# hku-systems/apus

Measured on NVIDIA B200. Metric: committed ops/s, higher is better.
Workload: dtype u8

## Files before the change

### apus_b200/csrc/apus_engine.cu

```cuda
#include <cuda.h>
#include <cuda_runtime.h>
#include <emmintrin.h>
#include <pthread.h>
#include <sched.h>
#include <stdarg.h>
#include <stdint.h>
#include <stdio.h>
#include <stdlib.h>
#include <string.h>
#include <time.h>
#include <unistd.h>

#include "apus_gpu.h"
#include "apus_layout.h"

extern "C" cudaError_t apus_launch_roles(const apus_role_t *d_roles, int n_roles, cudaStream_t stream);
extern "C" size_t apus_kernel_smem_bytes(void);

#define MAX_ROLES 160
static __thread char g_err[512];

static int fail(const char *fmt, ...)
{
    va_list ap;
    va_start(ap, fmt);
    vsnprintf(g_err, sizeof g_err, fmt, ap);
    va_end(ap);
    return APUS_ERROR;
}

#define CK(call)                                                                             \
    do {                                                                                     \
        cudaError_t _e = (call);                                                             \
        if (_e != cudaSuccess)                                                               \
            return fail("%s failed: %s (%s:%d)", #call, cudaGetErrorString(_e), __FILE__, __LINE__); \
    } while (0)

struct drv_t {
    CUresult (*MemCreate)(CUmemGenericAllocationHandle *, size_t, const CUmemAllocationProp *, unsigned long long);
    CUresult (*MemAddressReserve)(CUdeviceptr *, size_t, size_t, CUdeviceptr, unsigned long long);
    CUresult (*MemMap)(CUdeviceptr, size_t, size_t, CUmemGenericAllocationHandle, unsigned long long);
    CUresult (*MemSetAccess)(CUdeviceptr, size_t, const CUmemAccessDesc *, size_t);
    CUresult (*MemGetAllocationGranularity)(size_t *, const CUmemAllocationProp *, CUmemAllocationGranularity_flags);
    CUresult (*MemUnmap)(CUdeviceptr, size_t);
    CUresult (*MemRelease)(CUmemGenericAllocationHandle);
    CUresult (*MemAddressFree)(CUdeviceptr, size_t);
    CUresult (*MulticastCreate)(CUmemGenericAllocationHandle *, const CUmulticastObjectProp *);
    CUresult (*MulticastAddDevice)(CUmemGenericAllocationHandle, CUdevice);
    CUresult (*MulticastBindMem)(CUmemGenericAllocationHandle, size_t, CUmemGenericAllocationHandle, size_t, size_t, unsigned long long);
    CUresult (*MulticastGetGranularity)(size_t *, const CUmulticastObjectProp *, CUmulticastGranularity_flags);
    CUresult (*DeviceGetAttribute)(int *, CUdevice_attribute, CUdevice);
    int ok;
};
static drv_t g_drv;
static int drv_load(void)
{
    if (g_drv.ok) return APUS_OK;
#define DRV(field, name) do { void *fn = NULL; cudaDriverEntryPointQueryResult qr;                                   \
        if (cudaGetDriverEntryPoint(name, &fn, cudaEnableDefault, &qr) != cudaSuccess || !fn) {                    \
            cudaGetLastError(); return fail("driver entry point %s is not available", name); }                      \
        *(void **)(&g_drv.field) = fn; } while (0)
    DRV(MemCreate, "cuMemCreate"); DRV(MemAddressReserve, "cuMemAddressReserve"); DRV(MemMap, "cuMemMap");
    DRV(MemSetAccess, "cuMemSetAccess"); DRV(MemGetAllocationGranularity, "cuMemGetAllocationGranularity");
    DRV(MemUnmap, "cuMemUnmap"); DRV(MemRelease, "cuMemRelease"); DRV(MemAddressFree, "cuMemAddressFree");
    DRV(MulticastCreate, "cuMulticastCreate"); DRV(MulticastAddDevice, "cuMulticastAddDevice");
    DRV(MulticastBindMem, "cuMulticastBindMem"); DRV(MulticastGetGranularity, "cuMulticastGetGranularity");
    DRV(DeviceGetAttribute, "cuDeviceGetAttribute");
#undef DRV
    g_drv.ok = 1;
    return APUS_OK;
}
#define CU(call) do { CUresult _e = (call); if (_e != CUDA_SUCCESS) return fail("%s failed: driver error %d (%s:%d)", #call, (int)_e, __FILE__, __LINE__); } while (0)

struct StageLock {
    pthread_mutex_t *m;
    explicit StageLock(pthread_mutex_t *mu) : m(mu) { pthread_mutex_lock(m); }
    ~StageLock() { pthread_mutex_unlock(m); }
};

struct DeviceGuard {
    int prev;
    bool ok;
    explicit DeviceGuard(int dev) : prev(-1), ok(false)
    {
        if (cudaGetDevice(&prev) != cudaSuccess) prev = -1;
        ok = (cudaSetDevice(dev) == cudaSuccess);
    }
    ~DeviceGuard()
    {
        if (prev >= 0) cudaSetDevice(prev);
    }
};

#define PEER_MAGIC 0x4150555342323030ull

struct peer_blob {
    uint64_t magic;
    int64_t  pid;
    int32_t  device;
    uint32_t pad;
    uint64_t ptr;
    uint64_t bytes;
    cudaIpcMemHandle_t ipc;
};
static_assert(sizeof(peer_blob) <= sizeof(apus_peer_handle_t), "peer handle too small");

struct apus_replica {
    apus_config_t cfg;
    uint64_t log_len;
    uint64_t entries_off;
    uint32_t idx_cap;
    uint8_t *region;
    size_t   region_bytes;
    apus_devctx_t  h_ctx;
    apus_devctx_t *d_ctx;
    apus_role_t   *d_roles;
    apus_hostwords_t *hw;
    apus_hostwords_t *hw_dev;
    apus_slot_t *ring_desc_host;
    uint8_t     *ring_pay_host;
    apus_slot_t *ring_desc_dev;
    uint8_t     *ring_pay_dev;
    uint64_t    *sub_tail_dev;
    uint64_t    *sub_tail_stage;
    uint32_t ring_slots, ring_bytes;
    uint64_t submitted, flushed;
    uint64_t belled;
    CUmemGenericAllocationHandle vmm_handle;
    size_t   vmm_bytes;
    CUmemGenericAllocationHandle mc_handle;
    uint8_t *mc_region;
    uint8_t *stage;
    pthread_mutex_t stage_mu;
    size_t   stage_bytes;
    uint64_t pay_head;
    uint64_t pay_flushed;
    uint64_t *pay_end;
    int      defer;
    cudaStream_t stream, copy_stream;
    cudaEvent_t  ev_start, ev_stop;
    apus_replica *launch_owner;
    int      in_flight;
    uint64_t launches;
    void    *peer_ptr[APUS_MAX_SERVERS];
    int      peer_is_ipc[APUS_MAX_SERVERS];
    uint32_t *d_lat;
};

extern "C" int apus_abi_version(void) { return APUS_ABI_VERSION; }
extern "C" const char *apus_last_error(void) { return g_err; }
extern "C" int apus_device_count(void)
{
    int n = 0;
    if (cudaGetDeviceCount(&n) != cudaSuccess) return 0;
    return n;
}

extern "C" int apus_device_numa_node(int device)
{
    char bus[64] = {0}, path[160];
    if (cudaDeviceGetPCIBusId(bus, sizeof bus, device) != cudaSuccess) { cudaGetLastError(); return -1; }
    for (char *c = bus; *c; c++) if (*c >= 'A' && *c <= 'F') *c = (char)(*c - 'A' + 'a');
    snprintf(path, sizeof path, "/sys/bus/pci/devices/%s/numa_node", bus);
    FILE *f = fopen(path, "r");
    if (!f) return -1;
    int node = -1;
    if (fscanf(f, "%d", &node) != 1) node = -1;
    fclose(f);
    return node;
}

static inline int is_leader(const apus_replica *r) { return r->cfg.server_idx == r->cfg.leader_idx; }

static int ensure_host_ring(apus_replica *r)
{
    if (r->ring_desc_host) return APUS_OK;
    CK(cudaHostAlloc(&r->ring_desc_host, sizeof(apus_slot_t) * r->ring_slots, cudaHostAllocMapped | cudaHostAllocPortable));
    CK(cudaHostAlloc(&r->ring_pay_host, r->ring_bytes, cudaHostAllocMapped | cudaHostAllocPortable));
    return APUS_OK;
}

static int fabric_alloc_region(apus_replica *r);
static int leader_ring_init(apus_replica *r)
{
    if (r->pay_end) return APUS_OK;
    if (!r->ring_slots) { r->ring_slots = r->cfg.ring_slots ? r->cfg.ring_slots : (1u << 16);
                          r->ring_bytes = r->cfg.ring_bytes ? r->cfg.ring_bytes : (16u << 20); }
    r->pay_end = (uint64_t *)calloc(r->ring_slots, sizeof(uint64_t));
    if (!r->pay_end) return fail("out of memory");
    if (r->cfg.ring_mode == APUS_RING_HOST_MAPPED) {
        if (ensure_host_ring(r) != APUS_OK) return APUS_ERROR;
        memset(r->ring_desc_host, 0, sizeof(apus_slot_t) * r->ring_slots);
        CK(cudaHostGetDevicePointer(&r->ring_desc_dev, r->ring_desc_host, 0));
        CK(cudaHostGetDevicePointer(&r->ring_pay_dev, r->ring_pay_host, 0));
    } else {
        CK(cudaMalloc(&r->ring_desc_dev, sizeof(apus_slot_t) * r->ring_slots));
        CK(cudaMalloc(&r->ring_pay_dev, r->ring_bytes));
        CK(cudaMalloc(&r->sub_tail_dev, 128));
        CK(cudaMemset(r->sub_tail_dev, 0, 128));
        CK(cudaHostAlloc(&r->sub_tail_stage, 64, cudaHostAllocPortable));
    }
    return APUS_OK;
}

static int replica_init(apus_replica *r, const apus_config_t *cfg, uint64_t log_len)
{
    r->log_len = log_len;
    uint32_t cap = 1024;
    while ((uint64_t)cap * 64ull < log_len) cap <<= 1;
    r->idx_cap = cap;
    r->entries_off = (APUS_INDEX_OFF + (uint64_t)cap * 4ull + 4095ull) & ~4095ull;
    r->region_bytes = r->entries_off + log_len;
    if (r->cfg.flags & APUS_F_FABRIC) { if (fabric_alloc_region(r) != APUS_OK) return APUS_ERROR; }
    else CK(cudaMalloc(&r->region, r->region_bytes));
    CK(cudaMemset(r->region, 0, r->region_bytes));
    apus_loghdr_t h;
    memset(&h, 0, sizeof h);
    h.len = log_len; h.end = log_len; h.tail = log_len; h.old_end = log_len;
    CK(cudaMemcpy(r->region + APUS_HDR_OFF, &h, sizeof h, cudaMemcpyHostToDevice));
    apus_ctrl_t c;
    memset(&c, 0, sizeof c);
    c.next_idx = 1;
    c.pend_head_end = log_len;
    CK(cudaMemcpy(r->region, &c, sizeof c, cudaMemcpyHostToDevice));

    CK(cudaHostAlloc(&r->hw, sizeof(apus_hostwords_t), cudaHostAllocMapped | cudaHostAllocPortable));
    memset((void *)r->hw, 0, sizeof(apus_hostwords_t));
    CK(cudaHostGetDevicePointer(&r->hw_dev, r->hw, 0));
    pthread_mutex_init(&r->stage_mu, NULL);
    r->stage_bytes = 1u << 20;
    CK(cudaHostAlloc(&r->stage, r->stage_bytes, cudaHostAllocPortable));
    CK(cudaMalloc(&r->d_ctx, sizeof(apus_devctx_t)));
    CK(cudaMalloc(&r->d_roles, sizeof(apus_role_t) * MAX_ROLES));
    CK(cudaMalloc(&r->d_lat, sizeof(uint32_t) * APUS_LAT_RING));
    CK(cudaMemset(r->d_lat, 0, sizeof(uint32_t) * APUS_LAT_RING));
    CK(cudaStreamCreateWithFlags(&r->stream, cudaStreamNonBlocking));
    CK(cudaStreamCreateWithFlags(&r->copy_stream, cudaStreamNonBlocking));
    CK(cudaEventCreate(&r->ev_start));
    CK(cudaEventCreate(&r->ev_stop));

    if (is_leader(r) && leader_ring_init(r) != APUS_OK) return APUS_ERROR;
    {
        apus_ctlwords_t w;
        memset(&w, 0, sizeof w);
        w.sid = (r->cfg.term << 9) | (1ull << 8) | r->cfg.leader_idx;
        for (int i = 0; i < 16; i++) w.vote_ack[i] = log_len;
        CK(cudaMemcpy(r->region + APUS_CTL_OFF, &w, sizeof w, cudaMemcpyHostToDevice));
    }
    r->peer_ptr[cfg->server_idx] = r->region;
    return APUS_OK;
}

extern "C" int apus_replica_create(const apus_config_t *cfg, apus_replica_t **out)
{
    if (!cfg || !out) return fail("null argument");
    if (cfg->struct_size != sizeof(apus_config_t) && cfg->struct_size != APUS_CONFIG_SIZE_V1)
        return fail("apus_config_t size mismatch (ABI)");
    if (cfg->group_size < 1 || cfg->group_size > APUS_MAX_SERVER_COUNT) return fail("group_size out of range");
    if (cfg->server_idx >= cfg->group_size || cfg->leader_idx >= cfg->group_size) return fail("bad server/leader idx");
    int ndev = apus_device_count();
    if (ndev <= 0) return fail("no CUDA device: the engine has no CPU fallback");
    if (cfg->device < 0 || cfg->device >= ndev) return fail("device %d out of range (%d present)", cfg->device, ndev);
    uint64_t log_len = cfg->log_size ? cfg->log_size : APUS_LOG_SIZE;
    if (log_len % 4096 || log_len < 8192) return fail("log_size must be a multiple of 4096 (>= 8192)");
    if (log_len > (1ull << 31)) return fail("log_size above 2 GiB is not supported (32-bit offset index)");
    uint32_t slots = cfg->ring_slots ? cfg->ring_slots : (1u << 16);
    uint32_t bytes = cfg->ring_bytes ? cfg->ring_bytes : (16u << 20);
    if (slots & (slots - 1)) return fail("ring_slots must be a power of two");
    if (bytes % 4096 || bytes < (1u << 17)) return fail("ring_bytes must be a multiple of 4096, >= 128 KiB");
    if (bytes / 16 > 0x00ffffffu) return fail("ring_bytes too large for the 24-bit descriptor offset");

    DeviceGuard g(cfg->device);
    if (!g.ok) return fail("cudaSetDevice(%d) failed", cfg->device);
    apus_replica *r = (apus_replica *)calloc(1, sizeof(*r));
    if (!r) return fail("out of memory");
    memset(&r->cfg, 0, sizeof r->cfg);
    memcpy(&r->cfg, cfg, cfg->struct_size);
    r->cfg.struct_size = sizeof(apus_config_t);
    if (!(r->cfg.flags & APUS_F_EXPLICIT)) r->cfg.flags |= APUS_F_DEVICE_STATS;
    if (cfg->server_idx == cfg->leader_idx) { r->ring_slots = slots; r->ring_bytes = bytes; }
    if (replica_init(r, cfg, log_len) != APUS_OK) {
        char keep[sizeof g_err];
        memcpy(keep, g_err, sizeof keep);
        apus_replica_destroy(r);
        memcpy(g_err, keep, sizeof keep);
        return APUS_ERROR;
    }
    *out = r;
    return APUS_OK;
}

extern "C" void apus_replica_destroy(apus_replica_t *r)
{
    if (!r) return;
    DeviceGuard g(r->cfg.device);
    if (r->in_flight && r->hw) {
        r->hw->stop = 1;
        cudaEventSynchronize(r->launch_owner ? r->launch_owner->ev_stop : r->ev_stop);
    }
    for (int i = 0; i < APUS_MAX_SERVER_COUNT; i++)
        if (r->peer_is_ipc[i] && r->peer_ptr[i]) cudaIpcCloseMemHandle(r->peer_ptr[i]);
    if (r->cfg.ring_mode != APUS_RING_HOST_MAPPED) {
        if (r->ring_desc_dev) cudaFree(r->ring_desc_dev);
        if (r->ring_pay_dev) cudaFree(r->ring_pay_dev);
        if (r->sub_tail_dev) cudaFree(r->sub_tail_dev);
        if (r->sub_tail_stage) cudaFreeHost(r->sub_tail_stage);
    }
    if (r->ring_desc_host) cudaFreeHost(r->ring_desc_host);
    if (r->ring_pay_host) cudaFreeHost(r->ring_pay_host);
    if (r->stage) cudaFreeHost(r->stage);
    if (r->d_lat) cudaFree(r->d_lat);
    if (r->d_roles) cudaFree(r->d_roles);
    if (r->d_ctx) cudaFree(r->d_ctx);
    if (r->ev_start) cudaEventDestroy(r->ev_start);
    if (r->ev_stop) cudaEventDestroy(r->ev_stop);
    if (r->stream) cudaStreamDestroy(r->stream);
    if (r->copy_stream) cudaStreamDestroy(r->copy_stream);
    if (r->hw) cudaFreeHost((void *)r->hw);
    if (r->vmm_handle && g_drv.ok) {
// ... 433 lines not shown
static void pool_run(const fill_job *j)
{
    pthread_mutex_lock(&g_pool_run);
    pthread_mutex_lock(&g_pool.mu);
    if (!g_pool.started) {
        int want = 8;
        const char *e = getenv("apus_submit_threads");
        if (e) want = atoi(e);
        long cores = sysconf(_SC_NPROCESSORS_ONLN);
        if (want > cores - 1) want = (int)cores - 1;
        if (want > POOL_MAX) want = POOL_MAX;
        if (want < 1) want = 1;
        g_pool.nthreads = want - 1;
        for (int i = 0; i < g_pool.nthreads; i++)
            if (pthread_create(&g_pool.th[i], NULL, pool_main, NULL)) { g_pool.nthreads = i; break; }
        g_pool.started = 1;
    }
    g_pool.job = j;
    g_pool.chunk = 4096;
    g_pool.parts = (j->n + g_pool.chunk - 1) / g_pool.chunk;
    g_pool.next = 0; g_pool.done_parts = 0;
    g_pool.progressive = (j->r->cfg.ring_mode == APUS_RING_HOST_MAPPED && !j->r->defer && j->r->flushed == j->r->submitted);
    g_pool.adv = 0; g_pool.adv_lock = 0;
    static uint8_t *done_buf; static uint32_t done_cap;
    if (done_cap < g_pool.parts) { free(done_buf); done_cap = g_pool.parts * 2; done_buf = (uint8_t *)malloc(done_cap); }
    memset(done_buf, 0, g_pool.parts);
    g_pool.done = done_buf;
    __atomic_fetch_add(&g_pool.gen, 1, __ATOMIC_RELEASE);
    pthread_cond_broadcast(&g_pool.cv);
    pthread_mutex_unlock(&g_pool.mu);
    pool_work(j);
    while (__atomic_load_n(&g_pool.done_parts, __ATOMIC_ACQUIRE) < g_pool.parts) _mm_pause();
    pthread_mutex_unlock(&g_pool_run);
}

extern "C" int apus_submit_uniform(apus_replica_t *r, uint32_t n, uint8_t type, uint16_t connection_id,
                                   uint64_t first_req_id, uint16_t len, const void *payloads, size_t stride,
                                   uint64_t *first_ticket)
{
    if (!r) return fail("null argument");
    if (!is_leader(r)) return fail("submit on a follower");
    if (len && !payloads) return fail("null payload");
    if (n == 0) return APUS_OK;
    const uint64_t consumed = r->hw->consumed;
    if (r->submitted + n - consumed > r->ring_slots) { snprintf(g_err, sizeof g_err, "submission ring full"); return APUS_RETRY; }
    if (!r->ring_desc_host && ensure_host_ring(r) != APUS_OK) return APUS_ERROR;
    const uint32_t mask = r->ring_slots - 1;
    const uint32_t nb = image_bytes(type, len);
    fill_job j;
    memset(&j, 0, sizeof j);
    j.r = r; j.n = n; j.type = type; j.conn = connection_id; j.first_req = first_req_id; j.len = len;
    j.payloads = (const uint8_t *)payloads; j.stride = stride; j.first_slot = r->submitted;
    uint32_t *tos = NULL; uint64_t *poss = NULL;
    uint64_t head = r->pay_head;
    if (nb > APUS_SLOT_INLINE) {
        tos = (uint32_t *)malloc(sizeof(uint32_t) * n); poss = (uint64_t *)malloc(sizeof(uint64_t) * n);
        if (!tos || !poss) { free(tos); free(poss); return fail("out of memory"); }
        for (uint32_t k = 0; k < n; k++) {
            int rc = place_image(r, type, nb, consumed, &head, &tos[k], &poss[k]);
            if (rc != APUS_OK) { free(tos); free(poss); snprintf(g_err, sizeof g_err, "payload ring full"); return rc; }
            r->pay_end[(r->submitted + k) & mask] = head;
        }
        j.type_off = tos; j.pos = poss;
    } else {
        j.type_off_inline = ((uint32_t)type & APUS_SLOT_TYPE_MASK) << APUS_SLOT_TYPE_SHIFT;
        for (uint32_t k = 0; k < n; k++) r->pay_end[(r->submitted + k) & mask] = head;
    }
    if (n >= 16384) pool_run(&j); else fill_range(&j, 0, n);
    free(tos); free(poss);
    r->pay_head = head;
    if (first_ticket) *first_ticket = r->submitted + 1;
    r->submitted += n;
    if (!r->defer) return ring_flush(r);
    return APUS_OK;
}

__global__ void apus_synth_kernel(apus_slot_t *ring, uint32_t mask, uint8_t *pay, uint64_t first_slot, uint32_t n,
                                  uint32_t type, uint32_t conn, uint64_t first_req, uint32_t len, uint32_t seed,
                                  uint64_t pay_pos0, uint32_t need)
{
    for (uint32_t k = blockIdx.x * blockDim.x + threadIdx.x; k < n; k += gridDim.x * blockDim.x) {
        const uint64_t s = first_slot + k, req = first_req + k;
        apus_slot_t *d = &ring[s & mask];
        const uint32_t nb = 2u + len;
        uint32_t type_off = (type & APUS_SLOT_TYPE_MASK) << APUS_SLOT_TYPE_SHIFT;
        uint8_t *dst0 = d->inl0, *dst1 = d->inl1;
        if (need) {
            const uint64_t pos = pay_pos0 + (uint64_t)k * need;
            type_off |= APUS_SLOT_EXT | (uint32_t)(pos / 16);
            uint8_t *p = pay + pos;
            p[0] = (uint8_t)len; p[1] = (uint8_t)(len >> 8);
            for (uint32_t q = 0; q < len; q++) p[2 + q] = synth_byte(seed, req, q);
        } else {
            for (uint32_t q = 0; q < nb; q++) {
                const uint8_t v = q == 0 ? (uint8_t)len : q == 1 ? (uint8_t)(len >> 8) : synth_byte(seed, req, q - 2);
                if (q < 32) dst0[q] = v; else dst1[q - 32] = v;
            }
        }
        d->req_id = req; d->type_off = type_off; d->len = (uint16_t)len; d->clt_id = (uint16_t)conn;
        d->stamp0 = s + 1; d->stamp1 = s + 1; d->rsv0 = 0; d->rsv1 = 0;
    }
}

extern "C" int apus_submit_synth(apus_replica_t *r, uint32_t n, uint8_t type, uint16_t connection_id,
                                 uint64_t first_req_id, uint16_t len, uint32_t seed, uint64_t *first_ticket)
{
    if (!r) return fail("null argument");
    if (!is_leader(r)) return fail("submit on a follower");
    if (r->cfg.ring_mode != APUS_RING_DEVICE) return fail("apus_submit_synth needs the device submission ring");
    if (type == APUS_NOOP || type == APUS_CONFIG || type == APUS_HEAD) return fail("apus_submit_synth: request types only");
    if (n == 0) return APUS_OK;
    const uint64_t consumed = r->hw->consumed;
    if (r->submitted + n - consumed > r->ring_slots) { snprintf(g_err, sizeof g_err, "submission ring full"); return APUS_RETRY; }
    if (r->flushed != r->submitted) { int rc = ring_push(r); if (rc != APUS_OK) return rc; }
    const uint32_t mask = r->ring_slots - 1;
    const uint32_t nb = 2u + len;
    uint32_t need = 0;
    uint64_t pos0 = 0, head = r->pay_head;
    if (nb > APUS_SLOT_INLINE) {
        need = (nb + 15u) & ~15u;
        const uint64_t R = r->ring_bytes;
        pos0 = head % R;
        const uint64_t tail = consumed ? r->pay_end[(consumed - 1) & mask] : 0;
        if (pos0 + (uint64_t)n * need > R || (head - tail) + (uint64_t)n * need > R)
            return fail("apus_submit_synth: %u images of %u B do not fit the payload ring without wrapping", n, need);
    }
    DeviceGuard g(r->cfg.device);
    const int threads = 256;
    int blocks = (int)((n + threads - 1) / threads);
    if (blocks > 148 * 8) blocks = 148 * 8;
    apus_synth_kernel<<<blocks, threads, 0, r->copy_stream>>>(r->ring_desc_dev, mask, r->ring_pay_dev, r->submitted, n, type,
                                                              connection_id, first_req_id, len, seed, pos0, need);
    CK(cudaGetLastError());
    CK(cudaStreamSynchronize(r->copy_stream));
    for (uint32_t k = 0; k < n; k++) { head += need; r->pay_end[(r->submitted + k) & mask] = head; }
    r->pay_head = head; r->pay_flushed = head;
    if (first_ticket) *first_ticket = r->submitted + 1;
    r->submitted += n;
    r->flushed = r->submitted;
    if (!r->defer) return ring_bell(r, r->submitted);
    return APUS_OK;
}

extern "C" int apus_submit_defer(apus_replica_t *r, int defer)
{
    if (!r) return fail("null argument");
    r->defer = defer;
    return APUS_OK;
}
extern "C" int apus_submit_flush(apus_replica_t *r)
{
    if (!r) return fail("null argument");
    return ring_flush(r);
}
extern "C" int apus_submit_release(apus_replica_t *r, uint64_t ticket)
{
    if (!r) return fail("null argument");
    if (ticket > r->submitted) return fail("release beyond what was submitted");
    int rc = ring_push(r);
    if (rc != APUS_OK) return rc;
    DeviceGuard g(r->cfg.device);
    return ring_bell(r, ticket);
}

extern "C" uint64_t apus_committed_tickets(apus_replica_t *r) { return r ? r->hw->committed_tickets : 0; }

extern "C" int apus_progress(apus_replica_t *r, uint64_t *offset, uint64_t *count)
{
    if (!r) return fail("null argument");
    const __m128i v = _mm_load_si128((const __m128i *)(const void *)&r->hw->commit_off);
    uint64_t w[2];
    _mm_storeu_si128((__m128i *)w, v);
    if (offset) *offset = w[0];
    if (count) *count = w[1];
    return r->hw->error ? fail("kernel reported protocol error %llu", (unsigned long long)r->hw->error) : APUS_OK;
}

extern "C" int apus_wait_committed(apus_replica_t *r, uint64_t ticket, int64_t timeout_us)
{
    if (!r) return fail("null argument");
    if (r->hw->committed_tickets >= ticket) return APUS_OK;
    struct timespec t0, t;
    clock_gettime(CLOCK_MONOTONIC, &t0);
    uint32_t spins = 0;
    while (r->hw->committed_tickets < ticket) {
        if ((++spins & 0x3ff) == 0) {
            if (r->hw->error) return fail("kernel reported protocol error %llu", (unsigned long long)r->hw->error);
            if (timeout_us >= 0) {
                clock_gettime(CLOCK_MONOTONIC, &t);
                int64_t us = (t.tv_sec - t0.tv_sec) * 1000000 + (t.tv_nsec - t0.tv_nsec) / 1000;
                if (us > timeout_us) { snprintf(g_err, sizeof g_err, "timeout"); return APUS_RETRY; }
            }
        }
    }
    return APUS_OK;
}

extern "C" int apus_closed_loop(apus_replica_t *r, uint32_t n, uint16_t payload_len, uint16_t connection_id,
                                uint64_t first_req_id, uint32_t *lat_ns)
{
    if (!r || !lat_ns) return fail("null argument");
    if (!is_leader(r)) return fail("submit on a follower");
    uint8_t *buf = (uint8_t *)malloc(payload_len ? payload_len : 1);
    if (!buf) return fail("out of memory");
    for (uint32_t k = 0; k < payload_len; k++) buf[k] = (uint8_t)(k * 131u + 7u);
    struct timespec t0, t1;
    for (uint32_t i = 0; i < n; i++) {
        clock_gettime(CLOCK_MONOTONIC, &t0);
        int rc = ring_put(r, APUS_SEND, connection_id, first_req_id + i, buf, payload_len);
        if (rc == APUS_OK) rc = ring_flush(r);
        if (rc != APUS_OK) { free(buf); return rc == APUS_RETRY ? rc : fail("closed loop: submit failed"); }
        const uint64_t ticket = r->submitted;
        uint32_t spins = 0;
        while (r->hw->committed_tickets < ticket) {
            if ((++spins & 0xffffff) == 0) {
                clock_gettime(CLOCK_MONOTONIC, &t1);
                if (t1.tv_sec - t0.tv_sec > 10 || r->hw->error) { free(buf); return fail("closed loop: commit timeout"); }
            }
        }
        clock_gettime(CLOCK_MONOTONIC, &t1);
        int64_t ns = (t1.tv_sec - t0.tv_sec) * 1000000000ll + (t1.tv_nsec - t0.tv_nsec);
        lat_ns[i] = ns > 0xffffffffll ? 0xffffffffu : (uint32_t)ns;
    }
    free(buf);
    return APUS_OK;
}

extern "C" int apus_log_offsets(apus_replica_t *r, apus_log_offsets_t *out)
{
    if (!r || !out) return fail("null argument");
    DeviceGuard g(r->cfg.device);
    apus_loghdr_t h;
    CK(cudaMemcpyAsync(&h, r->region + APUS_HDR_OFF, sizeof h, cudaMemcpyDeviceToHost, r->copy_stream));
    CK(cudaStreamSynchronize(r->copy_stream));
    out->head = h.head; out->apply = h.apply; out->commit = h.commit; out->end = h.end;
    out->tail = h.tail; out->old_end = h.old_end; out->old_commit = h.old_commit; out->len = h.len;
    return APUS_OK;
}

extern "C" int apus_log_read(apus_replica_t *r, uint64_t off, uint64_t len, void *dst)
{
    if (!r || !dst) return fail("null argument");
    if (off + len > r->log_len) return fail("range beyond the log");
    DeviceGuard g(r->cfg.device);
    StageLock sl(&r->stage_mu);
    uint8_t *out = (uint8_t *)dst;
    while (len) {
        const uint64_t run = len < r->stage_bytes ? len : r->stage_bytes;
        CK(cudaMemcpyAsync(r->stage, r->region + r->entries_off + off, run, cudaMemcpyDeviceToHost, r->copy_stream));
        CK(cudaStreamSynchronize(r->copy_stream));
        memcpy(out, r->stage, run);
        out += run; off += run; len -= run;
    }
    return APUS_OK;
}

extern "C" int apus_log_read_range(apus_replica_t *r, uint64_t from, uint64_t to, void *dst, uint64_t cap, uint64_t *got)
{
    if (!r || !dst || !got) return fail("null argument");
    if (from >= r->log_len || to >= r->log_len) return fail("range beyond the log");
    const uint64_t L = r->log_len;
    uint64_t n1 = to >= from ? to - from : L - from, n2 = to >= from ? 0 : to;
    if (n1 > cap) { n1 = cap; n2 = 0; }
    if (n1 + n2 > cap) n2 = cap - n1;
    int rc = n1 ? apus_log_read(r, from, n1, dst) : APUS_OK;
    if (rc == APUS_OK && n2) rc = apus_log_read(r, 0, n2, (uint8_t *)dst + n1);
    *got = n1 + n2;
    return rc;
}

extern "C" int apus_set_applied(apus_replica_t *r, uint64_t offset)
{
    if (!r) return fail("null argument");
    if (offset >= r->log_len) return fail("offset beyond the log");
    r->hw->host_apply = offset;
    return APUS_OK;
}

extern "C" uint64_t apus_leader_suspect(apus_replica_t *r) { return r ? r->hw->leader_suspect : 0; }
extern "C" uint64_t apus_last_commit_ns(apus_replica_t *r) { return r ? r->hw->last_commit_ns : 0; }

extern "C" int apus_get_stats(apus_replica_t *r, apus_stats_t *out)
{
    if (!r || !out) return fail("null argument");
    DeviceGuard g(r->cfg.device);
    apus_ctrl_t c;
    CK(cudaMemcpyAsync(&c, r->region, sizeof c, cudaMemcpyDeviceToHost, r->copy_stream));
    CK(cudaStreamSynchronize(r->copy_stream));
    memset(out, 0, sizeof *out);
    out->tickets_submitted = r->submitted;
    out->tickets_consumed = c.consumed;
    out->tickets_committed = c.committed_tickets;
    out->entries_acked = c.acked;
    out->bytes_replicated = c.bytes_replicated;
    out->batches = c.batches;
    out->kernel_launches = r->launches;
    out->lat_samples = c.lat_count;
    out->auto_heads = c.auto_heads;
    out->entries_published = c.published;
    for (int i = 0; i < 8; i++) { out->phase_ns[i] = c.phase_ns[i]; out->turn_ns[i] = c.turn_ns[i]; }
    return APUS_OK;
}

extern "C" int apus_latency_samples(apus_replica_t *r, uint32_t *dst, uint32_t max, uint32_t *n)
{
    if (!r || !dst || !n) return fail("null argument");
    DeviceGuard g(r->cfg.device);
    apus_ctrl_t c;
    CK(cudaMemcpyAsync(&c, r->region, sizeof c, cudaMemcpyDeviceToHost, r->copy_stream));
    CK(cudaStreamSynchronize(r->copy_stream));
    uint64_t have = c.lat_count < APUS_LAT_RING ? c.lat_count : APUS_LAT_RING;
    uint32_t take = (uint32_t)(have < max ? have : max);
    uint32_t *tmp = (uint32_t *)malloc(sizeof(uint32_t) * APUS_LAT_RING);
    if (!tmp) return fail("out of memory");
    cudaError_t e = cudaMemcpyAsync(tmp, r->d_lat, sizeof(uint32_t) * APUS_LAT_RING, cudaMemcpyDeviceToHost, r->copy_stream);
    if (e == cudaSuccess) e = cudaStreamSynchronize(r->copy_stream);
    if (e != cudaSuccess) { free(tmp); return fail("latency copy failed: %s", cudaGetErrorString(e)); }
    for (uint32_t k = 0; k < take; k++)
        dst[k] = tmp[(c.lat_count - take + k) & (APUS_LAT_RING - 1)];
    free(tmp);
    *n = take;
    return APUS_OK;
}



static int fabric_alloc_region(apus_replica *r)
{
    if (drv_load() != APUS_OK) return APUS_ERROR;
    int ndev = apus_device_count();
    CUmemAllocationProp ap;
    memset(&ap, 0, sizeof ap);
    ap.type = CU_MEM_ALLOCATION_TYPE_PINNED;
    ap.location.type = CU_MEM_LOCATION_TYPE_DEVICE;
    ap.location.id = r->cfg.device;
    ap.requestedHandleTypes = CU_MEM_HANDLE_TYPE_POSIX_FILE_DESCRIPTOR;
    size_t gran = 0;
    CU(g_drv.MemGetAllocationGranularity(&gran, &ap, CU_MEM_ALLOC_GRANULARITY_RECOMMENDED));
    if (gran < (2u << 20)) gran = 2u << 20;
    r->vmm_bytes = (r->region_bytes + gran - 1) / gran * gran;
    CU(g_drv.MemCreate(&r->vmm_handle, r->vmm_bytes, &ap, 0));
    CUdeviceptr va = 0;
    CU(g_drv.MemAddressReserve(&va, r->vmm_bytes, gran, 0, 0));
    CU(g_drv.MemMap(va, r->vmm_bytes, 0, r->vmm_handle, 0));
    CUmemAccessDesc acc[64];
    for (int d = 0; d < ndev && d < 64; d++) { acc[d].location.type = CU_MEM_LOCATION_TYPE_DEVICE; acc[d].location.id = d; acc[d].flags = CU_MEM_ACCESS_FLAGS_PROT_READWRITE; }
    CU(g_drv.MemSetAccess(va, r->vmm_bytes, acc, (size_t)(ndev < 64 ? ndev : 64)));
    r->region = (uint8_t *)va;
    return APUS_OK;
}

extern "C" int apus_group_multicast(apus_replica_t **rs, int n)
{
    if (!rs || n < 2 || n > APUS_MAX_SERVER_COUNT) return fail("bad replica list");
    if (drv_load() != APUS_OK) return APUS_ERROR;
    apus_replica *lead = NULL;
    for (int i = 0; i < n; i++) {
        if (!rs[i] || !rs[i]->vmm_handle) return fail("replica %d was not created with APUS_F_FABRIC", i);
        if (rs[i]->in_flight) return fail("stop the kernels first");
        if (rs[i]->vmm_bytes != rs[0]->vmm_bytes) return fail("regions differ in size");
        for (int j = 0; j < i; j++) if (rs[j]->cfg.device == rs[i]->cfg.device) return fail("multicast needs one GPU per replica");
        int mc = 0;
        CU(g_drv.DeviceGetAttribute(&mc, CU_DEVICE_ATTRIBUTE_MULTICAST_SUPPORTED, rs[i]->cfg.device));
        if (!mc) return fail("device %d does not support multicast", rs[i]->cfg.device);
        if (is_leader(rs[i])) lead = rs[i];
    }
    if (!lead) return fail("no leader in the list");
    if (lead->mc_region) return APUS_OK;
    CUmulticastObjectProp mp;
    memset(&mp, 0, sizeof mp);
    mp.numDevices = (unsigned)n; mp.size = lead->vmm_bytes; mp.handleTypes = CU_MEM_HANDLE_TYPE_POSIX_FILE_DESCRIPTOR;
    size_t mgran = 0;
    CU(g_drv.MulticastGetGranularity(&mgran, &mp, CU_MULTICAST_GRANULARITY_MINIMUM));
    if (lead->vmm_bytes % mgran) return fail("region size %zu is not a multiple of the multicast granularity %zu", lead->vmm_bytes, mgran);
    CU(g_drv.MulticastCreate(&lead->mc_handle, &mp));
    for (int i = 0; i < n; i++) CU(g_drv.MulticastAddDevice(lead->mc_handle, rs[i]->cfg.device));
    for (int i = 0; i < n; i++) {
        DeviceGuard g(rs[i]->cfg.device);
        CU(g_drv.MulticastBindMem(lead->mc_handle, 0, rs[i]->vmm_handle, 0, rs[i]->vmm_bytes, 0));
    }
    DeviceGuard g(lead->cfg.device);
    CUdeviceptr va = 0;
    CU(g_drv.MemAddressReserve(&va, lead->vmm_bytes, mgran, 0, 0));
    CU(g_drv.MemMap(va, lead->vmm_bytes, 0, lead->mc_handle, 0));
    CUmemAccessDesc acc;
    acc.location.type = CU_MEM_LOCATION_TYPE_DEVICE; acc.location.id = lead->cfg.device; acc.flags = CU_MEM_ACCESS_FLAGS_PROT_READWRITE;
    CU(g_drv.MemSetAccess(va, lead->vmm_bytes, &acc, 1));
    lead->mc_region = (uint8_t *)va;
    return APUS_OK;
}

#define SID_TERM(s) ((s) >> 9)

static int own_read(apus_replica *r, size_t off, void *dst, size_t len)
{
    StageLock sl(&r->stage_mu);
    CK(cudaMemcpyAsync(r->stage, r->region + off, len, cudaMemcpyDeviceToHost, r->copy_stream));
    CK(cudaStreamSynchronize(r->copy_stream));
    memcpy(dst, r->stage, len);
    return APUS_OK;
}
static int own_write(apus_replica *r, size_t off, const void *src, size_t len)
{
    StageLock sl(&r->stage_mu);
    memcpy(r->stage, src, len);
    CK(cudaMemcpyAsync(r->region + off, r->stage, len, cudaMemcpyHostToDevice, r->copy_stream));
    CK(cudaStreamSynchronize(r->copy_stream));
    return APUS_OK;
}
static int peer_read(apus_replica *r, uint8_t peer, size_t off, void *dst, size_t len)
{
    StageLock sl(&r->stage_mu);
    if (!r->peer_ptr[peer]) return fail("peer %u is not connected", (unsigned)peer);
    CK(cudaMemcpyAsync(r->stage, (uint8_t *)r->peer_ptr[peer] + off, len, cudaMemcpyDefault, r->copy_stream));
    CK(cudaStreamSynchronize(r->copy_stream));
    memcpy(dst, r->stage, len);
    return APUS_OK;
}
static int peer_write(apus_replica *r, uint8_t peer, size_t off, const void *src, size_t len)
{
    StageLock sl(&r->stage_mu);
    if (!r->peer_ptr[peer]) return fail("peer %u is not connected", (unsigned)peer);
    memcpy(r->stage, src, len);
    CK(cudaMemcpyAsync((uint8_t *)r->peer_ptr[peer] + off, r->stage, len, cudaMemcpyDefault, r->copy_stream));
    CK(cudaStreamSynchronize(r->copy_stream));
    return APUS_OK;
}

extern "C" int apus_ctl_read(apus_replica_t *r, apus_ctl_view_t *out)
{
    if (!r || !out) return fail("null argument");
    DeviceGuard g(r->cfg.device);
    apus_ctlwords_t w;
    if (own_read(r, APUS_CTL_OFF, &w, sizeof w) != APUS_OK) return APUS_ERROR;
    memset(out, 0, sizeof *out);
    out->sid = w.sid; out->leader_sid = w.leader_sid; out->adj_end = w.adj_end; out->adj_count = w.adj_count;
    for (int i = 0; i < APUS_MAX_SERVER_COUNT; i++) {
        out->vote_ack[i] = w.vote_ack[i];
        out->vote_req[i].sid = w.vote_req[i].sid; out->vote_req[i].index = w.vote_req[i].index;
        out->vote_req[i].term = w.vote_req[i].term;
        out->vote_req[i].cid[0] = w.vote_req[i].cid[0]; out->vote_req[i].cid[1] = w.vote_req[i].cid[1];
    }
    return APUS_OK;
}

extern "C" int apus_ctl_set_sid(apus_replica_t *r, uint64_t sid)
{
    if (!r) return fail("null argument");
    DeviceGuard g(r->cfg.device);
    return own_write(r, APUS_CTL_OFF + offsetof(apus_ctlwords_t, sid), &sid, 8);
}

extern "C" int apus_ctl_reset_votes(apus_replica_t *r)
{
    if (!r) return fail("null argument");
    DeviceGuard g(r->cfg.device);
    uint64_t v[16];
    for (int i = 0; i < 16; i++) v[i] = r->log_len;
    return own_write(r, APUS_CTL_OFF + offsetof(apus_ctlwords_t, vote_ack), v, sizeof v);
}

extern "C" int apus_ctl_clear_vote_request(apus_replica_t *r, uint8_t from_idx)
{
    if (!r || from_idx >= APUS_MAX_SERVER_COUNT) return fail("bad argument");
    DeviceGuard g(r->cfg.device);
    uint64_t z = 0;
    return own_write(r, APUS_CTL_OFF + offsetof(apus_ctlwords_t, vote_req) + sizeof(apus_vote_req_t) * from_idx, &z, 8);
}

extern "C" int apus_ctl_send_vote_request(apus_replica_t *r, uint8_t peer_idx, uint64_t sid, uint64_t index, uint64_t term,
                                          const void *cid16)
{
    if (!r || peer_idx >= r->cfg.group_size) return fail("bad argument");
    DeviceGuard g(r->cfg.device);
    apus_vote_req_t q;
    memset(&q, 0, sizeof q);
    q.index = index; q.term = term;
    if (cid16) memcpy(q.cid, cid16, 16);
    const size_t base = APUS_CTL_OFF + offsetof(apus_ctlwords_t, vote_req) + sizeof(apus_vote_req_t) * r->cfg.server_idx;
    if (peer_write(r, peer_idx, base + 8, (uint8_t *)&q + 8, sizeof q - 8) != APUS_OK) return APUS_ERROR;
    return peer_write(r, peer_idx, base, &sid, 8);
}

extern "C" int apus_ctl_send_vote_ack(apus_replica_t *r, uint8_t candidate_idx, uint64_t commit)
{
    if (!r || candidate_idx >= r->cfg.group_size) return fail("bad argument");
    DeviceGuard g(r->cfg.device);
    return peer_write(r, candidate_idx, APUS_CTL_OFF + offsetof(apus_ctlwords_t, vote_ack) + 8u * r->cfg.server_idx, &commit, 8);
}

static int entry_at(apus_replica *r, int peer, uint64_t cum, uint64_t *off, uint64_t *idx, uint64_t *term, uint32_t *stride)
{
    uint32_t w = 0;
    const size_t ioff = APUS_INDEX_OFF + 4ull * (cum & (r->idx_cap - 1));
    int rc = peer < 0 ? own_read(r, ioff, &w, 4) : peer_read(r, (uint8_t)peer, ioff, &w, 4);
    if (rc != APUS_OK) return rc;
    const uint64_t o = w & ~APUS_IDX_HEAD_FLAG;
    if (o + APUS_HDR_BYTES > r->log_len) return fail("offset index names an offset beyond the log");
    uint8_t h[64];
    rc = peer < 0 ? own_read(r, r->entries_off + o, h, 64) : peer_read(r, (uint8_t)peer, r->entries_off + o, h, 64);
    if (rc != APUS_OK) return rc;
    memcpy(idx, h + E_IDX, 8); memcpy(term, h + E_TERM, 8);
    uint16_t len; memcpy(&len, h + E_DATA, 2);
    const uint8_t ty = h[E_TYPE];
    *stride = (ty == T_NOOP || ty == T_CONFIG || ty == T_HEAD) ? APUS_HDR_BYTES : APUS_HDR_BYTES + len;
    *off = o;
    return APUS_OK;
}

extern "C" int apus_ctl_heartbeat(apus_replica_t *r, uint64_t *word)
{
    if (!r || !word) return fail("null argument");
    DeviceGuard g(r->cfg.device);
    return own_read(r, offsetof(apus_ctrl_t, hb), word, sizeof *word);
}

extern "C" int apus_ctl_last_entry(apus_replica_t *r, uint64_t *idx, uint64_t *term, uint64_t *commit, uint64_t *end)
{
    if (!r || !idx || !term) return fail("null argument");
    if (r->in_flight) return fail("the replica's kernel must be stopped (exclusive log access)");
    DeviceGuard g(r->cfg.device);
    apus_loghdr_t h; apus_ctrl_t c;
    if (own_read(r, APUS_HDR_OFF, &h, sizeof h) != APUS_OK || own_read(r, 0, &c, sizeof c) != APUS_OK) return APUS_ERROR;
    if (commit) *commit = h.commit;
    if (end) *end = h.end;
    const uint64_t count = is_leader(r) ? c.published : c.acked;
    *idx = 0; *term = 0;
    if (h.end == r->log_len || count == 0) return APUS_OK;
    uint64_t off; uint32_t stride;
    if (entry_at(r, -1, count, &off, idx, term, &stride) != APUS_OK) return APUS_ERROR;
    if (*idx != count) return fail("entry counter %llu does not match the idx %llu of the last entry", (unsigned long long)count, (unsigned long long)*idx);
    return APUS_OK;
}

static int copy_to_peer(apus_replica *r, uint8_t peer, size_t off, size_t len)
{
    if (!len) return APUS_OK;
    CK(cudaMemcpyAsync((uint8_t *)r->peer_ptr[peer] + off, r->region + off, len, cudaMemcpyDefault, r->copy_stream));
    return APUS_OK;
}

extern "C" int apus_ctl_adjust_follower(apus_replica_t *r, uint8_t peer, uint64_t sid, uint64_t *resent)
{
    if (!r || peer >= r->cfg.group_size || peer == r->cfg.server_idx) return fail("bad argument");
    if (!is_leader(r)) return fail("log adjustment is the leader's job");
    if (r->in_flight) return fail("the leader's kernel must be stopped");
    if (!r->peer_ptr[peer]) return fail("peer %u is not connected", (unsigned)peer);
    DeviceGuard g(r->cfg.device);
    const uint64_t L = r->log_len;
    apus_loghdr_t mh, fh; apus_ctrl_t mc, fc;
    if (own_read(r, APUS_HDR_OFF, &mh, sizeof mh) != APUS_OK || own_read(r, 0, &mc, sizeof mc) != APUS_OK) return APUS_ERROR;
    if (peer_read(r, peer, APUS_HDR_OFF, &fh, sizeof fh) != APUS_OK || peer_read(r, peer, 0, &fc, sizeof fc) != APUS_OK) return APUS_ERROR;
    const uint64_t mine = mc.published, theirs = fc.acked;
    uint64_t j = mine < theirs ? mine : theirs;
    uint64_t keep_end = (mh.end == L) ? L : 0;
    bool found = false;
    while (j > 0) {
        uint64_t o1, i1, t1, o2, i2, t2; uint32_t s1, s2;
        if (entry_at(r, -1, j, &o1, &i1, &t1, &s1) != APUS_OK || entry_at(r, peer, j, &o2, &i2, &t2, &s2) != APUS_OK) return APUS_ERROR;
        if (o1 == o2 && i1 == i2 && t1 == t2 && i1 == j) { keep_end = o1 + s1; if (keep_end == L) keep_end = 0; found = true; break; }
        j--;
    }
    if (!found) { j = 0; keep_end = 0; }
    uint64_t bytes = 0;
    if (mine > j && mh.end != L) {
        const uint64_t from = (j == 0) ? mh.head : keep_end;
        const uint64_t to = mh.end;
        if (to > from) { if (copy_to_peer(r, peer, r->entries_off + from, to - from) != APUS_OK) return APUS_ERROR; bytes += to - from; }
        else if (to < from || (to == from && mine > j)) {
            if (copy_to_peer(r, peer, r->entries_off + from, L - from) != APUS_OK) return APUS_ERROR;
            if (copy_to_peer(r, peer, r->entries_off, to) != APUS_OK) return APUS_ERROR;
            bytes += L - from + to;
        }
        const uint64_t cap = r->idx_cap, a = (j + 1) & (cap - 1), n = mine - j;
        if (n >= cap) { if (copy_to_peer(r, peer, APUS_INDEX_OFF, 4ull * cap) != APUS_OK) return APUS_ERROR; }
        else if (a + n <= cap) { if (copy_to_peer(r, peer, APUS_INDEX_OFF + 4ull * a, 4ull * n) != APUS_OK) return APUS_ERROR; }
        else {
            if (copy_to_peer(r, peer, APUS_INDEX_OFF + 4ull * a, 4ull * (cap - a)) != APUS_OK) return APUS_ERROR;
            if (copy_to_peer(r, peer, APUS_INDEX_OFF, 4ull * (a + n - cap)) != APUS_OK) return APUS_ERROR;
        }
        CK(cudaStreamSynchronize(r->copy_stream));
    }
    if (j == 0) {
        if (peer_write(r, peer, APUS_HDR_OFF + offsetof(apus_loghdr_t, head), &mh.head, 8) != APUS_OK) return APUS_ERROR;
        if (peer_write(r, peer, APUS_HDR_OFF + offsetof(apus_loghdr_t, commit), &mh.commit, 8) != APUS_OK) return APUS_ERROR;
    }
    const uint64_t endw[2] = { mh.end, mh.end };
    if (peer_write(r, peer, APUS_HDR_OFF + offsetof(apus_loghdr_t, end), &endw[0], 8) != APUS_OK) return APUS_ERROR;
    if (peer_write(r, peer, APUS_HDR_OFF + offsetof(apus_loghdr_t, old_end), &endw[1], 8) != APUS_OK) return APUS_ERROR;
    if (peer_write(r, peer, offsetof(apus_ctrl_t, acked), &mine, 8) != APUS_OK) return APUS_ERROR;
    const uint64_t none = L;
    if (peer_write(r, peer, offsetof(apus_ctrl_t, pend_head_end), &none, 8) != APUS_OK) return APUS_ERROR;
    if (own_write(r, offsetof(apus_ctrl_t, ack) + 8u * peer, &mine, 8) != APUS_OK) return APUS_ERROR;
    const uint64_t adj[3] = { sid, mh.end, mine };
    if (peer_write(r, peer, APUS_CTL_OFF + offsetof(apus_ctlwords_t, adj_end), &adj[1], 16) != APUS_OK) return APUS_ERROR;
    if (peer_write(r, peer, APUS_CTL_OFF + offsetof(apus_ctlwords_t, leader_sid), &adj[0], 8) != APUS_OK) return APUS_ERROR;
    if (resent) *resent = bytes;
    return APUS_OK;
}

extern "C" int apus_follower_beats(apus_replica_t *r, uint64_t out[APUS_MAX_SERVER_COUNT])
{
    if (!r || !out) return fail("null argument");
    DeviceGuard g(r->cfg.device);
    uint64_t b[16];
    if (own_read(r, offsetof(apus_ctrl_t, fbeat), b, sizeof b) != APUS_OK) return APUS_ERROR;
// ... 83 lines not shown
```

### apus_b200/csrc/apus_kernels.cu

```cuda
#include <cuda_runtime.h>
#include <stdint.h>

#include "apus_layout.h"
#include "apus_cert.h"

__device__ __forceinline__ uint64_t ld_relaxed_sys(const volatile void *p)
{
    uint64_t v;
    asm volatile("ld.relaxed.sys.global.u64 %0, [%1];" : "=l"(v) : "l"(p) : "memory");
    return v;
}
__device__ __forceinline__ uint64_t ld_acquire_sys(const volatile void *p)
{
    uint64_t v;
    asm volatile("ld.acquire.sys.global.u64 %0, [%1];" : "=l"(v) : "l"(p) : "memory");
    return v;
}
__device__ __forceinline__ uint32_t ld_relaxed_sys_u32(const volatile void *p)
{
    uint32_t v;
    asm volatile("ld.relaxed.sys.global.u32 %0, [%1];" : "=r"(v) : "l"(p) : "memory");
    return v;
}
__device__ __forceinline__ void ld_acquire_sys_2x64(const volatile void *p, uint64_t &a, uint64_t &b)
{
    asm volatile("ld.acquire.sys.global.v2.u64 {%0,%1}, [%2];" : "=l"(a), "=l"(b) : "l"(p) : "memory");
}
__device__ __forceinline__ void ld_relaxed_sys_2x64(const volatile void *p, uint64_t &a, uint64_t &b)
{
    asm volatile("ld.relaxed.sys.global.v2.u64 {%0,%1}, [%2];" : "=l"(a), "=l"(b) : "l"(p) : "memory");
}
__device__ __forceinline__ void st_relaxed_sys(volatile void *p, uint64_t v)
{
    asm volatile("st.relaxed.sys.global.u64 [%0], %1;" ::"l"(p), "l"(v) : "memory");
}
__device__ __forceinline__ void st_relaxed_sys_2x64(volatile void *p, uint64_t a, uint64_t b)
{
    asm volatile("st.relaxed.sys.global.v2.u64 [%0], {%1,%2};" ::"l"(p), "l"(a), "l"(b) : "memory");
}
__device__ __forceinline__ void st_relaxed_sys_u8(volatile void *p, uint8_t v)
{
    asm volatile("st.relaxed.sys.global.u8 [%0], %1;" ::"l"(p), "r"((uint32_t)v) : "memory");
}
__device__ __forceinline__ uint4 ld_relaxed_sys_v4(const void *p)
{
    uint4 v;
    asm volatile("ld.relaxed.sys.global.v4.u32 {%0,%1,%2,%3}, [%4];"
                 : "=r"(v.x), "=r"(v.y), "=r"(v.z), "=r"(v.w)
                 : "l"(p)
                 : "memory");
    return v;
}
__device__ __forceinline__ void st_v4(void *p, uint4 v)
{
    asm volatile("st.global.v4.u32 [%0], {%1,%2,%3,%4};" ::"l"(p), "r"(v.x), "r"(v.y), "r"(v.z),
                 "r"(v.w)
                 : "memory");
}
__device__ __forceinline__ void mst_v4(void *p, uint4 v)
{
    asm volatile("multimem.st.relaxed.sys.global.v4.f32 [%0], {%1,%2,%3,%4};" ::"l"(p), "f"(__uint_as_float(v.x)),
                 "f"(__uint_as_float(v.y)), "f"(__uint_as_float(v.z)), "f"(__uint_as_float(v.w))
                 : "memory");
}
__device__ __forceinline__ void mst_u32(void *p, uint32_t v)
{
    asm volatile("multimem.st.relaxed.sys.global.b32 [%0], %1;" ::"l"(p), "r"(v) : "memory");
}
__device__ __forceinline__ void st_u8(void *p, uint32_t v)
{
    asm volatile("st.global.u8 [%0], %1;" ::"l"(p), "r"(v) : "memory");
}
__device__ __forceinline__ uint64_t globaltimer_ns()
{
    uint64_t t;
    asm volatile("mov.u64 %0, %%globaltimer;" : "=l"(t));
    return t;
}
__device__ __forceinline__ void bar_sync(int id, int nthreads)
{
    asm volatile("bar.sync %0, %1;" ::"r"(id), "r"(nthreads) : "memory");
}

__device__ __forceinline__ bool has_cmd(uint32_t type)
{
    return !(type == T_NOOP || type == T_CONFIG || type == T_HEAD);
}
__device__ __forceinline__ uint32_t data_bytes(uint32_t type, uint32_t len)
{
    if (type == T_NOOP) return 0;
    if (type == T_CONFIG) return 16;
    if (type == T_HEAD) return 8;
    return 2u + len;
}
__device__ __forceinline__ uint32_t entry_stride(uint32_t type, uint32_t len)
{
    return has_cmd(type) ? APUS_HDR_BYTES + len : APUS_HDR_BYTES;
}
__device__ __forceinline__ uint64_t ring_dist(uint64_t from, uint64_t to, uint64_t L)
{
    return to >= from ? to - from : L - (from - to);
}
__device__ __forceinline__ uint64_t adopt_head(uint64_t head, uint64_t carried, uint64_t new_end, uint64_t L)
{
    if (carried >= L) return head;
    const uint64_t ne = (new_end == L) ? 0 : new_end;
    return (ring_dist(head, carried, L) <= ring_dist(head, ne, L)) ? carried : head;
}
__device__ __forceinline__ uint64_t slot_head_value(const apus_cslot_t *sl)
{
    uint64_t v = 0;
#pragma unroll
    for (int q = 7; q >= 0; q--) v = (v << 8) | sl->inl[q];
    return v;
}

#define WATCHDOG_NS (20ull * 1000ull * 1000ull * 1000ull)

#define APUS_KERR_WATCHDOG_LEADER   1
#define APUS_KERR_WATCHDOG_FOLLOWER 2
#define APUS_KERR_WATCHDOG_COMMIT   3
#define APUS_KERR_BAD_ENTRY         4
#define APUS_KERR_COUNT_MISMATCH    5

#define N_PRODUCER_WARPS 15
#define NT (N_PRODUCER_WARPS * 32)
#define MAXB APUS_MAX_TILE_ENTRIES
#define PUBMASK (APUS_PUBRING_RECORDS - 1)

struct LeaderShared {
    uint32_t es[MAXB];
    uint32_t xb[MAXB];
    uint32_t cum_es[MAXB];
    uint32_t cum_xb[MAXB];
    uint32_t rel[MAXB];
    uint32_t xoff[MAXB];
    uint64_t ap[32];
    uint32_t ap_valid;
    uint32_t static_cut;
    uint32_t first_ext_all;
    uint32_t host_head_k;
    uint64_t idx_base;
    uint8_t  ty[MAXB];
    uint8_t  flg[MAXB];
    uint32_t n_fetch, finish, abort, was_blocked;
    uint32_t avg_es, avg_xb;
    uint64_t slot0, my_seq, t_dequeue, st_head, t_place_acq, pub_h, pub_tail_seen;
    uint64_t st_end, st_tail, st_next_idx, st_hwm, st_placed;
    uint32_t st_prev_head, pad0;
    uint32_t kbase, m, gap, ghost, fresh, auto_head, ext_bytes, last, blocked, hbytes;
    uint32_t base_es, base_xb, fast, pad1;
    uint64_t ext_base, auto_head_val, a, b, idx0, cum_after, new_end, tail_after, hwm_after;
    uint8_t  *peer_entries[APUS_MAX_SERVERS];
    uint32_t *peer_index[APUS_MAX_SERVERS];
};

#define LS_BYTES ((sizeof(LeaderShared) + 127u) & ~127u)
#define L_SLOTS_OFF LS_BYTES
#define L_EXT_OFF   (L_SLOTS_OFF + MAXB * APUS_CSLOT_BYTES)
#define L_IMG_OFF   (L_EXT_OFF + APUS_LEADER_EXT_BYTES)
#define L_TOTAL     (L_IMG_OFF + APUS_LEADER_IMG_BYTES + 16)

struct FollowerShared {
    uint32_t off[APUS_FOLLOWER_WIN_BYTES / 64 + 8];
    uint32_t n;
    uint32_t done;
    uint64_t win_lo, win_hi, next;
    uint64_t head_val, head_end;
    uint64_t end_seen, cum_seen, commit_seen;
    uint32_t head_j;
    uint32_t cert;
    uint64_t cert_start;
};
#define FS_BYTES ((sizeof(FollowerShared) + 127u) & ~127u)
#define F_TOTAL (FS_BYTES + APUS_FOLLOWER_WIN_BYTES + 16)

extern __shared__ __align__(16) uint8_t smem_raw[];

__device__ __forceinline__ uint64_t ld_acquire_gpu(const volatile void *p)
{
    uint64_t v;
    asm volatile("ld.acquire.gpu.global.u64 %0, [%1];" : "=l"(v) : "l"(p) : "memory");
    return v;
}
__device__ __forceinline__ void ld_acquire_gpu_2x64(const volatile void *p, uint64_t &a, uint64_t &b)
{
    asm volatile("ld.acquire.gpu.global.v2.u64 {%0,%1}, [%2];" : "=l"(a), "=l"(b) : "l"(p) : "memory");
}
__device__ __forceinline__ void st_release_gpu(volatile void *p, uint64_t v)
{
    asm volatile("st.release.gpu.global.u64 [%0], %1;" ::"l"(p), "l"(v) : "memory");
}

__device__ __forceinline__ uint64_t cs_chunk(const uint4 v, uint64_t lo, uint64_t a, uint64_t b)
{
    return cs_chunk_words((uint64_t)v.x | ((uint64_t)v.y << 32), (uint64_t)v.z | ((uint64_t)v.w << 32), lo, a, b);
}
__device__ __forceinline__ uint4 chunk_select(const uint4 nw, const uint4 old, int n)
{
    uint32_t a[4] = {nw.x, nw.y, nw.z, nw.w}, o[4] = {old.x, old.y, old.z, old.w}, r[4];
#pragma unroll
    for (int w = 0; w < 4; w++) {
        const int k = n - 4 * w;
        const uint32_t m = k >= 4 ? 0xffffffffu : (k <= 0 ? 0u : ((1u << (8 * k)) - 1u));
        r[w] = (a[w] & m) | (o[w] & ~m);
    }
    return make_uint4(r[0], r[1], r[2], r[3]);
}


__device__ __forceinline__ uint32_t hdr_byte(uint32_t j, uint64_t idx, uint64_t term, uint64_t req_id,
                                             uint32_t clt, uint32_t type, uint32_t sender)
{
    if (j < 8) return (uint32_t)(idx >> (8 * j)) & 0xFF;
    if (j < 16) return (uint32_t)(term >> (8 * (j - 8))) & 0xFF;
    if (j < 24) return (uint32_t)(req_id >> (8 * (j - 16))) & 0xFF;
    if (j == 24) return clt & 0xFF;
    if (j == 25) return (clt >> 8) & 0xFF;
    if (j == 26) return type;
    if (j == 27) return sender;
    return 0;
}

__device__ __noinline__ void group_write_header(uint8_t *e, int sub, int gl, uint64_t idx, uint64_t term, uint64_t req_id,
                                                   uint32_t clt, uint32_t type, uint32_t sender, bool skip_sender)
{
    if ((((uint32_t)(uintptr_t)e) & 15u) == 0 && !skip_sender) {
        if (sub == 0) *reinterpret_cast<uint4 *>(e + 0) = make_uint4((uint32_t)idx, (uint32_t)(idx >> 32), (uint32_t)term, (uint32_t)(term >> 32));
        else if (sub == 1) *reinterpret_cast<uint4 *>(e + 16) = make_uint4((uint32_t)req_id, (uint32_t)(req_id >> 32),
                                                                         (clt & 0xffffu) | (type << 16) | (sender << 24), 0u);
        else if (sub == 2) *reinterpret_cast<uint64_t *>(e + 32) = 0;
        else if (sub == 3) e[40] = 0;
    } else if ((((uint32_t)(uintptr_t)e) & 7u) == 0) {
        if (sub == 0) *reinterpret_cast<uint64_t *>(e + 0) = idx;
        else if (sub == 1) *reinterpret_cast<uint64_t *>(e + 8) = term;
        else if (sub == 2) *reinterpret_cast<uint64_t *>(e + 16) = req_id;
        else if (sub == 3) {
            if (skip_sender) {
                e[24] = (uint8_t)clt; e[25] = (uint8_t)(clt >> 8); e[26] = (uint8_t)type;
                e[28] = 0; e[29] = 0; e[30] = 0; e[31] = 0;
            } else {
                *reinterpret_cast<uint64_t *>(e + 24) =
                    (uint64_t)(clt & 0xffffu) | ((uint64_t)type << 16) | ((uint64_t)sender << 24);
            }
        } else if (sub == 4) *reinterpret_cast<uint64_t *>(e + 32) = 0;
        else if (sub == 5) e[40] = 0;
    } else {
        for (uint32_t j = sub; j < 41; j += gl)
            if (!(skip_sender && j == E_SENDER)) e[j] = (uint8_t)hdr_byte(j, idx, term, req_id, clt, type, sender);
    }
}

__device__ __noinline__ void group_copy_smem(uint8_t *dst, const uint8_t *src, uint32_t nbytes, int sub, int gl)
{
    const uint32_t nchunks = (nbytes + 15u) >> 4;
    const uint32_t dalign = (uint32_t)(uintptr_t)dst & 15u;
    for (uint32_t c = sub; c < nchunks; c += gl) {
        const uint4 v = *reinterpret_cast<const uint4 *>(src + 16u * c);
        uint8_t *d = dst + 16u * c;
        const uint32_t left = nbytes - 16u * c;
        if (dalign == 0 && left >= 16) {
            *reinterpret_cast<uint4 *>(d) = v;
        } else if ((dalign & 3u) == 0 && left >= 16) {
            uint32_t *d4 = reinterpret_cast<uint32_t *>(d);
            d4[0] = v.x; d4[1] = v.y; d4[2] = v.z; d4[3] = v.w;
        } else if ((dalign & 1u) == 0 && left >= 16) {
            uint16_t *d2 = reinterpret_cast<uint16_t *>(d);
            const uint32_t w[4] = {v.x, v.y, v.z, v.w};
#pragma unroll
            for (int k = 0; k < 8; k++) d2[k] = (uint16_t)(w[k >> 1] >> (16 * (k & 1)));
        } else {
            const uint32_t w[4] = {v.x, v.y, v.z, v.w};
            const uint32_t nb = left < 16 ? left : 16;
#pragma unroll
            for (uint32_t k = 0; k < 16; k++)
                if (k < nb) d[k] = (uint8_t)(w[k >> 2] >> (8 * (k & 3)));
        }
    }
}

__device__ __noinline__ void cta_fetch_chunks(uint8_t *dst, const uint8_t *src, uint32_t nchunks, int tid)
{
    uint32_t c = tid;
    for (; c + 3u * NT < nchunks; c += 4u * NT) {
        const uint4 v0 = ld_relaxed_sys_v4(src + 16ull * c);
        const uint4 v1 = ld_relaxed_sys_v4(src + 16ull * (c + NT));
        const uint4 v2 = ld_relaxed_sys_v4(src + 16ull * (c + 2u * NT));
        const uint4 v3 = ld_relaxed_sys_v4(src + 16ull * (c + 3u * NT));
        reinterpret_cast<uint4 *>(dst)[c] = v0;
        reinterpret_cast<uint4 *>(dst)[c + NT] = v1;
        reinterpret_cast<uint4 *>(dst)[c + 2u * NT] = v2;
        reinterpret_cast<uint4 *>(dst)[c + 3u * NT] = v3;
    }
    for (; c < nchunks; c += NT) reinterpret_cast<uint4 *>(dst)[c] = ld_relaxed_sys_v4(src + 16ull * c);
}

__device__ __forceinline__ void note_desc(LeaderShared *S, uint32_t k, const uint4 v)
{
    const uint32_t to = v.z, ty = (to >> APUS_SLOT_TYPE_SHIFT) & APUS_SLOT_TYPE_MASK, len = v.w & 0xffffu;
    S->ty[k] = (uint8_t)ty;
    S->flg[k] = (uint8_t)(((to & APUS_SLOT_EXT) ? 1u : 0u) | ((to & APUS_SLOT_WRAP) ? 2u : 0u));
    S->es[k] = entry_stride(ty, len);
    S->xb[k] = (to & APUS_SLOT_EXT) ? ((data_bytes(ty, len) + 15u) & ~15u) : 0u;
}

__device__ __noinline__ void cta_fetch_slots(LeaderShared *S, uint8_t *slots, const apus_slot_t *ring, uint64_t s, uint32_t k0,
                                                uint32_t cnt, int tid)
{
    const uint8_t *src = reinterpret_cast<const uint8_t *>(ring + s);
    uint8_t *dst = slots + (size_t)k0 * APUS_CSLOT_BYTES;
    const uint32_t nq = cnt * 6u;
    uint32_t q = (tid >= 32) ? tid - 32 : tid + NT - 32;
#define SRC_OF(qq, kk, rr) const uint32_t kk = (qq) / 6u, rr = (qq) - 6u * kk; const uint8_t *p_##qq = src + (size_t)kk * APUS_SLOT_BYTES + 16u * (rr < 3u ? rr : rr + 1u)
    for (; q + 3u * NT < nq; q += 4u * NT) {
        const uint32_t q0 = q, q1 = q + NT, q2 = q + 2u * NT, q3 = q + 3u * NT;
        SRC_OF(q0, ka, ra); SRC_OF(q1, kb, rb); SRC_OF(q2, kc, rc); SRC_OF(q3, kd, rd);
        const uint4 v0 = ld_relaxed_sys_v4(p_q0);
        const uint4 v1 = ld_relaxed_sys_v4(p_q1);
        const uint4 v2 = ld_relaxed_sys_v4(p_q2);
        const uint4 v3 = ld_relaxed_sys_v4(p_q3);
        reinterpret_cast<uint4 *>(dst)[q0] = v0;
        reinterpret_cast<uint4 *>(dst)[q1] = v1;
        reinterpret_cast<uint4 *>(dst)[q2] = v2;
        reinterpret_cast<uint4 *>(dst)[q3] = v3;
        if (ra == 0) note_desc(S, k0 + ka, v0);
        if (rb == 0) note_desc(S, k0 + kb, v1);
        if (rc == 0) note_desc(S, k0 + kc, v2);
        if (rd == 0) note_desc(S, k0 + kd, v3);
    }
    for (; q < nq; q += NT) {
        const uint32_t q0 = q;
        SRC_OF(q0, ka, ra);
        const uint4 v = ld_relaxed_sys_v4(p_q0);
        reinterpret_cast<uint4 *>(dst)[q0] = v;
        if (ra == 0) note_desc(S, k0 + ka, v);
    }
#undef SRC_OF
}

__device__ void leader_commit_warp(const apus_devctx_t *__restrict__ cx)
{
    const int lane = threadIdx.x & 31;
    const int N = cx->group_size, me = cx->idx, quorum = cx->quorum;
    apus_ctrl_t *ctrl = reinterpret_cast<apus_ctrl_t *>(cx->region);
    apus_seq_t *seq = reinterpret_cast<apus_seq_t *>(cx->region + APUS_SEQ_OFF);
    const apus_pubrec_t *ring = reinterpret_cast<const apus_pubrec_t *>(cx->region + APUS_PUBRING_OFF);
    apus_loghdr_t *hdr = reinterpret_cast<apus_loghdr_t *>(cx->region + APUS_HDR_OFF);
    apus_hostwords_t *hw = cx->hw;
    uint64_t committed = ctrl->committed;
    uint64_t committed_tickets = ctrl->committed_tickets;
    uint64_t lat_count = ctrl->lat_count;
    uint64_t bytes_rep = ctrl->bytes_replicated, batches = ctrl->batches;
    uint64_t tail = 0;
    uint64_t seen = 0;
    uint64_t published = ctrl->published;
    uint64_t last_progress = globaltimer_ns();
    uint32_t spins = 0, hb_spins = 0;
    uint64_t last_hb = 0, hb_beat = globaltimer_ns() >> 10;
    bool S_rec_ok = false;
    volatile uint64_t *peer_commit = nullptr;
    if (lane < N && lane != me && cx->peer[lane])
        peer_commit = &reinterpret_cast<apus_loghdr_t *>(cx->peer[lane] + APUS_HDR_OFF)->commit;

    for (;;) {
        uint64_t st = 0, rv = 0, v = 0;
        const uint64_t seen_before = seen;
        {
            const uint64_t rn = seen + (uint64_t)(lane >> 3);
            ld_relaxed_sys_2x64(&ring[rn & PUBMASK].w[2 * (lane & 7)], st, rv);
            const uint32_t okm = __ballot_sync(0xffffffffu, st == rn + 1);
            uint32_t nvalid = 0;
            while (nvalid < 4 && ((okm >> (8 * nvalid)) & 0xffu) == 0xffu) nvalid++;
            if (nvalid) {
                published = __shfl_sync(0xffffffffu, rv, 8 * (nvalid - 1) + PR_CUM);
                seen += nvalid;
            }
            S_rec_ok = nvalid != 0;
        }
        if (lane < N && lane != me) v = ld_relaxed_sys(&ctrl->ack[lane]);
        if (lane == me) v = published;
        int cnt = 0;
        for (int j = 0; j < N; j++) {
            uint64_t vj = __shfl_sync(0xffffffffu, v, j);
            cnt += (vj >= v) ? 1 : 0;
        }
        uint64_t cand = (lane < N && cnt >= quorum) ? v : 0;
        for (int s = 16; s > 0; s >>= 1) {
            uint64_t o = __shfl_xor_sync(0xffffffffu, cand, s);
            cand = o > cand ? o : cand;
        }
        const uint64_t Q = cand;
        if (Q > committed && tail != seen) {
            uint64_t off = 0, tickets = committed_tickets, r_tail = 0, r_hwm = 0, r_next = 0;
            bool any = false;
            bool reuse = (tail == seen_before);
            while (tail != seen) {
                const uint64_t rn = tail + (uint64_t)(lane >> 3);
                uint64_t st2 = 0, val = 0;
                if (reuse) { val = rv; reuse = false; }
                else if (rn < seen) ld_relaxed_sys_2x64(&ring[rn & PUBMASK].w[2 * (lane & 7)], st2, val);
                const uint32_t cm = __ballot_sync(0xffffffffu, (lane & 7) == PR_CUM && rn < seen && val <= Q);
                uint32_t nc = 0;
                while (nc < 4 && ((cm >> (8 * nc)) & 1u)) nc++;
                if (nc == 0) break;
                const int base = 8 * (int)(nc - 1);
                committed = __shfl_sync(0xffffffffu, val, base + PR_CUM);
                off = __shfl_sync(0xffffffffu, val, base + PR_END);
                tickets = __shfl_sync(0xffffffffu, val, base + PR_TICKETS);
                r_tail = __shfl_sync(0xffffffffu, val, base + PR_TAIL);
                r_hwm = __shfl_sync(0xffffffffu, val, base + PR_HWM);
                r_next = __shfl_sync(0xffffffffu, val, base + PR_NEXTIDX);
                for (uint32_t q = 0; q < nc; q++) {
                    bytes_rep += __shfl_sync(0xffffffffu, val, 8 * q + PR_BYTES);
                    const uint64_t t0 = __shfl_sync(0xffffffffu, val, 8 * q + PR_T0);
                    if ((cx->flags & APUS_FLAG_STATS) && cx->lat_ns && lane == 0) {
                        const uint64_t d = globaltimer_ns() - t0;
                        cx->lat_ns[(lat_count + q) & (APUS_LAT_RING - 1)] = d > 0xffffffffull ? 0xffffffffu : (uint32_t)d;
                    }
                }
                lat_count += nc; batches += nc;
                tail += nc;
                any = true;
                if (nc < 4) break;
            }
            if (any) {
                if (peer_commit) st_relaxed_sys(peer_commit, off);
                if (lane == 0) {
                    st_relaxed_sys_2x64(&hw->commit_off, off, tickets);
                    st_relaxed_sys(&hw->consumed, tickets);
                    st_relaxed_sys(&hw->last_commit_ns, globaltimer_ns());
                    st_relaxed_sys(&seq->pub_tail, tail);
                    hdr->commit = off;
                    st_relaxed_sys(&hdr->apply, off);
                    hdr->end = off; hdr->tail = r_tail; hdr->old_end = off;
                    ctrl->committed = committed; ctrl->committed_tickets = tickets; ctrl->lat_count = lat_count;
                    ctrl->published = committed; ctrl->consumed = tickets; ctrl->next_idx = r_next; ctrl->hwm = r_hwm;
                    ctrl->bytes_replicated = bytes_rep; ctrl->batches = batches;
                }
                committed_tickets = tickets;
                last_progress = globaltimer_ns();
                __syncwarp();
            }
        }
        if (cx->hb_period_ns && (++hb_spins & 0x1fu) == 0) {
            const uint64_t now = globaltimer_ns();
            if (now - last_hb >= cx->hb_period_ns) {
                last_hb = now; hb_beat++;
                if (lane < N && lane != me && cx->peer[lane])
                    st_relaxed_sys(&reinterpret_cast<apus_ctrl_t *>(cx->peer[lane])->hb,
                                   ((cx->term & 0xffffull) << APUS_PUB_TERM_SHIFT) | (hb_beat & APUS_PUB_CUM_MASK));
            }
        }
        const bool rec_ok = S_rec_ok;
        int ex = 0;
        if (lane == 0) {
            if (!rec_ok && tail == seen && committed == published && ld_acquire_gpu(&seq->workers_done) == cx->n_workers) {
                ex = 3;
            } else if ((++spins & 0x3ffu) == 0) {
                if (ld_relaxed_sys(&seq->abort_flag)) ex = 2;
                else if (globaltimer_ns() - last_progress > WATCHDOG_NS && (tail != seen || committed != published) &&
                         (cx->target != ~0ull || ld_relaxed_sys_u32(&hw->stop))) {
                    st_relaxed_sys(&hw->error, APUS_KERR_WATCHDOG_COMMIT);
                    st_relaxed_sys(&seq->abort_flag, 1);
                    ex = 2;
                }
            }
        }
        ex = __shfl_sync(0xffffffffu, ex, 0);
        if (ex == 3) {
            uint64_t st3 = 0, v3 = 0;
            if (lane >= 16 && lane < 24) ld_relaxed_sys_2x64(&ring[seen & PUBMASK].w[2 * (lane - 16)], st3, v3);
            const bool more = __ballot_sync(0xffffffffu, lane >= 16 && lane < 24 && st3 == seen + 1) == 0x00ff0000u;
            ex = more ? 0 : 1;
        }
        if (ex) {
            if (ex == 1 && cx->target != ~0ull && lane < N && lane != me && cx->peer[lane]) {
                apus_ctrl_t *pc = reinterpret_cast<apus_ctrl_t *>(cx->peer[lane]);
                st_relaxed_sys(&pc->fin_entries, committed);
                __threadfence_system();
                st_relaxed_sys(&pc->fin_target, cx->target);
            }
            break;
        }
    }
}

__device__ __noinline__ void leader_prescan(const apus_devctx_t *__restrict__ cx, LeaderShared *S, int lane)
{
    const uint32_t nf = S->n_fetch;
    uint32_t carry = 0, xcarry = 0, scut = nf, fext = 0xffffffffu, hhk = 0xffffffffu;
    const uint32_t es0 = S->es[0], xb0 = S->xb[0];
    bool uniform = true;
    for (uint32_t r = 0; r < nf; r += 32) {
        const uint32_t k = r + lane;
        if (__ballot_sync(0xffffffffu, k < nf && (S->es[k] != es0 || S->xb[k] != xb0))) { uniform = false; break; }
    }
    for (uint32_t r = 0; r < nf; r += 32) {
        const uint32_t k = r + lane;
        const bool in = k < nf;
        uint32_t inc = in ? S->es[k] : 0u, xinc = in ? S->xb[k] : 0u;
        if (uniform) {
            if (in) { S->cum_es[k] = (k + 1u) * es0; S->cum_xb[k] = (k + 1u) * xb0; }
        } else {
#pragma unroll
            for (int sft = 1; sft < 32; sft <<= 1) {
                const uint32_t o = __shfl_up_sync(0xffffffffu, inc, sft);
                const uint32_t xo = __shfl_up_sync(0xffffffffu, xinc, sft);
                if (lane >= sft) { inc += o; xinc += xo; }
            }
            if (in) { S->cum_es[k] = carry + inc; S->cum_xb[k] = xcarry + xinc; }
            carry += __shfl_sync(0xffffffffu, inc, 31);
            xcarry += __shfl_sync(0xffffffffu, xinc, 31);
        }
        const uint32_t hm = __ballot_sync(0xffffffffu, in && S->ty[k] == T_HEAD);
        if (hm) hhk = r + (31u - (uint32_t)__clz(hm));
        const uint32_t wm = __ballot_sync(0xffffffffu, in && k > 0 && (S->flg[k] & 2u));
        const uint32_t em = __ballot_sync(0xffffffffu, in && (S->flg[k] & 1u));
        if (wm && scut == nf) scut = r + (uint32_t)(__ffs(wm) - 1);
        if (em && fext == 0xffffffffu) fext = r + (uint32_t)(__ffs(em) - 1);
    }
    if (lane == 0) { S->static_cut = scut; S->first_ext_all = fext; S->host_head_k = hhk; }
}

__device__ __noinline__ void leader_place(const apus_devctx_t *__restrict__ cx, LeaderShared *S, const apus_cslot_t *sl, int lane)
{
    const int N = cx->group_size;
    apus_loghdr_t *hdr = reinterpret_cast<apus_loghdr_t *>(cx->region + APUS_HDR_OFF);
    const uint64_t L = cx->log_len;
    const bool autoprune = (cx->flags & APUS_FLAG_AUTOPRUNE) != 0;
    const uint32_t kbase = S->kbase, nf = S->n_fetch;
    const uint64_t end = S->st_end;

    uint64_t head = S->st_head;
    const uint64_t pos0 = (end == L) ? 0 : end;
    uint64_t used = (end == L) ? 0 : ring_dist(head, end, L);
    uint32_t autoh = 0;
    uint64_t new_head = 0;
    if (autoprune && end != L && used >= (L >> 2) && (!S->st_prev_head || S->was_blocked) && L - pos0 >= APUS_HDR_BYTES) {
        uint64_t d = 0;
        if (lane < N) {
            d = ring_dist(S->ap[lane], end, L);
            if (d > used) d = used;
        }
#pragma unroll
        for (int sft = 16; sft > 0; sft >>= 1) {
            const uint64_t o = __shfl_xor_sync(0xffffffffu, d, sft);
            d = o > d ? o : d;
        }
        if (d == 0) d = ring_dist(S->st_tail, end, L);
        if (d <= used && used - d >= (L >> 3)) {
            autoh = 1;
            new_head = (end >= d) ? end - d : L - (d - end);
            used = d;
            head = new_head;
        }
    }
    const uint32_t hbytes = autoh ? APUS_HDR_BYTES : 0;
    uint64_t lim = L - pos0;
    const uint64_t imgcap = APUS_LEADER_IMG_BYTES - 16u - (pos0 & 15u);
    if (lim > imgcap) lim = imgcap;
    const uint64_t reserve = autoprune ? APUS_HDR_BYTES : 0;
    const uint64_t lim_space = (L - used > 1 + reserve) ? (L - used - 1 - reserve) : 0;
    const uint64_t limit = lim < lim_space ? lim : lim_space;
    const uint32_t base_es = kbase ? S->cum_es[kbase - 1] : 0u, base_xb = kbase ? S->cum_xb[kbase - 1] : 0u;

    uint32_t m = nf - kbase, first_ext = 0xffffffffu;
    for (uint32_t r = kbase; r < nf; r += 32) {
        const uint32_t k = r + lane;
        const bool in = k < nf;
        const bool bad = in && ((uint64_t)hbytes + (S->cum_es[k] - base_es) > limit ||
                                S->cum_xb[k] - base_xb > APUS_LEADER_EXT_BYTES || (k > kbase && (S->flg[k] & 2u)));
        const uint32_t badmask = __ballot_sync(0xffffffffu, bad);
        const uint32_t good = badmask ? (uint32_t)(__ffs(badmask) - 1) : 32u;
        if (first_ext == 0xffffffffu) {
            const uint32_t extmask = __ballot_sync(0xffffffffu, in && (uint32_t)lane < good && (S->flg[k] & 1u));
            if (extmask) first_ext = r + (uint32_t)(__ffs(extmask) - 1);
        }
        if (badmask) { m = r + good - kbase; break; }
    }
    if (lane == 0) {
        const uint32_t carry = hbytes + (m ? S->cum_es[kbase + m - 1] - base_es : 0u);
        const uint32_t xcarry = m ? S->cum_xb[kbase + m - 1] - base_xb : 0u;
        S->gap = 0; S->ghost = 0; S->blocked = 0; S->last = 0;
        uint64_t a = pos0, b = pos0;
        if (m == 0 && !autoh) {
            const uint32_t es0 = S->es[kbase];
            const uint64_t left = L - pos0;
            if (es0 > left && used + left + es0 + reserve < L) {
                S->gap = 1;
                S->ghost = (left >= APUS_HDR_BYTES && has_cmd(S->ty[kbase])) ? 1u : 0u;
                b = L;
            } else {
                S->blocked = 1;
            }
        } else {
            b = pos0 + carry;
        }
        S->a = a; S->b = b; S->m = m;
        S->hbytes = hbytes; S->base_es = base_es; S->base_xb = base_xb;
        S->ext_bytes = (m && first_ext != 0xffffffffu) ? xcarry : 0u;
        S->ext_base = (first_ext != 0xffffffffu) ? (uint64_t)(sl[first_ext].type_off & APUS_SLOT_OFF_MASK) * 16ull : 0ull;
        S->auto_head = autoh; S->auto_head_val = new_head;
        S->idx0 = S->st_next_idx;
        S->fresh = (a >= S->st_hwm) ? 1u : 0u;
        if (S->blocked) S->was_blocked = 1;
        if (!S->blocked) {
            S->was_blocked = 0;
            if (autoh) st_relaxed_sys(&hdr->head, new_head);
            if (autoh) S->st_head = new_head;
            if (S->host_head_k != 0xffffffffu && S->host_head_k >= kbase && S->host_head_k < kbase + m) {
                const uint64_t nh = adopt_head(S->st_head, slot_head_value(&sl[S->host_head_k]), b, L);
                if (nh != S->st_head) { S->st_head = nh; st_relaxed_sys(&hdr->head, nh); }
            }
            if (S->gap) {
                S->st_end = 0; S->st_hwm = L;
            } else {
                uint64_t ne = b; if (ne == L) ne = 0;
                S->new_end = ne;
                S->st_end = ne;
                S->st_tail = m ? a + hbytes + (S->cum_es[kbase + m - 1] - base_es) - S->es[kbase + m - 1] : a;
                S->tail_after = S->st_tail;
                S->st_next_idx += m + autoh;
                S->st_placed += m + autoh;
                S->cum_after = S->st_placed;
                if (autoh) atomicAdd(reinterpret_cast<unsigned long long *>(&reinterpret_cast<apus_ctrl_t *>(cx->region)->auto_heads), 1ull);
                S->st_prev_head = (autoh && m == 0) ? 1u : 0u;
                if (b > S->st_hwm) S->st_hwm = b;
                S->last = (kbase + m == nf) ? 1u : 0u;
            }
            S->hwm_after = S->st_hwm;
        }
    }
}


struct Express {
    uint64_t next_seq;
    uint64_t placed, end, tf, head;
    uint64_t pub_h;
    uint32_t have_place;
    uint32_t hold;
    uint64_t pub_tail_seen;
    uint64_t dt[5];
};

__device__ __forceinline__ void express_release(apus_seq_t *seq, Express &X, int lane)
{
    __syncwarp();
    if (lane == 0) {
        __threadfence_system();
        st_relaxed_sys_2x64(seq->pub_turn, X.next_seq, X.pub_h);
    }
    X.hold = 0;
    __syncwarp();
}

__device__ __noinline__ int leader_express(const apus_devctx_t *__restrict__ cx, const LeaderShared *S, Express &X,
                                              const uint64_t claimed, uint4 sv, const bool have_slot, uint8_t *scratch,
                                              const int lane, const uint4 pf, const uint64_t pf_pos)
{
    const int N = cx->group_size, me = cx->idx;
    const uint64_t L = cx->log_len;
    apus_ctrl_t *ctrl = reinterpret_cast<apus_ctrl_t *>(cx->region);
    apus_seq_t *seq = reinterpret_cast<apus_seq_t *>(cx->region + APUS_SEQ_OFF);
    apus_pubrec_t *pubring = reinterpret_cast<apus_pubrec_t *>(cx->region + APUS_PUBRING_OFF);
    uint8_t *entries = cx->region + cx->entries_off;
    uint32_t *lindex = reinterpret_cast<uint32_t *>(cx->region + APUS_INDEX_OFF);
    const uint64_t t_deq = (cx->flags & (APUS_FLAG_STATS | APUS_FLAG_PROFILE)) ? globaltimer_ns() : 0;

    if (!have_slot && lane < 8)
        sv = ld_relaxed_sys_v4(reinterpret_cast<const uint8_t *>(cx->sub_slots + (claimed & cx->sub_mask)) + 16u * lane);
    const uint32_t to = __shfl_sync(0xffffffffu, sv.z, 0), lw = __shfl_sync(0xffffffffu, sv.w, 0);
    const uint32_t ty = (to >> APUS_SLOT_TYPE_SHIFT) & APUS_SLOT_TYPE_MASK, len = lw & 0xffffu, clt = lw >> 16;
    const uint64_t req_id = (uint64_t)__shfl_sync(0xffffffffu, sv.x, 0) | ((uint64_t)__shfl_sync(0xffffffffu, sv.y, 0) << 32);
    if (!has_cmd(ty) || (to & APUS_SLOT_EXT)) return 1;
    const uint32_t es = APUS_HDR_BYTES + len, nb = 2u + len;

    const bool isf = lane < N && lane != me && cx->peer[lane];
    uint64_t ackv = 0;
    if (isf) ackv = ld_relaxed_sys(&ctrl->ack[lane]);

    uint64_t placed = X.placed, end = X.end, tf = X.tf, headv = X.head;
    if (!(X.have_place && X.next_seq == claimed)) {
        uint32_t ab = 0;
        if (lane == 0) {
            uint64_t s0, s1, s2, s3;
            uint32_t spins = 0;
            for (;;) {
                ld_relaxed_sys_2x64(seq->rec_placed, s0, placed);
                ld_relaxed_sys_2x64(seq->rec_end, s1, end);
                ld_relaxed_sys_2x64(seq->rec_tail, s2, tf);
                ld_relaxed_sys_2x64(seq->rec_head, s3, headv);
                if (s0 == claimed && s1 == claimed && s2 == claimed && s3 == claimed) break;
                if ((++spins & 0x3ffu) == 0 && ld_relaxed_sys(&seq->abort_flag)) { ab = 1; break; }
            }
        }
        ab = __shfl_sync(0xffffffffu, ab, 0);
        if (ab) return 2;
        placed = __shfl_sync(0xffffffffu, placed, 0); end = __shfl_sync(0xffffffffu, end, 0);
        tf = __shfl_sync(0xffffffffu, tf, 0); headv = __shfl_sync(0xffffffffu, headv, 0);
        X.placed = placed; X.end = end; X.tf = tf; X.head = headv; X.have_place = 1; X.next_seq = claimed;
    }
    const bool wrapped = (tf & APUS_REC_WRAPPED) != 0;
    const uint64_t pos0 = (end == L) ? 0 : end;
    const uint64_t used = (end == L) ? 0 : ring_dist(headv, end, L);
    const bool autoprune = (cx->flags & APUS_FLAG_AUTOPRUNE) != 0;
    const uint64_t reserve = autoprune ? APUS_HDR_BYTES : 0;
    if (autoprune && used >= (L >> 1)) return 1;
    if (pos0 + es > L || used + es + reserve >= L) return 1;

    const uint64_t a = pos0, b = pos0 + es;
    const uint64_t ne = (b == L) ? 0 : b;
    const bool nw = wrapped || b == L;
    const uint64_t cum = placed + 1;
    if (lane == 0) {
        st_relaxed_sys_2x64(seq->rec_placed, claimed + 1, cum);
        st_relaxed_sys_2x64(seq->rec_end, claimed + 1, ne);
        st_relaxed_sys_2x64(seq->rec_tail, claimed + 1, a | (nw ? APUS_REC_WRAPPED : 0ull));
        st_relaxed_sys_2x64(seq->rec_head, claimed + 1, headv);
    }
    X.placed = cum; X.end = ne; X.tf = a | (nw ? APUS_REC_WRAPPED : 0ull); X.head = headv; X.have_place = 1;
    const uint64_t idx = S->idx_base + placed + 1;
    const bool xprof = (cx->flags & APUS_FLAG_PROFILE) != 0;
    const uint64_t t_place = xprof ? globaltimer_ns() : 0;

    const uint64_t a16 = a & ~15ull;
    const uint32_t nch = (uint32_t)(((b + 15ull) & ~15ull) - a16) >> 4;
    const uint64_t lo = a16 + 16ull * lane;
    uint4 v = make_uint4(0, 0, 0, 0);
    if ((a & 15ull) == 0) {
        uint4 oldv = make_uint4(0, 0, 0, 0);
        if (wrapped) {
            if (pf_pos == a) oldv = pf;
            else if (lane < (int)nch) oldv = ld_relaxed_sys_v4(entries + lo);
        }
        const int j = lane - 3;
        const int srcl = (j < 0) ? 0 : ((j < 2) ? j + 1 : ((j + 2) & 31));
        uint4 dv;
        dv.x = __shfl_sync(0xffffffffu, sv.x, srcl); dv.y = __shfl_sync(0xffffffffu, sv.y, srcl);
        dv.z = __shfl_sync(0xffffffffu, sv.z, srcl); dv.w = __shfl_sync(0xffffffffu, sv.w, srcl);
        if (lane == 0) v = make_uint4((uint32_t)idx, (uint32_t)(idx >> 32), (uint32_t)cx->term, (uint32_t)(cx->term >> 32));
        else if (lane == 1) v = make_uint4((uint32_t)req_id, (uint32_t)(req_id >> 32), (clt & 0xffffu) | (ty << 16) | ((uint32_t)me << 24), 0u);
        else if (lane == 2) v = make_uint4(0u, 0u, oldv.z & 0xffffff00u, oldv.w);
        else v = chunk_select(dv, oldv, (int)nb - 16 * j);
    } else {
        uint8_t *img = scratch, *xsl = scratch + 256;
        if (lane < (int)nch)
            reinterpret_cast<uint4 *>(img)[lane] = wrapped ? ld_relaxed_sys_v4(entries + lo) : make_uint4(0, 0, 0, 0);
        if (lane == 1 || lane == 2) reinterpret_cast<uint4 *>(xsl)[lane - 1] = sv;
        if (lane >= 4 && lane <= 6) reinterpret_cast<uint4 *>(xsl)[lane - 2] = sv;
        __syncwarp();
        uint8_t *e = img + (a - a16);
        group_write_header(e, lane, 32, idx, cx->term, req_id, clt, ty, me, false);
        group_copy_smem(e + E_DATA, xsl, nb, lane, 32);
        __syncwarp();
        if (lane < (int)nch) v = reinterpret_cast<const uint4 *>(img)[lane];
    }
    const uint64_t t_compose = xprof ? globaltimer_ns() : 0;

    uint64_t cs = 0;
    if (lane < (int)nch) {
        cs = cs_chunk(v, lo, a, b);
        if (lo >= a && lo + 16 <= b) {
            if (cx->mc_region) {
                mst_v4(cx->mc_region + cx->entries_off + lo, v);
            } else {
                st_v4(entries + lo, v);
#pragma unroll 1
                for (int f = 0; f < N; f++)
                    if (S->peer_entries[f]) st_v4(S->peer_entries[f] + lo, v);
            }
        } else {
#pragma unroll 1
            for (uint32_t jb = 0; jb < 16; jb++) {
                const uint64_t o = lo + jb;
                if (o < a || o >= b) continue;
                const uint32_t w = (jb < 4) ? v.x : (jb < 8) ? v.y : (jb < 12) ? v.z : v.w;
                const uint32_t byte = (w >> (8 * (jb & 3))) & 0xff;
                st_u8(entries + o, byte);
#pragma unroll 1
                for (int f = 0; f < N; f++)
                    if (S->peer_entries[f]) st_u8(S->peer_entries[f] + o, byte);
            }
        }
    }
    {
        const uint32_t at = (uint32_t)cum & cx->idx_mask;
        uint32_t *ip = (lane == me) ? lindex : (lane < N ? S->peer_index[lane] : nullptr);
        if (ip) ip[at] = (uint32_t)a;
    }
#pragma unroll
    for (int sft = 16; sft > 0; sft >>= 1) cs += __shfl_xor_sync(0xffffffffu, cs, sft);
    const bool caught = __ballot_sync(0xffffffffu, isf && ackv != placed) == 0;

    const uint64_t t_push = xprof ? globaltimer_ns() : 0;
    uint64_t h = X.pub_h;
    if (!X.hold) {
        uint32_t ab = 0;
        if (lane == 0) {
            uint64_t sq;
            uint32_t spins = 0;
            for (;;) {
                ld_acquire_gpu_2x64(seq->pub_turn, sq, h);
                if (sq == claimed) break;
                if ((++spins & 0x3ffu) == 0 && ld_relaxed_sys(&seq->abort_flag)) { ab = 1; break; }
            }
        }
        ab = __shfl_sync(0xffffffffu, ab, 0);
        if (ab) return 2;
        h = __shfl_sync(0xffffffffu, h, 0);
    }
    if (lane == 0) {
        uint32_t spins = 0;
        while (h - X.pub_tail_seen >= APUS_PUBRING_RECORDS - 2) {
            X.pub_tail_seen = ld_relaxed_sys(&seq->pub_tail);
            if ((++spins & 0x3ffu) == 0 && ld_relaxed_sys(&seq->abort_flag)) break;
        }
    }
    __syncwarp();
    const uint64_t t_turn = xprof ? globaltimer_ns() : 0;
    const uint64_t cumt = cum | ((cx->term & 0xffffull) << APUS_PUB_TERM_SHIFT);
    const bool cert = caught && !(cx->flags & APUS_FLAG_NO_EXPRESS);
    if (isf) {
        apus_ctrl_t *pc = reinterpret_cast<apus_ctrl_t *>(cx->peer[lane]);
        if (cert) {
            st_relaxed_sys_2x64(&pc->pub_csum, cs + cs_key(cumt), a);
            st_relaxed_sys_2x64(&pc->pub_end, ne | APUS_PUB_CERT, cumt);
        } else {
            __threadfence_system();
            st_relaxed_sys_2x64(&pc->pub_end, ne, cumt);
        }
    }
    if (lane >= 16 && lane < 24) {
        const int q = lane - 16;
        const uint64_t val = q == PR_CUM ? cum : q == PR_END ? ne : q == PR_TICKETS ? claimed + 1
                           : q == PR_T0 ? t_deq : q == PR_TAIL ? a : q == PR_HWM ? (nw ? L : b)
                           : q == PR_NEXTIDX ? idx + 1 : (uint64_t)es * (uint64_t)(N - 1);
        st_relaxed_sys_2x64(&pubring[h & PUBMASK].w[2 * q], h + 1, val);
    }
    X.next_seq = claimed + 1; X.pub_h = h + 1;
    if (xprof) {
        const uint64_t t_end = globaltimer_ns();
        X.dt[0] = t_place - t_deq; X.dt[1] = t_compose - t_place; X.dt[2] = t_push - t_compose; X.dt[3] = t_turn - t_push; X.dt[4] = t_end - t_turn;
    }
    if (cert) {
        X.hold = 1;
    } else {
        X.hold = 0;
        __syncwarp();
        if (lane == 0) st_relaxed_sys_2x64(seq->pub_turn, claimed + 1, h + 1);
    }
    return 0;
}

__device__ void leader_main(const apus_devctx_t *__restrict__ cx, const uint32_t wid)
{
    LeaderShared *S = reinterpret_cast<LeaderShared *>(smem_raw);
    uint8_t *slots = smem_raw + L_SLOTS_OFF;
    uint8_t *ext = smem_raw + L_EXT_OFF;
    uint8_t *img = smem_raw + L_IMG_OFF;
    const int tid = threadIdx.x, lane = tid & 31, warp = tid >> 5;
    const int N = cx->group_size, me = cx->idx;
    apus_ctrl_t *ctrl = reinterpret_cast<apus_ctrl_t *>(cx->region);
    apus_seq_t *seq = reinterpret_cast<apus_seq_t *>(cx->region + APUS_SEQ_OFF);
    apus_pubrec_t *pubring = reinterpret_cast<apus_pubrec_t *>(cx->region + APUS_PUBRING_OFF);
    apus_loghdr_t *hdr = reinterpret_cast<apus_loghdr_t *>(cx->region + APUS_HDR_OFF);
    uint8_t *entries = cx->region + cx->entries_off;
    uint32_t *lindex = reinterpret_cast<uint32_t *>(cx->region + APUS_INDEX_OFF);
    apus_hostwords_t *hw = cx->hw;

    if (tid == 0) {
        if (wid == 0) {
            seq->claimed_slots = ctrl->consumed;
            seq->doorbell = ctrl->consumed;
            seq->place_seq = 0; seq->workers_done = 0; seq->abort_flag = 0; seq->w0_idle = 0;
            for (uint32_t i = 0; i < APUS_PUBRING_RECORDS; i++)
                for (int q = 0; q < 8; q++) pubring[i].w[2 * q] = 0;
            seq->rec_placed[0] = ctrl->consumed; seq->rec_placed[1] = ctrl->published;
            seq->rec_end[0] = ctrl->consumed; seq->rec_end[1] = hdr->end;
            seq->rec_tail[0] = ctrl->consumed; seq->rec_tail[1] = hdr->tail | (ctrl->hwm == cx->log_len ? APUS_REC_WRAPPED : 0ull);
            seq->rec_head[0] = ctrl->consumed; seq->rec_head[1] = hdr->head;
            seq->pub_head = 0; seq->pub_tail = 0;
            seq->pub_turn[0] = ctrl->consumed; seq->pub_turn[1] = 0;
            __threadfence();
            st_release_gpu(&seq->ready_epoch, cx->epoch);
        } else {
            while (ld_acquire_gpu(&seq->ready_epoch) != cx->epoch) { }
        }
        S->finish = 0; S->abort = 0; S->was_blocked = 0; S->avg_es = 128; S->avg_xb = 0; S->pub_tail_seen = 0; S->ap_valid = 0;
        S->idx_base = ctrl->next_idx - 1 - ctrl->published;
        for (int i = 0; i < APUS_MAX_SERVERS; i++) {
            S->peer_entries[i] = (i < N && i != me && cx->peer[i]) ? cx->peer[i] + cx->entries_off : nullptr;
            S->peer_index[i] = (i < N && i != me && cx->peer[i]) ? reinterpret_cast<uint32_t *>(cx->peer[i] + APUS_INDEX_OFF) : nullptr;
        }
    }
    __syncthreads();

    if (warp == N_PRODUCER_WARPS) {
        if (wid == 0) leader_commit_warp(cx);
        else if (wid == 1 && cx->doorbell_relay && lane == 0) {
            uint64_t last = ld_relaxed_sys(&seq->doorbell);
            uint32_t spins = 0;
            for (;;) {
                const uint64_t t = ld_acquire_sys(cx->sub_tail);
                if (t != last) { st_release_gpu(&seq->doorbell, t); last = t; }
                if ((++spins & 0x3fu) == 0 &&
                    (ld_relaxed_sys(&seq->abort_flag) || ld_relaxed_sys(&seq->workers_done) >= cx->n_workers)) break;
            }
        }
        return;
    }

    uint64_t last_progress = globaltimer_ns();
    const bool prof = (cx->flags & APUS_FLAG_STATS) != 0 && tid == 0 && wid == 0;
    uint64_t ph[8], tn[8], tprev = globaltimer_ns();
    for (int i = 0; i < 8; i++) { ph[i] = ctrl->phase_ns[i]; tn[i] = ctrl->turn_ns[i]; }
#define PHASE(i) do { if (prof) { const uint64_t _t = globaltimer_ns(); ph[i] += _t - tprev; tprev = _t; } } while (0)
    Express X;
    X.next_seq = 0; X.placed = 0; X.end = 0; X.tf = 0; X.head = 0; X.pub_h = 0; X.have_place = 0; X.hold = 0; X.pub_tail_seen = 0;
    for (int q = 0; q < 5; q++) X.dt[q] = 0;
    uint64_t xguess = ctrl->consumed;
    uint4 pf = make_uint4(0, 0, 0, 0);
    uint64_t pf_pos = ~0ull;

    for (;;) {
        if (warp == 0) {
            uint32_t n = 0, fin = 0, spins = 0, lone_waits = 0;
            const uint64_t tw0 = prof ? globaltimer_ns() : 0;
            uint64_t claimed = 0;
            const bool poll_slot = cx->slot_poll != 0 && wid == 0;
            const bool express_on = (cx->flags & APUS_FLAG_NO_EXPRESS) == 0;
            if (wid == 0 && lane == 0) st_relaxed_sys(&seq->w0_idle, 1);
            for (;;) {
                uint4 sv = make_uint4(0, 0, 0, 0);
                const uint64_t sv_for = xguess;
                if (poll_slot && lane < 8)
                    sv = ld_relaxed_sys_v4(reinterpret_cast<const uint8_t *>(cx->sub_slots + (xguess & cx->sub_mask)) + 16u * lane);
                if (express_on && X.have_place && X.end != cx->log_len && (X.tf & APUS_REC_WRAPPED) && pf_pos != X.end &&
                    (X.end & 15ull) == 0 && X.end + 16ull * 12 <= cx->log_len) {
                    if (lane < 12) pf = ld_relaxed_sys_v4(entries + X.end + 16ull * lane);
                    pf_pos = X.end;
                }
                uint32_t ctl = 0;
                uint64_t t = 0, w0i = 0;
                if (lane == 0) {
                    if ((spins & 0x3fu) == 0 && ld_relaxed_sys(&seq->abort_flag)) ctl = 1;
                    t = cx->doorbell_relay ? ld_relaxed_sys(&seq->doorbell) : ld_relaxed_sys(cx->sub_tail);
                    claimed = ld_relaxed_sys(&seq->claimed_slots);
                    if (claimed >= cx->target) ctl = 1;
                    if (wid != 0) w0i = ld_relaxed_sys(&seq->w0_idle);
                    if (t > claimed) t = cx->doorbell_relay ? ld_acquire_gpu(&seq->doorbell) : ld_acquire_sys(cx->sub_tail);
                }
                ctl = __shfl_sync(0xffffffffu, ctl, 0);
                claimed = __shfl_sync(0xffffffffu, claimed, 0);
                t = __shfl_sync(0xffffffffu, t, 0);
                w0i = __shfl_sync(0xffffffffu, w0i, 0);
                if (X.hold && (ctl || claimed != X.next_seq)) express_release(seq, X, lane);
                if (ctl) { fin = 1; break; }
                bool slot_ok = false;
                if (poll_slot) {
                    const uint64_t stamp = (uint64_t)sv.x | ((uint64_t)sv.y << 32);
                    slot_ok = (__ballot_sync(0xffffffffu, (lane == 3 || lane == 7) && stamp == sv_for + 1) == 0x88u) && sv_for == claimed;
                    xguess = claimed;
                }
                uint64_t avail = t > claimed ? t - claimed : 0;
                if (slot_ok && avail == 0) avail = 1;
                if (poll_slot && express_on && avail == 1 && !slot_ok && ++lone_waits < 8) avail = 0; else lone_waits = 0;
                if (avail == 1 && wid != 0 && w0i) avail = 0;
                if (avail) {
                    const uint64_t room = cx->target - claimed;
                    if (avail > room) avail = room;
                    uint32_t nn = 0, won = 0;
                    if (lane == 0) {
                        uint64_t want = (avail + cx->n_workers - 1) / cx->n_workers;
                        if (want < 32) want = avail < 32 ? avail : 32;
                        uint64_t aes = ld_relaxed_sys(&seq->avg_es), axb = ld_relaxed_sys(&seq->avg_xb);
                        if (aes < 64) aes = 128;
                        uint64_t fit = (APUS_LEADER_IMG_BYTES - 256u) / aes;
                        if (axb) { const uint64_t xf = APUS_LEADER_EXT_BYTES / axb; if (xf < fit) fit = xf; }
                        if (fit < 1) fit = 1;
                        if (want > fit) want = fit;
                        nn = want > MAXB ? MAXB : (uint32_t)want;
                        won = atomicCAS(reinterpret_cast<unsigned long long *>(&seq->claimed_slots), (unsigned long long)claimed,
                                        (unsigned long long)(claimed + nn)) == (unsigned long long)claimed;
                    }
                    nn = __shfl_sync(0xffffffffu, nn, 0);
                    won = __shfl_sync(0xffffffffu, won, 0);
                    if (!won) continue;
                    if (nn == 1 && express_on) {
                        const int rc = leader_express(cx, S, X, claimed, sv, slot_ok, img, lane, pf, pf_pos);
                        if (rc == 0) {
                            xguess = claimed + 1; last_progress = globaltimer_ns();
                            if (prof) { tn[5]++; ph[7]++; for (int q = 0; q < 5; q++) ph[1 + q] += X.dt[q]; }
                            continue;
                        }
                        if (rc == 2) { fin = 1; break; }
                    }
                    n = nn;
                    break;
                }
                if ((++spins & 0x1ffu) == 0) {
                    uint32_t stopf = 0;
                    if (lane == 0) {
                        if (ld_relaxed_sys_u32(&hw->stop)) stopf = 1;
                        else if (cx->target != ~0ull && globaltimer_ns() - last_progress > WATCHDOG_NS) {
                            st_relaxed_sys(&hw->error, APUS_KERR_WATCHDOG_LEADER);
                            st_relaxed_sys(&seq->abort_flag, 1); stopf = 1;
                        }
                        if (prof) for (int i = 0; i < 8; i++) { ctrl->phase_ns[i] = ph[i]; ctrl->turn_ns[i] = tn[i]; }
                    }
                    stopf = __shfl_sync(0xffffffffu, stopf, 0);
                    if (stopf) { fin = 1; break; }
                }
            }
            if (X.hold) express_release(seq, X, lane);
            X.have_place = 0; pf_pos = ~0ull;
            if (lane == 0) {
                if (wid == 0) st_relaxed_sys(&seq->w0_idle, 0);
                if (prof) { tn[0] += globaltimer_ns() - tw0; tn[6]++; }
                if (n) { S->slot0 = claimed; S->my_seq = claimed; }
                S->n_fetch = n; S->finish = fin;
                S->t_dequeue = globaltimer_ns();
            }
        }
        bar_sync(1, NT);
        if (S->finish) break;
        const uint32_t nf = S->n_fetch;
        PHASE(0);

        {
            const uint64_t s0 = S->slot0 & cx->sub_mask;
            const uint64_t nslots = (uint64_t)cx->sub_mask + 1;
            const uint32_t first = (s0 + nf <= nslots) ? nf : (uint32_t)(nslots - s0);
            cta_fetch_slots(S, slots, cx->sub_slots, s0, 0, first, tid);
            if (first < nf) cta_fetch_slots(S, slots, cx->sub_slots, 0, first, nf - first, tid);
        }
        if (tid == 0) S->kbase = 0;
        bar_sync(1, NT);
        PHASE(1);
        if (warp == 1) {
            uint32_t se = 0, sx = 0;
            for (uint32_t k = lane; k < nf; k += 32) { se += S->es[k]; sx += S->xb[k]; }
            for (int sft = 16; sft > 0; sft >>= 1) { se += __shfl_xor_sync(0xffffffffu, se, sft); sx += __shfl_xor_sync(0xffffffffu, sx, sft); }
            if (lane == 0) { st_relaxed_sys(&seq->avg_es, (se + nf - 1) / nf); st_relaxed_sys(&seq->avg_xb, (sx + nf - 1) / nf); }
        }
        const apus_cslot_t *sl = reinterpret_cast<const apus_cslot_t *>(slots);
        bool have_pub_turn = false, have_place_turn = false, aborted = false;
        uint64_t gap_bytes = 0;

        while (S->kbase < nf) {
            if (warp == 0) {
                bool placed_fast = false;
                if (!have_place_turn) {
                    if (nf == 1) {
                        if (lane == 0) {
                            S->cum_es[0] = S->es[0]; S->cum_xb[0] = S->xb[0];
                            S->static_cut = 1; S->first_ext_all = (S->flg[0] & 1u) ? 0u : 0xffffffffu;
                            S->host_head_k = (S->ty[0] == T_HEAD) ? 0u : 0xffffffffu;
                        }
                        S->ap_valid = 0;
                    } else {
                        leader_prescan(cx, S, lane);
                        if (lane == 0) S->ap_valid = 0;
                    }
                    __syncwarp();
                    if (lane == 0) {
                        uint32_t spins = 0;
                        const uint64_t tw0 = prof ? globaltimer_ns() : 0;
                        uint64_t s0, s1, s2, s3, placed, end, tf, headv;
                        for (;;) {
                            ld_relaxed_sys_2x64(seq->rec_placed, s0, placed);
                            ld_relaxed_sys_2x64(seq->rec_end, s1, end);
                            ld_relaxed_sys_2x64(seq->rec_tail, s2, tf);
                            ld_relaxed_sys_2x64(seq->rec_head, s3, headv);
                            if (s0 == S->my_seq && s1 == S->my_seq && s2 == S->my_seq && s3 == S->my_seq) break;
                            if ((++spins & 0x3ffu) == 0 && ld_relaxed_sys(&seq->abort_flag)) { S->abort = 1; break; }
                        }
                        if (prof) { tn[1] += globaltimer_ns() - tw0; S->t_place_acq = globaltimer_ns(); }
                        if (S->abort) { S->fast = 1; S->blocked = 0; goto place_done; }
                        {
                        const uint64_t L = cx->log_len;
                        const bool wrapped = (tf & APUS_REC_WRAPPED) != 0, prevh = (tf & APUS_REC_PREV_HEAD) != 0;
                        const uint64_t tail = tf & ~(APUS_REC_WRAPPED | APUS_REC_PREV_HEAD);
                        S->st_head = headv;
                        const uint64_t pos0 = (end == L) ? 0 : end;
                        const uint64_t used = (end == L) ? 0 : ring_dist(headv, end, L);
                        const uint64_t total = S->cum_es[nf - 1];
                        const bool autoprune = (cx->flags & APUS_FLAG_AUTOPRUNE) != 0;
                        const uint64_t reserve = autoprune ? APUS_HDR_BYTES : 0;
                        bool prune_due = false;
                        if (autoprune && end != L && used >= (L >> 2) && !prevh && L - pos0 >= APUS_HDR_BYTES) {
                            if (!S->ap_valid) {
                                for (int i = 0; i < cx->group_size; i++)
                                    S->ap[i] = (i == me) ? ld_relaxed_sys(&hdr->apply) : ld_relaxed_sys(&ctrl->apply_off[i]);
                                S->ap_valid = 1;
                            }
                            uint64_t d = 0;
                            for (int i = 0; i < cx->group_size; i++) {
                                uint64_t di = ring_dist(S->ap[i], end, L);
                                if (di > used) di = used;
                                d = di > d ? di : d;
                            }
                            if (d == 0) d = ring_dist(tail, end, L);
                            prune_due = (d <= used && used - d >= (L >> 3));
                        }
                        if (!prune_due && pos0 + total <= L &&
                            total <= APUS_LEADER_IMG_BYTES - 16u - (pos0 & 15u) && used + total + reserve < L && S->cum_xb[nf - 1] <= APUS_LEADER_EXT_BYTES && S->static_cut == nf) {
                            const uint64_t b = pos0 + total;
                            const uint64_t ne = (b == L) ? 0 : b;
                            const uint64_t nt = b - S->es[nf - 1];
                            const bool nw = wrapped || b == L;
                            if (S->host_head_k != 0xffffffffu) {
                                const uint64_t nh = adopt_head(headv, slot_head_value(&sl[S->host_head_k]), ne, L);
                                if (nh != headv) { headv = nh; st_relaxed_sys(&hdr->head, nh); }
                            }
                            st_relaxed_sys_2x64(seq->rec_placed, S->my_seq + S->n_fetch, placed + nf);
                            st_relaxed_sys_2x64(seq->rec_end, S->my_seq + S->n_fetch, ne);
                            st_relaxed_sys_2x64(seq->rec_tail, S->my_seq + S->n_fetch, nt | (nw ? APUS_REC_WRAPPED : 0ull));
                            st_relaxed_sys_2x64(seq->rec_head, S->my_seq + S->n_fetch, headv);
                            if (prof) { tn[7] += globaltimer_ns() - S->t_place_acq; tn[3]++; }
                            const uint64_t hwm = wrapped ? L : pos0;
                            S->gap = 0; S->ghost = 0; S->blocked = 0; S->last = 1;
                            S->a = pos0; S->b = b; S->m = nf;
                            S->hbytes = 0; S->base_es = 0; S->base_xb = 0;
                            S->ext_bytes = (S->first_ext_all != 0xffffffffu) ? S->cum_xb[nf - 1] : 0u;
                            S->ext_base = (S->first_ext_all != 0xffffffffu)
                                              ? (uint64_t)(sl[S->first_ext_all].type_off & APUS_SLOT_OFF_MASK) * 16ull : 0ull;
                            S->auto_head = 0; S->auto_head_val = 0;
                            S->idx0 = S->idx_base + placed + 1;
                            S->fresh = (pos0 >= hwm && !wrapped) ? 1u : 0u;
                            S->new_end = ne; S->tail_after = nt; S->cum_after = placed + nf;
                            S->hwm_after = nw ? L : b;
                            S->fast = 1;
                        } else {
                            S->st_end = end; S->st_tail = tail; S->st_placed = placed;
                            S->st_next_idx = S->idx_base + placed + 1;
                            S->st_hwm = wrapped ? L : pos0; S->st_prev_head = prevh ? 1u : 0u;
                            S->fast = 0;
                            if (prof) tn[4]++;
                        }
                        }
                    place_done:;
                    }
                    __syncwarp();
                    placed_fast = S->fast != 0;
                }
                if (!placed_fast) {
                    if (!S->ap_valid) {
                        if (lane < N) S->ap[lane] = (lane == me) ? ld_relaxed_sys(&hdr->apply) : ld_relaxed_sys(&ctrl->apply_off[lane]);
                        __syncwarp();
                        if (lane == 0) S->ap_valid = 1;
                        __syncwarp();
                    }
                    leader_place(cx, S, sl, lane);
                    if (lane == 0 && S->last) {
                        st_relaxed_sys_2x64(seq->rec_placed, S->my_seq + S->n_fetch, S->st_placed);
                        st_relaxed_sys_2x64(seq->rec_end, S->my_seq + S->n_fetch, S->st_end);
                        st_relaxed_sys_2x64(seq->rec_tail, S->my_seq + S->n_fetch, S->st_tail | (S->st_hwm == cx->log_len ? APUS_REC_WRAPPED : 0ull) |
                                                                              (S->st_prev_head ? APUS_REC_PREV_HEAD : 0ull));
                        st_relaxed_sys_2x64(seq->rec_head, S->my_seq + S->n_fetch, S->st_head);
                        if (prof) tn[7] += globaltimer_ns() - S->t_place_acq;
                    }
                }
            }
            have_place_turn = true;
            bar_sync(1, NT);
            PHASE(2);
            if (S->abort) { aborted = true; break; }
            if (S->blocked) {
                if (tid == 0) {
                    if (ld_relaxed_sys_u32(&hw->stop) || ld_relaxed_sys(&seq->abort_flag)) { st_relaxed_sys(&seq->abort_flag, 1); S->finish = 1; }
                    else if (cx->target != ~0ull && globaltimer_ns() - last_progress > WATCHDOG_NS) {
                        st_relaxed_sys(&hw->error, APUS_KERR_WATCHDOG_LEADER);
                        st_relaxed_sys(&seq->abort_flag, 1); S->finish = 1;
                    }
                }
                if (tid < N) S->ap[tid] = (tid == me) ? ld_relaxed_sys(&hdr->apply) : ld_relaxed_sys(&ctrl->apply_off[tid]);
                bar_sync(1, NT);
                if (S->finish) { aborted = true; break; }
                continue;
            }
            const uint32_t kbase = S->kbase, m = S->m, gap = S->gap, autoh = S->auto_head;
            const uint64_t a = S->a, b = S->b;
            const uint64_t a16 = a & ~15ull;
            const uint32_t nchunks = (uint32_t)(((b + 15ull) & ~15ull) - a16) >> 4;

            const bool holes_only = !gap && (b - a) >= (uint64_t)(m + autoh) * 512ull;
            if (holes_only) {
                for (uint32_t j = tid; j < m + autoh; j += NT) {
                    uint32_t rel, es_, nb_;
                    if (autoh && j == 0) { rel = 0; es_ = APUS_HDR_BYTES; nb_ = 8; }
                    else {
                        const uint32_t k = kbase + j - autoh;
                        rel = S->hbytes + (S->cum_es[k] - S->base_es) - S->es[k];
                        es_ = S->es[k]; nb_ = data_bytes(S->ty[k], sl[k].len);
                    }
                    const uint64_t eo = a + rel;
                    const uint64_t h0 = eo + 41, h1 = eo + 47, g0 = eo + 48 + nb_, g1 = eo + es_ - 1;
                    const uint64_t cs[4] = { h0 >> 4, h1 >> 4, g0 >> 4, g1 >> 4 };
#pragma unroll
                    for (int q = 0; q < 4; q++) {
                        if (q == 3 && g1 < g0) continue;
                        if (q == 2 && g1 < g0) continue;
                        if (q > 0 && cs[q] == cs[q - 1]) continue;
                        const uint64_t lo = cs[q] << 4;
                        if (lo < a16 || lo >= a16 + 16ull * nchunks) continue;
                        reinterpret_cast<uint4 *>(img)[(lo - a16) >> 4] =
                            S->fresh ? make_uint4(0, 0, 0, 0) : ld_relaxed_sys_v4(entries + lo);
                    }
                }
            } else if (S->fresh) {
                for (uint32_t c = tid; c < nchunks; c += NT) reinterpret_cast<uint4 *>(img)[c] = make_uint4(0, 0, 0, 0);
            } else {
                cta_fetch_chunks(img, entries + a16, nchunks, tid);
            }
            if (!gap && S->ext_bytes) cta_fetch_chunks(ext, cx->sub_pay + S->ext_base, S->ext_bytes >> 4, tid);
            for (uint32_t j = tid; j < m; j += NT) {
                const uint32_t k = kbase + j;
                S->rel[k] = S->hbytes + (S->cum_es[k] - S->base_es) - S->es[k];
                S->xoff[k] = (S->cum_xb[k] - S->base_xb) - S->xb[k];
            }
            bar_sync(1, NT);
            PHASE(3);

            if (gap) {
                if (S->ghost && warp == 0) {
                    uint8_t *e = img + (a - a16);
                    group_write_header(e, lane, 32, S->idx0, cx->term, sl[kbase].req_id, sl[kbase].clt_id, S->ty[kbase], 0, true);
                    if (lane == 8) { e[E_DATA] = (uint8_t)(sl[kbase].len & 0xff); e[E_DATA + 1] = (uint8_t)(sl[kbase].len >> 8); }
                }
            } else {
                if (autoh && warp == N_PRODUCER_WARPS - 1) {
                    uint8_t *e = img + (a - a16);
                    group_write_header(e, lane, 32, S->idx0, cx->term, 0, 0, T_HEAD, me, false);
                    if (lane >= 8 && lane < 16) e[E_DATA + lane - 8] = (uint8_t)(S->auto_head_val >> (8 * (lane - 8)));
                }
                const bool small = (b - a) <= (uint64_t)(m + autoh) * 256ull;
                const int gl = small ? 8 : 32;
                const int grp = small ? (lane >> 3) : 0, sub = small ? (lane & 7) : lane;
                const uint32_t per_step = small ? 4u * N_PRODUCER_WARPS : N_PRODUCER_WARPS;
                for (uint32_t j = (small ? warp * 4u + grp : warp); j < m; j += per_step) {
                    const uint32_t k = kbase + j;
                    uint8_t *e = img + (a - a16) + S->rel[k];
                    const uint32_t ty = S->ty[k];
                    const uint32_t nb = data_bytes(ty, sl[k].len);
                    const uint32_t es_k = S->es[k];
                    if (((uint32_t)(uintptr_t)e & 15u) == 0 && (es_k & 15u) == 0) {
                        const uint64_t idx = S->idx0 + autoh + j, rq = sl[k].req_id;
                        const uint8_t *src = (S->flg[k] & 1u) ? ext + S->xoff[k] : sl[k].inl;
                        const uint32_t nch_e = es_k >> 4;
                        for (uint32_t c = (uint32_t)sub; c < nch_e; c += (uint32_t)gl) {
                            uint4 *dst = reinterpret_cast<uint4 *>(e) + c;
                            if (c == 0) *dst = make_uint4((uint32_t)idx, (uint32_t)(idx >> 32), (uint32_t)cx->term, (uint32_t)(cx->term >> 32));
                            else if (c == 1) *dst = make_uint4((uint32_t)rq, (uint32_t)(rq >> 32),
                                                               ((uint32_t)sl[k].clt_id) | (ty << 16) | ((uint32_t)me << 24), 0u);
                            else if (c == 2) { const uint4 o = *dst; *dst = make_uint4(0u, 0u, o.z & 0xffffff00u, o.w); }
                            else {
                                const int nbv = (int)nb - 16 * (int)(c - 3);
                                if (nbv >= 16) *dst = *reinterpret_cast<const uint4 *>(src + 16u * (c - 3));
                                else if (nbv > 0) *dst = chunk_select(*reinterpret_cast<const uint4 *>(src + 16u * (c - 3)), *dst, nbv);
                            }
                        }
                    } else {
                        group_write_header(e, sub, gl, S->idx0 + autoh + j, cx->term, sl[k].req_id, sl[k].clt_id, ty, me, false);
                        if (nb) group_copy_smem(e + E_DATA, (S->flg[k] & 1u) ? ext + S->xoff[k] : sl[k].inl, nb, sub, gl);
                    }
                }
            }
            bar_sync(1, NT);
            PHASE(4);

            uint8_t *mc_entries = cx->mc_region ? cx->mc_region + cx->entries_off : nullptr;
            for (uint32_t c = tid; c < nchunks; c += NT) {
                const uint64_t lo = a16 + 16ull * c;
                const uint4 v = reinterpret_cast<const uint4 *>(img)[c];
                if (lo >= a && lo + 16 <= b) {
                    if (mc_entries) {
                        mst_v4(mc_entries + lo, v);
                    } else {
                        st_v4(entries + lo, v);
#pragma unroll 1
                        for (int f = 0; f < N; f++)
                            if (S->peer_entries[f]) st_v4(S->peer_entries[f] + lo, v);
                    }
                } else {
#pragma unroll 1
                    for (uint32_t j = 0; j < 16; j++) {
                        const uint64_t o = lo + j;
                        if (o < a || o >= b) continue;
                        const uint32_t w = (j < 4) ? v.x : (j < 8) ? v.y : (j < 12) ? v.z : v.w;
                        const uint32_t byte = (w >> (8 * (j & 3))) & 0xff;
                        st_u8(entries + o, byte);
#pragma unroll 1
                        for (int f = 0; f < N; f++)
                            if (S->peer_entries[f]) st_u8(S->peer_entries[f] + o, byte);
                    }
                }
            }
            if (!gap) {
                const uint64_t cum0 = S->cum_after - (m + autoh);
                for (uint32_t j = tid; j < m + autoh; j += NT) {
                    uint32_t w;
                    if (autoh && j == 0) w = (uint32_t)a | APUS_IDX_HEAD_FLAG;
                    else {
                        const uint32_t k = kbase + j - autoh;
                        w = (uint32_t)(a + S->rel[k]) | (S->ty[k] == T_HEAD ? APUS_IDX_HEAD_FLAG : 0u);
                    }
                    const uint32_t at = (uint32_t)(cum0 + 1 + j) & cx->idx_mask;
                    if (cx->mc_region) {
                        mst_u32(reinterpret_cast<uint32_t *>(cx->mc_region + APUS_INDEX_OFF) + at, w);
                    } else {
                        lindex[at] = w;
#pragma unroll 1
                        for (int f = 0; f < N; f++)
                            if (S->peer_index[f]) S->peer_index[f][at] = w;
                    }
                }
            }
            bar_sync(1, NT);
            PHASE(5);

            if (gap) {
                gap_bytes += b - a;
                bar_sync(1, NT);
                continue;
            }
            if (warp == 0) {
                const bool pubs = lane < N && lane != me && cx->peer[lane];
                if (pubs) __threadfence_system();
                if (lane == 0) {
                    if (!have_pub_turn) {
                        uint32_t spins = 0;
                        const uint64_t tw0 = prof ? globaltimer_ns() : 0;
                        uint64_t sq, h;
                        for (;;) {
                            ld_acquire_gpu_2x64(seq->pub_turn, sq, h);
                            if (sq == S->my_seq) break;
                            if ((++spins & 0x3ffu) == 0 && ld_relaxed_sys(&seq->abort_flag)) { S->abort = 1; break; }
                        }
                        if (prof) tn[2] += globaltimer_ns() - tw0;
                        S->pub_h = h;
                    }
                    uint32_t spins = 0;
                    while (!S->abort && S->pub_h - S->pub_tail_seen >= APUS_PUBRING_RECORDS - 2) {
                        S->pub_tail_seen = ld_relaxed_sys(&seq->pub_tail);
                        if ((++spins & 0x3ffu) == 0 && ld_relaxed_sys(&seq->abort_flag)) { S->abort = 1; break; }
                    }
                }
                __syncwarp();
                const bool pub_ok = S->abort == 0;
                if (pubs && pub_ok) {
                    apus_ctrl_t *pc = reinterpret_cast<apus_ctrl_t *>(cx->peer[lane]);
                    st_relaxed_sys_2x64(&pc->pub_end, S->new_end, S->cum_after | ((cx->term & 0xffffull) << APUS_PUB_TERM_SHIFT));
                }
                if (pub_ok && lane >= 16 && lane < 24) {
                    const int q = lane - 16;
                    const uint64_t h = S->pub_h;
                    const uint64_t val = q == PR_CUM ? S->cum_after : q == PR_END ? S->new_end : q == PR_TICKETS ? S->slot0 + kbase + m
                                       : q == PR_T0 ? S->t_dequeue : q == PR_TAIL ? S->tail_after : q == PR_HWM ? S->hwm_after
                                       : q == PR_NEXTIDX ? S->idx0 + m + autoh : (b - a + gap_bytes) * (uint64_t)(N - 1);
                    st_relaxed_sys_2x64(&pubring[h & PUBMASK].w[2 * q], h + 1, val);
                }
                __syncwarp();
                if (lane == 0 && pub_ok) {
                    S->pub_h += 1;
                    if (S->last) st_relaxed_sys_2x64(seq->pub_turn, S->my_seq + S->n_fetch, S->pub_h);
                    S->kbase = kbase + m;
                }
            }
            have_pub_turn = true;
            gap_bytes = 0;
            last_progress = globaltimer_ns();
            bar_sync(1, NT);
            if (S->abort) { aborted = true; break; }
            if (prof) {
                PHASE(6); ph[7]++;
                for (int i = 0; i < 8; i++) { ctrl->phase_ns[i] = ph[i]; ctrl->turn_ns[i] = tn[i]; }
            }
        }
        if (aborted) break;
    }
    if (prof) for (int i = 0; i < 8; i++) { ctrl->phase_ns[i] = ph[i]; ctrl->turn_ns[i] = tn[i]; }
    if (tid == 0) { __threadfence(); atomicAdd(reinterpret_cast<unsigned long long *>(&seq->workers_done), 1ull); }
}

__device__ void follower_main(const apus_devctx_t *__restrict__ cx)
{
    FollowerShared *S = reinterpret_cast<FollowerShared *>(smem_raw);
    uint8_t *win = smem_raw + FS_BYTES;
    const int tid = threadIdx.x, nthr = blockDim.x;
    const int me = cx->idx, ldr = cx->leader_idx;
    apus_ctrl_t *ctrl = reinterpret_cast<apus_ctrl_t *>(cx->region);
    apus_loghdr_t *hdr = reinterpret_cast<apus_loghdr_t *>(cx->region + APUS_HDR_OFF);
    uint8_t *entries = cx->region + cx->entries_off;
    apus_hostwords_t *hw = cx->hw;
    uint8_t *lregion = cx->peer[ldr];
    apus_ctrl_t *lctrl = reinterpret_cast<apus_ctrl_t *>(lregion);
    uint8_t *lentries = lregion + cx->entries_off;
    const uint64_t L = cx->log_len;
    const bool fenced = (cx->flags & APUS_FLAG_FENCED_ACK) != 0;
    const bool walk = (cx->flags & APUS_FLAG_WALK) != 0;
    const uint32_t *index = reinterpret_cast<const uint32_t *>(cx->region + APUS_INDEX_OFF);

    uint64_t old_end = hdr->old_end;
    uint64_t acked = ctrl->acked;
    uint64_t applied = hdr->apply;
    uint64_t pend_val = ctrl->pend_head_val, pend_end = ctrl->pend_head_end;
    uint64_t last_progress = globaltimer_ns();
    uint32_t spins = 0;

    const uint64_t myterm16 = cx->term & 0xffffull;
    const bool host_apply = (cx->flags & APUS_FLAG_HOST_APPLY) != 0;
    uint64_t host_applied = hdr->apply;
    uint64_t last_hb = ld_relaxed_sys(&ctrl->hb), last_hb_t = globaltimer_ns();
    bool suspected = false;
    const bool fstat = (cx->flags & APUS_FLAG_PROFILE) != 0;
    uint64_t cert_first_cum = 0, cert_first_t = 0, fbeat = globaltimer_ns() >> 8;

    for (;;) {
        if (tid < 32) {
            const int lane = tid;
            uint64_t e = 0, cumt = 0, c = 0, cert_start = 0;
            uint32_t done = 0, is_cert = 0;
            for (;;) {
                uint64_t x0 = 0, x1 = 0;
                const uint64_t spec_a = (old_end == L) ? 0 : old_end;
                const uint64_t spec_lo = (spec_a & ~15ull) + 16ull * (uint64_t)(lane - 4);
                uint4 spec = make_uint4(0, 0, 0, 0);
                if (lane == 0) ld_acquire_sys_2x64(&ctrl->pub_end, x0, x1);
                else if (lane == 1) ld_relaxed_sys_2x64(&ctrl->pub_csum, x0, x1);
                else if (lane == 2) x0 = ld_relaxed_sys(&hdr->commit);
                else if (lane == 3) x0 = ld_relaxed_sys(&ctrl->hb);
                else if (lane < 16 && spec_lo + 16 <= L) spec = ld_relaxed_sys_v4(entries + spec_lo);
                e = __shfl_sync(0xffffffffu, x0, 0); cumt = __shfl_sync(0xffffffffu, x1, 0);
                const uint64_t csum = __shfl_sync(0xffffffffu, x0, 1);
                cert_start = __shfl_sync(0xffffffffu, x1, 1);
                c = __shfl_sync(0xffffffffu, x0, 2);
                const uint64_t hbw = __shfl_sync(0xffffffffu, x0, 3);
                uint64_t cum = cumt & APUS_PUB_CUM_MASK;
                if ((cumt >> APUS_PUB_TERM_SHIFT) != myterm16) cum = 0;
                is_cert = (e & APUS_PUB_CERT) ? 1u : 0u;
                e &= ~APUS_PUB_CERT;
                bool new_entries = cum > acked;
                if (new_entries && is_cert && fstat && cum != cert_first_cum) { cert_first_cum = cum; cert_first_t = globaltimer_ns(); }
                if (new_entries && is_cert) {
                    const uint64_t a = cert_start, b = (e == 0) ? L : e;
                    bool ok = cum == acked + 1 && a == ((old_end == L) ? 0 : old_end) && b > a && b - a <= 32u * 16u - 16u;
                    if (ok) {
                        const uint64_t a16 = a & ~15ull;
                        const uint32_t nch = (uint32_t)(((b + 15ull) & ~15ull) - a16) >> 4;
                        uint64_t cs = 0;
                        if (nch <= 12) {
                            if (lane >= 4 && lane < 4 + (int)nch) cs = cs_chunk(spec, spec_lo, a, b);
                        } else if (lane < (int)nch) cs = cs_chunk(ld_relaxed_sys_v4(entries + a16 + 16ull * lane), a16 + 16ull * lane, a, b);
#pragma unroll
                        for (int sft = 16; sft > 0; sft >>= 1) cs += __shfl_xor_sync(0xffffffffu, cs, sft);
                        ok = (cs + cs_key(cumt)) == csum;
                    }
                    if (fstat && lane == 0) { if (ok) { ctrl->phase_ns[0]++; ctrl->phase_ns[1] += globaltimer_ns() - cert_first_t; } else ctrl->phase_ns[2]++; }
                    if (!ok) { new_entries = false; cum = acked; }
                }
                const bool new_commit = (c != applied) && (old_end != L) && (applied != old_end);
                if (new_entries || new_commit) { cumt = cum; break; }
                if (cx->target != ~0ull) {
                    uint64_t ft = 0;
                    if (lane == 0) ft = ld_acquire_sys(&ctrl->fin_target);
                    ft = __shfl_sync(0xffffffffu, ft, 0);
                    if (ft == cx->target) {
                        const uint64_t fe = ld_relaxed_sys(&ctrl->fin_entries);
                        if (acked >= fe && (old_end == L || (applied == old_end && c == old_end))) { done = 1; cumt = acked; break; }
                    }
                }
                if (hbw != last_hb) { last_hb = hbw; last_hb_t = globaltimer_ns(); if (lane == 0) st_relaxed_sys(&hw->hb_seen, hbw); }
                if ((++spins & 0xffu) == 0) {
                    uint32_t stopf = 0;
                    uint64_t ha = host_applied;
                    if (lane == 0) {
                        if (ld_relaxed_sys_u32(&hw->stop)) stopf = 1;
                        else if (cx->target != ~0ull && globaltimer_ns() - last_progress > WATCHDOG_NS) {
                            st_relaxed_sys(&hw->error, APUS_KERR_WATCHDOG_FOLLOWER);
                            stopf = 1;
                        }
                        if (cx->hb_timeout_ns && !suspected && globaltimer_ns() - last_hb_t > cx->hb_timeout_ns)
                            st_relaxed_sys(&hw->leader_suspect, 1 + cx->term);
                        if (host_apply) ha = ld_relaxed_sys(&hw->host_apply);
                    }
                    if (cx->hb_timeout_ns && globaltimer_ns() - last_hb_t > cx->hb_timeout_ns) suspected = true;
                    if (lane == 0) st_relaxed_sys(&lctrl->fbeat[me], ++fbeat);
                    stopf = __shfl_sync(0xffffffffu, stopf, 0);
                    ha = __shfl_sync(0xffffffffu, ha, 0);
                    if (host_apply && ha != host_applied) {
                        host_applied = ha;
                        if (lane == 0) { hdr->apply = ha; st_relaxed_sys(&lctrl->apply_off[me], ha); }
                    }
                    if (stopf) { done = 1; cumt = acked; break; }
                }
            }
            if (lane == 0) {
                if (!done && !fenced && cumt > acked) st_relaxed_sys(&lctrl->ack[me], cumt);
                S->end_seen = e; S->cum_seen = cumt; S->commit_seen = c; S->done = done;
                S->cert = (cumt > acked) ? is_cert : 0u; S->cert_start = cert_start;
            }
        }
        __syncthreads();
        if (S->done) break;
        const uint64_t end_seen = S->end_seen, cum_seen = S->cum_seen, commit_seen = S->commit_seen;

        if (cum_seen > acked && !walk) {
            const uint64_t n = cum_seen - acked;
            if (tid == 0) S->head_j = 0;
            __syncthreads();
            for (uint64_t j = tid; j < n; j += nthr) {
                const uint32_t w = S->cert ? (uint32_t)S->cert_start : ld_relaxed_sys_u32(&index[(uint32_t)(acked + 1 + j) & cx->idx_mask]);
                const uint64_t at = (uint64_t)(w & ~APUS_IDX_HEAD_FLAG) + E_REPLY + (uint64_t)me;
                st_relaxed_sys_u8(entries + at, 1);
                st_relaxed_sys_u8(lentries + at, 1);
                if (w & APUS_IDX_HEAD_FLAG) atomicMax(&S->head_j, (uint32_t)(j + 1));
            }
            __syncthreads();
            if (S->head_j) {
                const uint32_t w = ld_relaxed_sys_u32(&index[(uint32_t)(acked + S->head_j) & cx->idx_mask]);
                const uint64_t off = (uint64_t)(w & ~APUS_IDX_HEAD_FLAG);
                pend_val = ld_relaxed_sys(entries + ((off + E_DATA) & ~7ull));
                if ((off + E_DATA) & 7ull) {
                    uint64_t hv = 0;
                    for (int q = 7; q >= 0; q--) hv = (hv << 8) | (uint64_t)(ld_relaxed_sys_u32(entries + ((off + E_DATA + q) & ~3ull)) >> (8 * ((off + E_DATA + q) & 3ull)) & 0xffu);
                    pend_val = hv;
                }
                pend_end = (off + APUS_HDR_BYTES == L) ? 0 : off + APUS_HDR_BYTES;
            }
            acked = cum_seen;
            old_end = end_seen;
            if (tid == 0) {
                if (fenced) {
                    __threadfence_system();
                    st_relaxed_sys(&lctrl->ack[me], acked);
                }
                hdr->end = end_seen; hdr->old_end = old_end;
                ctrl->acked = acked;
                ctrl->pend_head_val = pend_val; ctrl->pend_head_end = pend_end;
            }
            last_progress = globaltimer_ns();
        } else if (cum_seen > acked) {
            uint64_t walked = 0;
            while (old_end != end_seen) {
                if (tid == 0) {
                    uint64_t lo = (old_end == L) ? 0 : old_end;
                    if (L - lo < APUS_HDR_BYTES) lo = 0;
                    uint64_t hi = (end_seen > lo) ? end_seen : L;
                    if (lo == end_seen) hi = lo;
                    if (hi - (lo & ~15ull) > APUS_FOLLOWER_WIN_BYTES) hi = (lo & ~15ull) + APUS_FOLLOWER_WIN_BYTES;
                    S->win_lo = lo; S->win_hi = hi;
                }
                __syncthreads();
                const uint64_t lo = S->win_lo, hi = S->win_hi;
                if (lo == hi) { old_end = lo; break; }
                const uint64_t lo16 = lo & ~15ull;
                const uint32_t nch = (uint32_t)(((hi + 15ull) & ~15ull) - lo16) >> 4;
                {
                    uint32_t c = tid;
                    const uint8_t *src = entries + lo16;
                    for (; c + 3u * nthr < nch; c += 4u * nthr) {
                        const uint4 v0 = ld_relaxed_sys_v4(src + 16ull * c);
                        const uint4 v1 = ld_relaxed_sys_v4(src + 16ull * (c + nthr));
                        const uint4 v2 = ld_relaxed_sys_v4(src + 16ull * (c + 2u * nthr));
                        const uint4 v3 = ld_relaxed_sys_v4(src + 16ull * (c + 3u * nthr));
                        reinterpret_cast<uint4 *>(win)[c] = v0;
                        reinterpret_cast<uint4 *>(win)[c + nthr] = v1;
                        reinterpret_cast<uint4 *>(win)[c + 2u * nthr] = v2;
                        reinterpret_cast<uint4 *>(win)[c + 3u * nthr] = v3;
                    }
                    for (; c < nch; c += nthr) reinterpret_cast<uint4 *>(win)[c] = ld_relaxed_sys_v4(src + 16ull * c);
                }
                __syncthreads();
                if (tid == 0) {
                    uint64_t off = lo;
                    uint32_t n = 0;
                    uint64_t next = off;
                    bool wrapped = false;
                    uint64_t hv = 0, he = L;
                    while (off < hi) {
                        if (L - off < APUS_HDR_BYTES) { next = 0; wrapped = true; break; }
                        if (hi - off < APUS_HDR_BYTES) { next = off; break; }
                        const uint8_t *e = win + (off - lo16);
                        const uint32_t ty = e[E_TYPE];
                        const uint32_t ln = (uint32_t)e[E_DATA] | ((uint32_t)e[E_DATA + 1] << 8);
                        const uint32_t es = entry_stride(ty, ln);
                        if (L - off < es) { next = 0; wrapped = true; break; }
                        if (off + es > hi) { next = off; break; }
                        if (ty == T_HEAD) {
                            hv = 0;
                            for (int q = 7; q >= 0; q--) hv = (hv << 8) | e[E_DATA + q];
                            he = (off + es == L) ? 0 : off + es;
                        }
                        S->off[n++] = (uint32_t)(off - lo);
                        off += es;
                        next = off;
                    }
                    if (!wrapped && next == L) next = 0;
                    S->n = n; S->next = next;
                    S->head_val = hv; S->head_end = he;
                }
                __syncthreads();
                const uint32_t n = S->n;
                for (uint32_t k = tid; k < n; k += nthr) {
                    const uint64_t at = lo + S->off[k] + E_REPLY + (uint64_t)me;
                    st_relaxed_sys_u8(entries + at, 1);
                    st_relaxed_sys_u8(lentries + at, 1);
                }
                __syncthreads();
                const uint64_t next = S->next;
                if (n == 0 && next == old_end) {
                    if (tid == 0) st_relaxed_sys(&hw->error, APUS_KERR_BAD_ENTRY);
                    old_end = end_seen;
                    break;
                }
                if (S->head_end != L) { pend_val = S->head_val; pend_end = S->head_end; }
                walked += n;
                old_end = next;
            }
            if (acked + walked != cum_seen && tid == 0) st_relaxed_sys(&hw->error, APUS_KERR_COUNT_MISMATCH);
            acked = cum_seen;
            if (tid == 0) {
                if (fenced) {
                    __threadfence_system();
                    st_relaxed_sys(&lctrl->ack[me], acked);
                }
                hdr->end = end_seen; hdr->old_end = old_end;
                ctrl->acked = acked;
                ctrl->pend_head_val = pend_val; ctrl->pend_head_end = pend_end;
            }
            last_progress = globaltimer_ns();
        }

        if (old_end != L && applied != old_end && commit_seen != applied) {
            const uint64_t from = applied;
            const uint64_t held = ring_dist(from, old_end, L);
            uint64_t want = ring_dist(from, commit_seen, L);
            uint64_t to = commit_seen;
            if (want > held) { want = held; to = old_end; }
            if (want) {
                if (pend_end != L) {
                    const uint64_t dh = ring_dist(from, pend_end, L);
                    if (dh > 0 && dh <= want) {
                        if (tid == 0) { hdr->head = pend_val; ctrl->pend_head_end = L; }
                        pend_end = L;
                    }
                }
                applied = to;
                if (tid == 0) {
                    if (!host_apply) {
                        hdr->apply = applied;
                        st_relaxed_sys(&lctrl->apply_off[me], applied);
                    }
                    st_relaxed_sys_2x64(&hw->commit_off, applied, acked);
                }
                last_progress = globaltimer_ns();
            }
        }
        __syncthreads();
    }
}

extern "C" __global__ void __launch_bounds__(APUS_KERNEL_THREADS, 1)
apus_replica_kernel(const apus_role_t *__restrict__ roles)
{
    const apus_role_t r = roles[blockIdx.x];
    if (r.kind == APUS_ROLE_LEADER) leader_main(r.ctx, r.worker);
    else if (r.kind == APUS_ROLE_FOLLOWER) follower_main(r.ctx);
}

extern "C" size_t apus_kernel_smem_bytes(void)
{
    size_t a = L_TOTAL, b = F_TOTAL;
    return a > b ? a : b;
}

extern "C" cudaError_t apus_launch_roles(const apus_role_t *d_roles, int n_roles, cudaStream_t stream)
{
    static bool attr_set[64] = {false};
    int dev = 0;
    cudaGetDevice(&dev);
    const size_t smem = apus_kernel_smem_bytes();
    if (dev < 64 && !attr_set[dev]) {
        cudaError_t e = cudaFuncSetAttribute(apus_replica_kernel, cudaFuncAttributeMaxDynamicSharedMemorySize, (int)smem);
// ... 7 lines not shown
```

### apus_b200/csrc/apus_layout.h

```cpp
#ifndef APUS_LAYOUT_H
#define APUS_LAYOUT_H

#include <stdint.h>

#define APUS_MAX_SERVERS      13
#define APUS_HDR_BYTES        64u
#define APUS_CTRL_BYTES       4096u
#define APUS_LOGHDR_REF_BYTES 319656u
#define APUS_LOGHDR_BYTES     (320u * 1024u)
#define APUS_SEQ_OFF          4096u
#define APUS_PUBRING_OFF      8192u
#define APUS_PUBRING_RECORDS  256u
#define APUS_HDR_OFF          65536u
#define APUS_INDEX_OFF        (APUS_HDR_OFF + APUS_LOGHDR_BYTES)
#define APUS_IDX_HEAD_FLAG    0x80000000u

#define E_IDX     0
#define E_TERM    8
#define E_REQID  16
#define E_CLTID  24
#define E_TYPE   26
#define E_SENDER 27
#define E_REPLY  28
#define E_DATA   48
#define E_CMD    50

#define T_NOOP   0
#define T_CONFIG 2
#define T_HEAD   3

typedef struct apus_loghdr {
    uint64_t head, apply, commit, end, tail, old_end, old_commit, len;
} apus_loghdr_t;

#define APUS_PUB_RING 1024u
#define APUS_LAT_RING 65536u

typedef struct apus_ctrl {
    uint64_t ack[16];
    uint64_t apply_off[16];
    uint64_t fbeat[16];
    uint64_t next_idx;
    uint64_t consumed;
    uint64_t published;
    uint64_t committed;
    uint64_t committed_tickets;
    uint64_t hwm;
    uint64_t bytes_replicated;
    uint64_t batches;
    uint64_t acked;
    uint64_t lat_count;
    uint64_t auto_heads;
    uint64_t pend_head_val;
    uint64_t pend_head_end;
    uint64_t pad0[3];
    uint64_t fin_entries;
    uint64_t fin_target;
    uint64_t pad1[14];
    uint64_t pub_end;
    uint64_t pub_cum;
    uint64_t pub_csum;
    uint64_t pub_start;
    uint64_t pad2[4];
    uint64_t hb;
    uint64_t pad3[7];
    uint64_t phase_ns[8];
    uint64_t turn_ns[8];
} apus_ctrl_t;

#define APUS_CTL_OFF 1024u
typedef struct apus_vote_req {
    uint64_t sid, index, term;
    uint64_t cid[2];
    uint64_t pad[3];
} apus_vote_req_t;
typedef struct apus_ctlwords {
    uint64_t sid;
    uint64_t leader_sid;
    uint64_t adj_end;
    uint64_t adj_count;
    uint64_t pad[4];
    uint64_t vote_ack[16];
    apus_vote_req_t vote_req[APUS_MAX_SERVERS];
} apus_ctlwords_t;

typedef struct apus_seq {
    uint64_t claimed_slots;
    uint64_t pad_c[15];
    uint64_t place_seq;      uint64_t pad_d[15];
    uint64_t pub_turn[2];    uint64_t pad_e[14];
    uint64_t pub_head;       uint64_t pad_f[15];
    uint64_t pub_tail;       uint64_t pad_g[15];
    uint64_t workers_done;
    uint64_t abort_flag;
    uint64_t ready_epoch;
    uint64_t pad_h[13];
    uint64_t rec_placed[2];
    uint64_t rec_end[2];
    uint64_t rec_tail[2];
    uint64_t rec_head[2];
    uint64_t avg_es, avg_xb;
    uint64_t doorbell;
    uint64_t w0_idle;
    uint64_t pad_i[4];
} apus_seq_t;
#define APUS_REC_PREV_HEAD (1ull << 62)
#define APUS_REC_WRAPPED   (1ull << 63)

#define PR_CUM     0
#define PR_END     1
#define PR_TICKETS 2
#define PR_T0      3
#define PR_TAIL    4
#define PR_HWM     5
#define PR_NEXTIDX 6
#define PR_BYTES   7
typedef struct apus_pubrec {
    uint64_t w[16];
} apus_pubrec_t;

#define APUS_SLOT_BYTES   128u
#define APUS_SLOT_INLINE  80u
#define APUS_CSLOT_BYTES  96u
#define APUS_SLOT_OFF_MASK 0x00ffffffu
#define APUS_SLOT_TYPE_SHIFT 24
#define APUS_SLOT_TYPE_MASK 0x1fu
#define APUS_SLOT_EXT   (1u << 29)
#define APUS_SLOT_WRAP  (1u << 30)
typedef struct apus_slot {
    uint64_t req_id;
    uint32_t type_off;
    uint16_t len;
    uint16_t clt_id;
    uint8_t  inl0[32];
    uint64_t stamp0, rsv0;
    uint8_t  inl1[48];
    uint64_t stamp1, rsv1;
} apus_slot_t;
typedef struct apus_cslot {
    uint64_t req_id;
    uint32_t type_off;
    uint16_t len;
    uint16_t clt_id;
    uint8_t  inl[APUS_SLOT_INLINE];
} apus_cslot_t;

typedef struct apus_hostwords {
    volatile uint64_t sub_tail;
    uint64_t pad0[15];
    volatile uint64_t commit_off;
    volatile uint64_t committed_tickets;
    volatile uint64_t consumed;
    volatile uint64_t last_commit_ns;
    uint64_t pad1[12];
    volatile uint32_t stop;
    uint32_t pad2[31];
    volatile uint64_t host_apply;
    uint64_t pad3[15];
    volatile uint64_t heartbeat;
    volatile uint64_t error;
    volatile uint64_t leader_suspect;
    volatile uint64_t hb_seen;
} apus_hostwords_t;

#define APUS_FLAG_FENCED_ACK 0x1u
#define APUS_FLAG_STATS      0x2u
#define APUS_FLAG_AUTOPRUNE  0x4u
#define APUS_FLAG_WALK       0x8u
#define APUS_FLAG_HOST_APPLY 0x10u
#define APUS_FLAG_NO_EXPRESS 0x20u
#define APUS_FLAG_PROFILE    0x40u

#define APUS_PUB_CERT      (1ull << 63)
#define APUS_PUB_TERM_SHIFT 48
#define APUS_PUB_CUM_MASK  ((1ull << 48) - 1)

#define APUS_ROLE_NONE     0
#define APUS_ROLE_LEADER   1
#define APUS_ROLE_FOLLOWER 2

typedef struct apus_devctx {
    uint8_t  idx, group_size, leader_idx, quorum;
    uint32_t flags;
    uint64_t term;
    uint64_t log_len;
    uint64_t entries_off;
    uint32_t idx_mask;
    uint32_t pad_i;
    uint64_t target;
    uint32_t n_workers;
    uint32_t doorbell_relay;
    uint32_t slot_poll;
    uint32_t epoch;
    uint64_t hb_period_ns;
    uint64_t hb_timeout_ns;
    uint8_t *region;
    uint8_t *mc_region;
    uint8_t *peer[APUS_MAX_SERVERS];
    const apus_slot_t *sub_slots;
    const uint8_t     *sub_pay;
    uint32_t           sub_mask;
    uint32_t           pad;
    const volatile uint64_t *sub_tail;
    apus_hostwords_t  *hw;
    uint32_t          *lat_ns;
} apus_devctx_t;

typedef struct apus_role {
    uint32_t       kind;
    uint32_t       worker;
    apus_devctx_t *ctx;
} apus_role_t;

#define APUS_KERNEL_THREADS    512
#define APUS_MAX_TILE_ENTRIES  256u
#define APUS_LEADER_IMG_BYTES  (80u * 1024u)
#define APUS_LEADER_EXT_BYTES  (66u * 1024u)
#define APUS_FOLLOWER_WIN_BYTES (96u * 1024u)

#endif
```

### apus_b200/engine.py

```python
import ctypes as C
import os

import numpy as np

HERE = os.path.dirname(os.path.abspath(__file__))
LIB_PATH = os.path.join(HERE, "libapus_gpu.so")

APUS_OK, APUS_ERROR, APUS_RETRY = 0, 1, -1
NOOP, CSM, CONFIG, HEAD, CONNECT, SEND, CLOSE = 0, 1, 2, 3, 4, 5, 6
RING_HOST_MAPPED, RING_DEVICE = 0, 1
LOG_SIZE = 16384 * 4096
MAX_SERVERS = 13
F_FENCED_ACK, F_DEVICE_STATS, F_AUTOPRUNE, F_FOLLOWER_WALK, F_EXPLICIT = 0x1, 0x2, 0x4, 0x8, 0x80000000
F_HOST_APPLY, F_NO_EXPRESS, F_PROFILE, F_FABRIC = 0x10, 0x20, 0x40, 0x100
UINT64_MAX = (1 << 64) - 1

u64, u32, u16, u8, i64, i32 = C.c_uint64, C.c_uint32, C.c_uint16, C.c_uint8, C.c_int64, C.c_int32


class ApusError(RuntimeError):
    pass


class Config(C.Structure):
    _fields_ = [("struct_size", u32), ("device", i32), ("server_idx", u8), ("group_size", u8),
                ("leader_idx", u8), ("ring_mode", u8), ("flags", u32), ("term", u64),
                ("log_size", u64), ("ring_slots", u32), ("ring_bytes", u32), ("leader_ctas", u32), ("reserved", u32),
                ("hb_period_us", u32), ("hb_timeout_us", u32)]


class PeerHandle(C.Structure):
    _fields_ = [("bytes", u8 * 128)]


class LogOffsets(C.Structure):
    _fields_ = [(k, u64) for k in ("head", "apply", "commit", "end", "tail", "old_end", "old_commit", "len")]


class Stats(C.Structure):
    _fields_ = [(k, u64) for k in ("tickets_submitted", "tickets_consumed", "tickets_committed",
                                   "entries_acked", "bytes_replicated", "batches", "kernel_launches",
                                   "lat_samples", "auto_heads", "entries_published")] + [("phase_ns", u64 * 8), ("turn_ns", u64 * 8)]


_lib = None

EXPORTS = [
    "apus_abi_version", "apus_last_error", "apus_device_count", "apus_replica_create",
    "apus_replica_destroy", "apus_replica_export", "apus_replica_connect", "apus_replicas_launch",
    "apus_replica_wait", "apus_replica_last_launch_ms", "apus_replicas_stop", "apus_submit",
    "apus_submit_batch", "apus_submit_defer", "apus_submit_flush", "apus_committed_tickets",
    "apus_progress", "apus_wait_committed", "apus_closed_loop", "apus_log_offsets", "apus_log_read", "apus_get_stats",
    "apus_latency_samples", "apus_set_head", "apus_remote_apply_offsets",
    "apus_submit_uniform", "apus_submit_synth", "apus_synth_byte", "apus_submit_release", "apus_set_applied",
    "apus_log_read_range", "apus_leader_suspect", "apus_last_commit_ns",
    "apus_ctl_read", "apus_ctl_set_sid", "apus_ctl_reset_votes", "apus_ctl_clear_vote_request", "apus_ctl_send_vote_request",
    "apus_ctl_send_vote_ack", "apus_ctl_last_entry", "apus_ctl_adjust_follower", "apus_replica_set_role",
    "apus_replica_disconnect", "apus_follower_beats", "apus_device_numa_node", "apus_group_multicast", "apus_ctl_heartbeat",
]


def load_library(path=LIB_PATH):
    global _lib
    if _lib is not None:
        return _lib
    if not os.path.exists(path):
        raise ApusError(f"{path} not built: run `python -c 'import __graft_entry__ as g; g.build()'` "
                        "(make -C apus_b200/csrc). There is no CPU fallback.")
    L = C.CDLL(path)
    vp = C.c_void_p
    L.apus_abi_version.restype = C.c_int
    L.apus_last_error.restype = C.c_char_p
    L.apus_device_count.restype = C.c_int
    L.apus_replica_create.argtypes = [C.POINTER(Config), C.POINTER(vp)]
    L.apus_replica_destroy.argtypes = [vp]
    L.apus_replica_destroy.restype = None
    L.apus_replica_export.argtypes = [vp, C.POINTER(PeerHandle)]
    L.apus_replica_connect.argtypes = [vp, u8, C.POINTER(PeerHandle)]
    L.apus_replicas_launch.argtypes = [C.POINTER(vp), C.c_int, u64]
    L.apus_replica_wait.argtypes = [vp, i64]
    L.apus_replica_last_launch_ms.argtypes = [vp, C.POINTER(C.c_float)]
    L.apus_replicas_stop.argtypes = [C.POINTER(vp), C.c_int]
    L.apus_submit.argtypes = [vp, u8, u16, u64, vp, u16, C.POINTER(u64)]
    L.apus_submit_batch.argtypes = [vp, u32, vp, vp, vp, vp, vp, C.c_size_t, C.POINTER(u64)]
    L.apus_submit_defer.argtypes = [vp, C.c_int]
    L.apus_submit_flush.argtypes = [vp]
    L.apus_committed_tickets.argtypes = [vp]
    L.apus_committed_tickets.restype = u64
    L.apus_wait_committed.argtypes = [vp, u64, i64]
    L.apus_closed_loop.argtypes = [vp, u32, u16, u16, u64, vp]
    L.apus_progress.argtypes = [vp, C.POINTER(u64), C.POINTER(u64)]
    L.apus_log_offsets.argtypes = [vp, C.POINTER(LogOffsets)]
    L.apus_log_read.argtypes = [vp, u64, u64, vp]
    L.apus_get_stats.argtypes = [vp, C.POINTER(Stats)]
    L.apus_latency_samples.argtypes = [vp, vp, u32, C.POINTER(u32)]
    L.apus_set_head.argtypes = [vp, u64]
    L.apus_remote_apply_offsets.argtypes = [vp, C.POINTER(u64)]
    if hasattr(L, "apus_submit_uniform"):
        L.apus_submit_uniform.argtypes = [vp, u32, u8, u16, u64, u16, vp, C.c_size_t, C.POINTER(u64)]
        L.apus_submit_synth.argtypes = [vp, u32, u8, u16, u64, u16, u32, C.POINTER(u64)]
        L.apus_synth_byte.argtypes = [u32, u64, u32]
        L.apus_synth_byte.restype = u8
        L.apus_submit_release.argtypes = [vp, u64]
        L.apus_set_applied.argtypes = [vp, u64]
        L.apus_log_read_range.argtypes = [vp, u64, u64, vp, u64, C.POINTER(u64)]
        L.apus_leader_suspect.argtypes = [vp]
        L.apus_leader_suspect.restype = u64
        L.apus_last_commit_ns.argtypes = [vp]
        L.apus_last_commit_ns.restype = u64
    _lib = L
    return L


def lib():
    return load_library()


def _ck(rc, what):
    if rc == APUS_OK:
        return
    msg = lib().apus_last_error().decode(errors="replace")
    if rc == APUS_RETRY:
        raise BlockingIOError(f"{what}: {msg}")
    raise ApusError(f"{what}: {msg}")


class Replica:
    def __init__(self, device, server_idx, group_size, leader_idx=0, term=1, log_size=0,
                 ring_mode=RING_HOST_MAPPED, ring_slots=0, ring_bytes=0, flags=None, leader_ctas=0,
                 hb_period_us=0, hb_timeout_us=0):
        cfg = Config()
        cfg.leader_ctas = leader_ctas
        cfg.hb_period_us, cfg.hb_timeout_us = hb_period_us, hb_timeout_us
        cfg.struct_size = C.sizeof(Config) if lib().apus_abi_version() >= 2 else 48
        cfg.device, cfg.server_idx, cfg.group_size, cfg.leader_idx = device, server_idx, group_size, leader_idx
        cfg.ring_mode, cfg.term, cfg.log_size = ring_mode, term, log_size
        cfg.ring_slots, cfg.ring_bytes = ring_slots, ring_bytes
        cfg.flags = 0 if flags is None else (flags | F_EXPLICIT)
        self.h = C.c_void_p()
        _ck(lib().apus_replica_create(C.byref(cfg), C.byref(self.h)), "apus_replica_create")
        self.cfg = cfg
        self.device, self.idx, self.n, self.leader = device, server_idx, group_size, leader_idx
        self.log_len = log_size or LOG_SIZE

    @property
    def is_leader(self):
        return self.idx == self.leader

    def close(self):
        if self.h:
            lib().apus_replica_destroy(self.h)
            self.h = C.c_void_p()

    def export(self) -> bytes:
        ph = PeerHandle()
        _ck(lib().apus_replica_export(self.h, C.byref(ph)), "apus_replica_export")
        return bytes(ph.bytes)

    def connect(self, peer_idx, blob: bytes):
        ph = PeerHandle()
        C.memmove(ph.bytes, blob, 128)
        _ck(lib().apus_replica_connect(self.h, peer_idx, C.byref(ph)), "apus_replica_connect")

    def wait(self, timeout_ms=-1):
        _ck(lib().apus_replica_wait(self.h, timeout_ms), "apus_replica_wait")

    def last_launch_ms(self):
        ms = C.c_float()
        _ck(lib().apus_replica_last_launch_ms(self.h, C.byref(ms)), "apus_replica_last_launch_ms")
        return float(ms.value)

    def submit(self, typ, conn, req_id, payload=b""):
        t = u64()
        buf = (u8 * max(len(payload), 1)).from_buffer_copy(bytes(payload) or b"\0")
        _ck(lib().apus_submit(self.h, typ, conn, req_id, C.cast(buf, C.c_void_p), len(payload), C.byref(t)),
            "apus_submit")
        return int(t.value)

    def submit_batch(self, types, conns, req_ids, lens, payloads, stride):
        n = len(types)
        types = np.ascontiguousarray(types, dtype=np.uint8)
        conns = np.ascontiguousarray(conns, dtype=np.uint16)
        req_ids = np.ascontiguousarray(req_ids, dtype=np.uint64)
        lens = np.ascontiguousarray(lens, dtype=np.uint16)
        pp = None
        if payloads is not None:
            payloads = np.ascontiguousarray(payloads, dtype=np.uint8)
            pp = payloads.ctypes.data
        t = u64()
        _ck(lib().apus_submit_batch(self.h, n, types.ctypes.data, conns.ctypes.data, req_ids.ctypes.data,
                                    lens.ctypes.data, pp, stride, C.byref(t)), "apus_submit_batch")
        return int(t.value)

    def submit_uniform(self, n, typ, conn, first_req_id, length, payloads, stride=None):
        pp = None
        if payloads is not None and length:
            payloads = np.ascontiguousarray(payloads, dtype=np.uint8)
            pp = payloads.ctypes.data
        t = u64()
        _ck(lib().apus_submit_uniform(self.h, n, typ, conn, first_req_id, length, pp, length if stride is None else stride,
                                      C.byref(t)), "apus_submit_uniform")
        return int(t.value)

    def submit_synth(self, n, typ, conn, first_req_id, length, seed):
        t = u64()
        _ck(lib().apus_submit_synth(self.h, n, typ, conn, first_req_id, length, seed, C.byref(t)), "apus_submit_synth")
        return int(t.value)

    def release(self, ticket):
        _ck(lib().apus_submit_release(self.h, ticket), "apus_submit_release")

    def set_applied(self, offset):
        _ck(lib().apus_set_applied(self.h, offset), "apus_set_applied")

    def read_range(self, start, stop, cap=1 << 20):
        out = np.empty(cap, dtype=np.uint8)
        got = u64()
        _ck(lib().apus_log_read_range(self.h, start, stop, out.ctypes.data, cap, C.byref(got)), "apus_log_read_range")
        return out[: got.value].copy()

    def leader_suspect(self):
        return int(lib().apus_leader_suspect(self.h))

    def last_commit_ns(self):
        return int(lib().apus_last_commit_ns(self.h))

    def defer(self, on=True):
        _ck(lib().apus_submit_defer(self.h, 1 if on else 0), "apus_submit_defer")

    def flush(self):
        _ck(lib().apus_submit_flush(self.h), "apus_submit_flush")

    def committed(self):
        return int(lib().apus_committed_tickets(self.h))

    def progress(self):
        off, cnt = u64(), u64()
        _ck(lib().apus_progress(self.h, C.byref(off), C.byref(cnt)), "apus_progress")
        return int(off.value), int(cnt.value)

    def wait_committed(self, ticket, timeout_us=10_000_000):
        _ck(lib().apus_wait_committed(self.h, ticket, timeout_us), "apus_wait_committed")

    def closed_loop(self, n, payload_len, conn, first_req_id):
        out = np.empty(n, dtype=np.uint32)
        _ck(lib().apus_closed_loop(self.h, n, payload_len, conn, first_req_id, out.ctypes.data), "apus_closed_loop")
        return out

    def offsets(self):
        o = LogOffsets()
        _ck(lib().apus_log_offsets(self.h, C.byref(o)), "apus_log_offsets")
        return {k: int(getattr(o, k)) for k, _ in LogOffsets._fields_}

    def image(self, start=0, stop=None):
        stop = self.log_len if stop is None else stop
        out = np.empty(stop - start, dtype=np.uint8)
        if stop > start:
            _ck(lib().apus_log_read(self.h, start, stop - start, out.ctypes.data), "apus_log_read")
        return out

    def stats(self):
        s = Stats()
        _ck(lib().apus_get_stats(self.h, C.byref(s)), "apus_get_stats")
        d = {k: int(getattr(s, k)) for k, _ in Stats._fields_ if k not in ("phase_ns", "turn_ns")}
        d["phase_ns"] = [int(x) for x in s.phase_ns]
        d["turn_ns"] = [int(x) for x in s.turn_ns]
        return d

    def latency_ns(self, max_samples=65536):
        out = np.empty(max_samples, dtype=np.uint32)
        n = u32()
        _ck(lib().apus_latency_samples(self.h, out.ctypes.data, max_samples, C.byref(n)), "apus_latency_samples")
        return out[: n.value].copy()

    def set_head(self, head):
        _ck(lib().apus_set_head(self.h, head), "apus_set_head")

    def remote_apply_offsets(self):
        arr = (u64 * MAX_SERVERS)()
        _ck(lib().apus_remote_apply_offsets(self.h, arr), "apus_remote_apply_offsets")
        return [int(x) for x in arr]


def synth_payload(seed: int, req_id: int, length: int) -> bytes:
    if length == 0:
        return b""
    w = np.arange((length + 3) // 4, dtype=np.uint64)
    x = (np.uint64(seed) ^ np.uint64((req_id * 0x9E3779B1) & 0xFFFFFFFF) ^ np.uint64(((req_id >> 32) * 0x7F4A7C15) & 0xFFFFFFFF)
         ^ ((w * np.uint64(0x85EBCA77)) & np.uint64(0xFFFFFFFF)))
    M = np.uint64(0xFFFFFFFF)
    x ^= x >> np.uint64(16); x = (x * np.uint64(0x7FEB352D)) & M
    x ^= x >> np.uint64(15); x = (x * np.uint64(0x846CA68B)) & M
    x ^= x >> np.uint64(16)
    return x.astype(np.uint32).view(np.uint8)[:length].tobytes()


def pin_to_device_node(device: int):
    try:
        lib().apus_device_numa_node.argtypes = [C.c_int]
        node = int(lib().apus_device_numa_node(device))
        if node < 0:
            return None
        cpus = set()
        for part in open(f"/sys/devices/system/node/node{node}/cpulist").read().strip().split(","):
            a, _, b = part.partition("-")
            cpus.update(range(int(a), int(b or a) + 1))
        cpus &= os.sched_getaffinity(0)
        if cpus:
            os.sched_setaffinity(0, cpus)
            return node
    except Exception:
        pass
    return None


def cid_image(n: int) -> bytes:
    return (0).to_bytes(8, "little") + bytes([n, 0, 0, 0]) + ((1 << n) - 1).to_bytes(4, "little")


class Group:

    def __init__(self, n, devices=None, leader=0, term=1, log_size=0, ring_mode=RING_HOST_MAPPED,
                 ring_slots=0, ring_bytes=0, flags=None, leader_ctas=0, hb_period_us=0, hb_timeout_us=0):
        ndev = lib().apus_device_count()
        if ndev <= 0:
            raise ApusError("no CUDA device visible: the engine has no CPU fallback")
        if devices is None:
            devices = [i % ndev for i in range(n)]
        self.n, self.leader_idx, self.devices = n, leader, list(devices)
        self.replicas = [Replica(devices[i], i, n, leader, term, log_size, ring_mode, ring_slots, ring_bytes, flags,
                                 leader_ctas, hb_period_us, hb_timeout_us) for i in range(n)]
        blobs = [r.export() for r in self.replicas]
        for r in self.replicas:
            for j, b in enumerate(blobs):
                if j != r.idx:
                    r.connect(j, b)
        self.tickets = 0

    @property
    def leader(self) -> Replica:
        return self.replicas[self.leader_idx]

    def close(self):
        for r in self.replicas:
            r.close()

    def __enter__(self):
        return self

    def __exit__(self, *a):
        try:
            self.stop()
        except Exception:
            pass
        self.close()

    def launch(self, target=None):
        target = self.tickets if target is None else target
        by_dev = {}
        for r in self.replicas:
            by_dev.setdefault(r.device, []).append(r)
        for dev, rs in sorted(by_dev.items(), key=lambda kv: any(r.is_leader for r in kv[1])):
            arr = (C.c_void_p * len(rs))(*[r.h for r in rs])
            _ck(lib().apus_replicas_launch(arr, len(rs), target), "apus_replicas_launch")

    def wait(self, timeout_ms=60_000):
        for r in self.replicas:
            r.wait(timeout_ms)

    def stop(self):
        arr = (C.c_void_p * self.n)(*[r.h for r in self.replicas])
        _ck(lib().apus_replicas_stop(arr, self.n), "apus_replicas_stop")

    def multicast(self):
        arr = (C.c_void_p * self.n)(*[r.h for r in self.replicas])
        lib().apus_group_multicast.argtypes = [C.POINTER(C.c_void_p), C.c_int]
        _ck(lib().apus_group_multicast(arr, self.n), "apus_group_multicast")

    def prologue(self):
        if self.n == 1:
            return 0
        self.tickets = self.leader.submit(CONFIG, 0, 0, cid_image(self.n))
        return self.tickets

    def submit(self, typ, conn, req_id, payload=b""):
        self.tickets = self.leader.submit(typ, conn, req_id, payload)
        return self.tickets

    def submit_stream(self, stream):
        self.leader.defer(True)
        try:
            for typ, conn, rid, payload in stream:
                self.tickets = self.leader.submit(typ, conn, rid, payload)
        finally:
            self.leader.flush()
            self.leader.defer(False)
        return self.tickets

    def submit_uniform(self, n_req, length, conn, first_req_id, payloads=None, typ=SEND):
        types = np.full(n_req, typ, dtype=np.uint8)
        conns = np.full(n_req, conn, dtype=np.uint16)
        req_ids = np.arange(first_req_id, first_req_id + n_req, dtype=np.uint64)
        lens = np.full(n_req, length, dtype=np.uint16)
        t0 = self.leader.submit_batch(types, conns, req_ids, lens, payloads, length)
        self.tickets = t0 + n_req - 1
        return self.tickets

    def run(self, timeout_ms=60_000):
        self.launch()
        self.wait(timeout_ms)
```

### include/apus_gpu.h

```cpp
#ifndef APUS_GPU_H
#define APUS_GPU_H

#include <stddef.h>
#include <stdint.h>

#ifdef __cplusplus
extern "C" {
#endif

#define APUS_ABI_VERSION 2

#define APUS_OK       0
#define APUS_ERROR    1
#define APUS_RETRY  (-1)

#define APUS_MAX_SERVER_COUNT 13
#define APUS_LOG_SIZE (16384ull * 4096ull)
#define APUS_ENTRY_HDR 64u

#define APUS_NOOP    0
#define APUS_CSM     1
#define APUS_CONFIG  2
#define APUS_HEAD    3
#define APUS_CONNECT 4
#define APUS_SEND    5
#define APUS_CLOSE   6

#define APUS_RING_HOST_MAPPED 0
#define APUS_RING_DEVICE      1

#define APUS_F_FENCED_ACK   0x1u
#define APUS_F_DEVICE_STATS 0x2u
#define APUS_F_AUTOPRUNE    0x4u
#define APUS_F_FOLLOWER_WALK 0x8u
#define APUS_F_HOST_APPLY   0x10u
#define APUS_F_NO_EXPRESS   0x20u
#define APUS_F_FABRIC      0x100u
#define APUS_F_PROFILE      0x40u
#define APUS_F_EXPLICIT     0x80000000u

typedef struct apus_replica apus_replica_t;

typedef struct apus_config {
    uint32_t struct_size;
    int32_t  device;
    uint8_t  server_idx;
    uint8_t  group_size;
    uint8_t  leader_idx;
    uint8_t  ring_mode;
    uint32_t flags;
    uint64_t term;
    uint64_t log_size;
    uint32_t ring_slots;
    uint32_t ring_bytes;
    uint32_t leader_ctas;
    uint32_t reserved;
    uint32_t hb_period_us;
    uint32_t hb_timeout_us;
} apus_config_t;
#define APUS_CONFIG_SIZE_V1 48u

typedef struct apus_peer_handle {
    uint8_t bytes[128];
} apus_peer_handle_t;

typedef struct apus_log_offsets {
    uint64_t head, apply, commit, end, tail, old_end, old_commit, len;
} apus_log_offsets_t;

typedef struct apus_stats {
    uint64_t tickets_submitted;
    uint64_t tickets_consumed;
    uint64_t tickets_committed;
    uint64_t entries_acked;
    uint64_t bytes_replicated;
    uint64_t batches;
    uint64_t kernel_launches;
    uint64_t lat_samples;
    uint64_t auto_heads;
    uint64_t entries_published;
    uint64_t phase_ns[8];
    uint64_t turn_ns[8];
} apus_stats_t;

int         apus_abi_version(void);
const char *apus_last_error(void);
int         apus_device_count(void);
int         apus_device_numa_node(int device);

int  apus_replica_create(const apus_config_t *cfg, apus_replica_t **out);
void apus_replica_destroy(apus_replica_t *r);

int  apus_replica_export(apus_replica_t *r, apus_peer_handle_t *out);
int  apus_replica_connect(apus_replica_t *r, uint8_t peer_idx, const apus_peer_handle_t *peer);

int  apus_group_multicast(apus_replica_t **rs, int n);

int  apus_replicas_launch(apus_replica_t **rs, int n, uint64_t target_tickets);
int  apus_replica_wait(apus_replica_t *r, int64_t timeout_ms);
int  apus_replica_last_launch_ms(apus_replica_t *r, float *ms);
int  apus_replicas_stop(apus_replica_t **rs, int n);

int  apus_submit(apus_replica_t *leader, uint8_t type, uint16_t connection_id, uint64_t req_id,
                 const void *cmd, uint16_t len, uint64_t *ticket);
int  apus_submit_batch(apus_replica_t *leader, uint32_t n, const uint8_t *types,
                       const uint16_t *connection_ids, const uint64_t *req_ids,
                       const uint16_t *lens, const void *payloads, size_t stride,
                       uint64_t *first_ticket);
int  apus_submit_uniform(apus_replica_t *leader, uint32_t n, uint8_t type, uint16_t connection_id,
                         uint64_t first_req_id, uint16_t len, const void *payloads, size_t stride,
                         uint64_t *first_ticket);
int  apus_submit_synth(apus_replica_t *leader, uint32_t n, uint8_t type, uint16_t connection_id,
                       uint64_t first_req_id, uint16_t len, uint32_t seed, uint64_t *first_ticket);
uint8_t apus_synth_byte(uint32_t seed, uint64_t req_id, uint32_t k);
int  apus_submit_defer(apus_replica_t *leader, int defer);
int  apus_submit_flush(apus_replica_t *leader);
int  apus_submit_release(apus_replica_t *leader, uint64_t ticket);

uint64_t apus_committed_tickets(apus_replica_t *leader);
int  apus_progress(apus_replica_t *r, uint64_t *offset, uint64_t *count);
int  apus_wait_committed(apus_replica_t *leader, uint64_t ticket, int64_t timeout_us);

int  apus_closed_loop(apus_replica_t *leader, uint32_t n, uint16_t payload_len, uint16_t connection_id,
                      uint64_t first_req_id, uint32_t *lat_ns);

int  apus_log_offsets(apus_replica_t *r, apus_log_offsets_t *out);
int  apus_log_read(apus_replica_t *r, uint64_t off, uint64_t len, void *dst);
int  apus_get_stats(apus_replica_t *r, apus_stats_t *out);
int  apus_latency_samples(apus_replica_t *r, uint32_t *dst_ns, uint32_t max, uint32_t *n);

int  apus_set_applied(apus_replica_t *r, uint64_t offset);
int  apus_log_read_range(apus_replica_t *r, uint64_t from, uint64_t to, void *dst, uint64_t cap, uint64_t *got);
uint64_t apus_leader_suspect(apus_replica_t *follower);
uint64_t apus_last_commit_ns(apus_replica_t *leader);

typedef struct apus_ctl_view {
    uint64_t sid, leader_sid, adj_end, adj_count;
    uint64_t vote_ack[APUS_MAX_SERVER_COUNT];
    struct { uint64_t sid, index, term, cid[2]; } vote_req[APUS_MAX_SERVER_COUNT];
} apus_ctl_view_t;
int  apus_ctl_read(apus_replica_t *r, apus_ctl_view_t *out);
int  apus_ctl_set_sid(apus_replica_t *r, uint64_t sid);
int  apus_ctl_reset_votes(apus_replica_t *r);
int  apus_ctl_clear_vote_request(apus_replica_t *r, uint8_t from_idx);
int  apus_ctl_send_vote_request(apus_replica_t *r, uint8_t peer_idx, uint64_t sid, uint64_t index, uint64_t term,
                                const void *cid16);
int  apus_ctl_send_vote_ack(apus_replica_t *r, uint8_t candidate_idx, uint64_t commit);
int  apus_ctl_heartbeat(apus_replica_t *r, uint64_t *word);
int  apus_ctl_last_entry(apus_replica_t *r, uint64_t *idx, uint64_t *term, uint64_t *commit, uint64_t *end);
int  apus_ctl_adjust_follower(apus_replica_t *leader, uint8_t peer_idx, uint64_t sid, uint64_t *resent);
int  apus_replica_set_role(apus_replica_t *r, uint8_t leader_idx, uint64_t term);
int  apus_follower_beats(apus_replica_t *leader, uint64_t out[APUS_MAX_SERVER_COUNT]);
int  apus_replica_disconnect(apus_replica_t *r, uint8_t peer_idx);

int  apus_set_head(apus_replica_t *r, uint64_t head);
int  apus_remote_apply_offsets(apus_replica_t *leader, uint64_t out[APUS_MAX_SERVER_COUNT]);

#ifdef __cplusplus
}
#endif
#endif
```

Baseline: 133.0 million.

## Replace serialized publish turn with placement-carried ring slot and commit-warp pushes

Workers no longer spin on a global pub_turn token before writing their publish-ring record. The ring slot index is now carried along with the placement sequence (rec_pubh). Publishing pub_end to peers for non-certified batches moves from each worker to the commit warp, which gates on a pub_fenced watermark advanced via atomicMax after a gpu-scope fence. The commit warp also reads up to eight ring records per iteration and adds per-worker profiling rows. This is meant to remove serialization between workers at the publish stage, at the cost of more complex ordering reasoning and extra work in the commit loop.

```diff
diff --git a/apus_b200/csrc/apus_engine.cu b/apus_b200/csrc/apus_engine.cu
--- a/apus_b200/csrc/apus_engine.cu
+++ b/apus_b200/csrc/apus_engine.cu
@@ -15,6 +15,11 @@
 #include "apus_layout.h"
 
 extern "C" cudaError_t apus_launch_roles(const apus_role_t *d_roles, int n_roles, cudaStream_t stream);
+
+static_assert(sizeof(apus_ctrl_t) <= APUS_CTL_OFF, "ctrl words overlap the control-plane words");
+static_assert(APUS_CTL_OFF + sizeof(apus_ctlwords_t) <= APUS_WSTAT_OFF, "control-plane words overlap the profiling rows");
+static_assert(APUS_WSTAT_OFF + (APUS_WSTAT_ROWS + 1) * APUS_WSTAT_WORDS * sizeof(uint64_t) <= APUS_CTRL_BYTES,
+              "profiling rows do not fit the ctrl block");
 extern "C" size_t apus_kernel_smem_bytes(void);
 
 #define MAX_ROLES 160
@@ -1054,6 +1059,18 @@
     return APUS_OK;
 }
 
+extern "C" int apus_worker_stats(apus_replica_t *r, uint64_t *dst, uint32_t rows)
+{
+    if (!r || !dst) return fail("null argument");
+    const uint32_t all = APUS_WSTAT_ROWS + 1;
+    if (rows > all) rows = all;
+    DeviceGuard g(r->cfg.device);
+    CK(cudaMemcpyAsync(dst, r->region + APUS_WSTAT_OFF, (size_t)rows * APUS_WSTAT_WORDS * sizeof(uint64_t),
+                       cudaMemcpyDeviceToHost, r->copy_stream));
+    CK(cudaStreamSynchronize(r->copy_stream));
+    return APUS_OK;
+}
+
 extern "C" int apus_latency_samples(apus_replica_t *r, uint32_t *dst, uint32_t max, uint32_t *n)
 {
     if (!r || !dst || !n) return fail("null argument");
diff --git a/apus_b200/csrc/apus_kernels.cu b/apus_b200/csrc/apus_kernels.cu
--- a/apus_b200/csrc/apus_kernels.cu
+++ b/apus_b200/csrc/apus_kernels.cu
@@ -153,6 +153,7 @@
     uint64_t ext_base, auto_head_val, a, b, idx0, cum_after, new_end, tail_after, hwm_after;
     uint8_t  *peer_entries[APUS_MAX_SERVERS];
     uint32_t *peer_index[APUS_MAX_SERVERS];
+    uint64_t prof_ph[8], prof_tn[8];
 };
 
 #define LS_BYTES ((sizeof(LeaderShared) + 127u) & ~127u)
@@ -186,6 +187,10 @@
 __device__ __forceinline__ void ld_acquire_gpu_2x64(const volatile void *p, uint64_t &a, uint64_t &b)
 {
     asm volatile("ld.acquire.gpu.global.v2.u64 {%0,%1}, [%2];" : "=l"(a), "=l"(b) : "l"(p) : "memory");
+}
+__device__ __forceinline__ void fence_acq_rel_gpu()
+{
+    asm volatile("fence.acq_rel.gpu;" ::: "memory");
 }
 __device__ __forceinline__ void st_release_gpu(volatile void *p, uint64_t v)
 {
@@ -359,24 +364,70 @@
     uint64_t last_hb = 0, hb_beat = globaltimer_ns() >> 10;
     bool S_rec_ok = false;
     volatile uint64_t *peer_commit = nullptr;
-    if (lane < N && lane != me && cx->peer[lane])
+    apus_ctrl_t *peer_ctrl = nullptr;
+    if (lane < N && lane != me && cx->peer[lane]) {
         peer_commit = &reinterpret_cast<apus_loghdr_t *>(cx->peer[lane] + APUS_HDR_OFF)->commit;
+        peer_ctrl = reinterpret_cast<apus_ctrl_t *>(cx->peer[lane]);
+    }
+    bool pend = false;
+    uint64_t pend_end = 0, pend_cumt = 0;
+    uint64_t self_hi = 0;
+    uint64_t need_fenced = 0;
+    uint64_t fenced_seen = 0;
+    const uint64_t term16 = (cx->term & 0xffffull) << APUS_PUB_TERM_SHIFT;
+    const bool cstat = (cx->flags & APUS_FLAG_STATS) != 0;
+    uint64_t *crow = reinterpret_cast<uint64_t *>(cx->region + APUS_WSTAT_OFF) + (size_t)APUS_WSTAT_ROWS * APUS_WSTAT_WORDS;
+    uint64_t cs_loops = crow[CS_LOOPS], cs_batches = crow[CS_BATCHES], cs_records = crow[CS_RECORDS],
+             cs_pub_ns = crow[CS_PUB_NS], cs_loop_ns = crow[CS_LOOP_NS];
+    const uint64_t t_start = globaltimer_ns();
+    bool wide = false;
 
     for (;;) {
-        uint64_t st = 0, rv = 0, v = 0;
+        uint64_t st = 0, rv = 0, st_b = 0, rv_b = 0, v = 0;
         const uint64_t seen_before = seen;
         {
             const uint64_t rn = seen + (uint64_t)(lane >> 3);
             ld_relaxed_sys_2x64(&ring[rn & PUBMASK].w[2 * (lane & 7)], st, rv);
-            const uint32_t okm = __ballot_sync(0xffffffffu, st == rn + 1);
+            if (wide) ld_relaxed_sys_2x64(&ring[(rn + 4) & PUBMASK].w[2 * (lane & 7)], st_b, rv_b);
+            const uint64_t okm = (uint64_t)__ballot_sync(0xffffffffu, st == rn + 1) |
+                                 ((uint64_t)__ballot_sync(0xffffffffu, wide && st_b == rn + 5) << 32);
             uint32_t nvalid = 0;
-            while (nvalid < 4 && ((okm >> (8 * nvalid)) & 0xffu) == 0xffu) nvalid++;
-            if (nvalid) {
-                published = __shfl_sync(0xffffffffu, rv, 8 * (nvalid - 1) + PR_CUM);
-                seen += nvalid;
-            }
+            while (nvalid < 8 && ((okm >> (8 * nvalid)) & 0xffull) == 0xffull) nvalid++;
+            for (uint32_t i = 0; i < nvalid; i++) {
+                const uint64_t e = __shfl_sync(0xffffffffu, i < 4 ? rv : rv_b, 8 * (i & 3) + PR_END);
+                const uint64_t c = __shfl_sync(0xffffffffu, i < 4 ? rv : rv_b, 8 * (i & 3) + PR_CUM);
+                if (e & PR_SELF) {
+                    pend = false;
+                    self_hi = seen + i + 1;
+                } else {
+                    pend = true; pend_end = e; pend_cumt = c | term16; need_fenced = self_hi;
+                }
+                published = c;
+            }
+            seen += nvalid;
+            wide = nvalid >= 4;
             S_rec_ok = nvalid != 0;
-        }
+            if (cstat) cs_records += nvalid;
+        }
+        if (pend) {
+            bool ok = need_fenced <= fenced_seen;
+            if (!ok) {
+                uint64_t f = 0;
+                if (lane == 0) f = ld_relaxed_sys(&seq->pub_fenced);
+                fenced_seen = __shfl_sync(0xffffffffu, f, 0);
+                ok = need_fenced <= fenced_seen;
+            }
+            if (ok) {
+                const uint64_t tp0 = cstat ? globaltimer_ns() : 0;
+                fence_acq_rel_gpu();
+                __syncwarp();
+                __threadfence_system();
+                if (peer_ctrl) st_relaxed_sys_2x64(&peer_ctrl->pub_end, pend_end, pend_cumt);
+                pend = false;
+                if (cstat) { cs_batches++; cs_pub_ns += globaltimer_ns() - tp0; }
+            }
+        }
+        if (cstat) cs_loops++;
         if (lane < N && lane != me) v = ld_relaxed_sys(&ctrl->ack[lane]);
         if (lane == me) v = published;
         int cnt = 0;
@@ -405,7 +456,7 @@
                 if (nc == 0) break;
                 const int base = 8 * (int)(nc - 1);
                 committed = __shfl_sync(0xffffffffu, val, base + PR_CUM);
-                off = __shfl_sync(0xffffffffu, val, base + PR_END);
+                off = __shfl_sync(0xffffffffu, val, base + PR_END) & ~PR_SELF;
                 tickets = __shfl_sync(0xffffffffu, val, base + PR_TICKETS);
                 r_tail = __shfl_sync(0xffffffffu, val, base + PR_TAIL);
                 r_hwm = __shfl_sync(0xffffffffu, val, base + PR_HWM);
@@ -454,11 +505,11 @@
         const bool rec_ok = S_rec_ok;
         int ex = 0;
         if (lane == 0) {
-            if (!rec_ok && tail == seen && committed == published && ld_acquire_gpu(&seq->workers_done) == cx->n_workers) {
+            if (!rec_ok && !pend && tail == seen && committed == published && ld_acquire_gpu(&seq->workers_done) == cx->n_workers) {
                 ex = 3;
             } else if ((++spins & 0x3ffu) == 0) {
                 if (ld_relaxed_sys(&seq->abort_flag)) ex = 2;
-                else if (globaltimer_ns() - last_progress > WATCHDOG_NS && (tail != seen || committed != published) &&
+                else if (globaltimer_ns() - last_progress > WATCHDOG_NS && (tail != seen || committed != published || pend) &&
                          (cx->target != ~0ull || ld_relaxed_sys_u32(&hw->stop))) {
                     st_relaxed_sys(&hw->error, APUS_KERR_WATCHDOG_COMMIT);
                     st_relaxed_sys(&seq->abort_flag, 1);
@@ -474,6 +525,10 @@
             ex = more ? 0 : 1;
         }
         if (ex) {
+            if (cstat && lane == 0) {
+                crow[CS_LOOPS] = cs_loops; crow[CS_BATCHES] = cs_batches; crow[CS_RECORDS] = cs_records;
+                crow[CS_PUB_NS] = cs_pub_ns; crow[CS_LOOP_NS] = cs_loop_ns + (globaltimer_ns() - t_start);
+            }
             if (ex == 1 && cx->target != ~0ull && lane < N && lane != me && cx->peer[lane]) {
                 apus_ctrl_t *pc = reinterpret_cast<apus_ctrl_t *>(cx->peer[lane]);
                 st_relaxed_sys(&pc->fin_entries, committed);
@@ -648,8 +703,8 @@
 {
     __syncwarp();
     if (lane == 0) {
-        __threadfence_system();
-        st_relaxed_sys_2x64(seq->pub_turn, X.next_seq, X.pub_h);
+        fence_acq_rel_gpu();
+        atomicMax(reinterpret_cast<unsigned long long *>(&seq->pub_fenced), (unsigned long long)X.pub_h);
     }
     X.hold = 0;
     __syncwarp();
@@ -680,18 +735,19 @@
     uint64_t ackv = 0;
     if (isf) ackv = ld_relaxed_sys(&ctrl->ack[lane]);
 
-    uint64_t placed = X.placed, end = X.end, tf = X.tf, headv = X.head;
+    uint64_t placed = X.placed, end = X.end, tf = X.tf, headv = X.head, h = X.pub_h;
     if (!(X.have_place && X.next_seq == claimed)) {
         uint32_t ab = 0;
         if (lane == 0) {
-            uint64_t s0, s1, s2, s3;
+            uint64_t s0, s1, s2, s3, s4;
             uint32_t spins = 0;
             for (;;) {
                 ld_relaxed_sys_2x64(seq->rec_placed, s0, placed);
                 ld_relaxed_sys_2x64(seq->rec_end, s1, end);
                 ld_relaxed_sys_2x64(seq->rec_tail, s2, tf);
                 ld_relaxed_sys_2x64(seq->rec_head, s3, headv);
-                if (s0 == claimed && s1 == claimed && s2 == claimed && s3 == claimed) break;
+                ld_relaxed_sys_2x64(seq->rec_pubh, s4, h);
+                if (s0 == claimed && s1 == claimed && s2 == claimed && s3 == claimed && s4 == claimed) break;
                 if ((++spins & 0x3ffu) == 0 && ld_relaxed_sys(&seq->abort_flag)) { ab = 1; break; }
             }
         }
@@ -699,7 +755,8 @@
         if (ab) return 2;
         placed = __shfl_sync(0xffffffffu, placed, 0); end = __shfl_sync(0xffffffffu, end, 0);
         tf = __shfl_sync(0xffffffffu, tf, 0); headv = __shfl_sync(0xffffffffu, headv, 0);
-        X.placed = placed; X.end = end; X.tf = tf; X.head = headv; X.have_place = 1; X.next_seq = claimed;
+        h = __shfl_sync(0xffffffffu, h, 0);
+        X.placed = placed; X.end = end; X.tf = tf; X.head = headv; X.pub_h = h; X.have_place = 1; X.next_seq = claimed;
     }
     const bool wrapped = (tf & APUS_REC_WRAPPED) != 0;
     const uint64_t pos0 = (end == L) ? 0 : end;
@@ -718,8 +775,9 @@
         st_relaxed_sys_2x64(seq->rec_end, claimed + 1, ne);
         st_relaxed_sys_2x64(seq->rec_tail, claimed + 1, a | (nw ? APUS_REC_WRAPPED : 0ull));
         st_relaxed_sys_2x64(seq->rec_head, claimed + 1, headv);
-    }
-    X.placed = cum; X.end = ne; X.tf = a | (nw ? APUS_REC_WRAPPED : 0ull); X.head = headv; X.have_place = 1;
+        st_relaxed_sys_2x64(seq->rec_pubh, claimed + 1, h + 1);
+    }
+    X.placed = cum; X.end = ne; X.tf = a | (nw ? APUS_REC_WRAPPED : 0ull); X.head = headv; X.pub_h = h + 1; X.have_place = 1;
     const uint64_t idx = S->idx_base + placed + 1;
     const bool xprof = (cx->flags & APUS_FLAG_PROFILE) != 0;
     const uint64_t t_place = xprof ? globaltimer_ns() : 0;
@@ -794,22 +852,6 @@
     const bool caught = __ballot_sync(0xffffffffu, isf && ackv != placed) == 0;
 
     const uint64_t t_push = xprof ? globaltimer_ns() : 0;
-    uint64_t h = X.pub_h;
-    if (!X.hold) {
-        uint32_t ab = 0;
-        if (lane == 0) {
-            uint64_t sq;
-            uint32_t spins = 0;
-            for (;;) {
-                ld_acquire_gpu_2x64(seq->pub_turn, sq, h);
-                if (sq == claimed) break;
-                if ((++spins & 0x3ffu) == 0 && ld_relaxed_sys(&seq->abort_flag)) { ab = 1; break; }
-            }
-        }
-        ab = __shfl_sync(0xffffffffu, ab, 0);
-        if (ab) return 2;
-        h = __shfl_sync(0xffffffffu, h, 0);
-    }
     if (lane == 0) {
         uint32_t spins = 0;
         while (h - X.pub_tail_seen >= APUS_PUBRING_RECORDS - 2) {
@@ -820,36 +862,28 @@
     __syncwarp();
     const uint64_t t_turn = xprof ? globaltimer_ns() : 0;
     const uint64_t cumt = cum | ((cx->term & 0xffffull) << APUS_PUB_TERM_SHIFT);
-    const bool cert = caught && !(cx->flags & APUS_FLAG_NO_EXPRESS);
-    if (isf) {
+    const bool cert = caught;
+    if (!cert && X.hold) express_release(seq, X, lane);
+    if (cert && isf) {
         apus_ctrl_t *pc = reinterpret_cast<apus_ctrl_t *>(cx->peer[lane]);
-        if (cert) {
-            st_relaxed_sys_2x64(&pc->pub_csum, cs + cs_key(cumt), a);
-            st_relaxed_sys_2x64(&pc->pub_end, ne | APUS_PUB_CERT, cumt);
-        } else {
-            __threadfence_system();
-            st_relaxed_sys_2x64(&pc->pub_end, ne, cumt);
-        }
-    }
+        st_relaxed_sys_2x64(&pc->pub_csum, cs + cs_key(cumt), a);
+        st_relaxed_sys_2x64(&pc->pub_end, ne | APUS_PUB_CERT, cumt);
+    }
+    __syncwarp();
     if (lane >= 16 && lane < 24) {
         const int q = lane - 16;
-        const uint64_t val = q == PR_CUM ? cum : q == PR_END ? ne : q == PR_TICKETS ? claimed + 1
+        const uint64_t val = q == PR_CUM ? cum : q == PR_END ? (ne | (cert ? PR_SELF : 0ull)) : q == PR_TICKETS ? claimed + 1
                            : q == PR_T0 ? t_deq : q == PR_TAIL ? a : q == PR_HWM ? (nw ? L : b)
                            : q == PR_NEXTIDX ? idx + 1 : (uint64_t)es * (uint64_t)(N - 1);
+        if (!cert) fence_acq_rel_gpu();
         st_relaxed_sys_2x64(&pubring[h & PUBMASK].w[2 * q], h + 1, val);
     }
-    X.next_seq = claimed + 1; X.pub_h = h + 1;
+    X.next_seq = claimed + 1;
     if (xprof) {
         const uint64_t t_end = globaltimer_ns();
         X.dt[0] = t_place - t_deq; X.dt[1] = t_compose - t_place; X.dt[2] = t_push - t_compose; X.dt[3] = t_turn - t_push; X.dt[4] = t_end - t_turn;
     }
-    if (cert) {
-        X.hold = 1;
-    } else {
-        X.hold = 0;
-        __syncwarp();
-        if (lane == 0) st_relaxed_sys_2x64(seq->pub_turn, claimed + 1, h + 1);
-    }
+    if (cert) X.hold = 1;
     return 0;
 }
 
@@ -880,8 +914,8 @@
             seq->rec_end[0] = ctrl->consumed; seq->rec_end[1] = hdr->end;
             seq->rec_tail[0] = ctrl->consumed; seq->rec_tail[1] = hdr->tail | (ctrl->hwm == cx->log_len ? APUS_REC_WRAPPED : 0ull);
             seq->rec_head[0] = ctrl->consumed; seq->rec_head[1] = hdr->head;
-            seq->pub_head = 0; seq->pub_tail = 0;
-            seq->pub_turn[0] = ctrl->consumed; seq->pub_turn[1] = 0;
+            seq->pub_head = 0; seq->pub_tail = 0; seq->pub_fenced = 0;
+            seq->rec_pubh[0] = ctrl->consumed; seq->rec_pubh[1] = 0;
             __threadfence();
             st_release_gpu(&seq->ready_epoch, cx->epoch);
         } else {
@@ -912,10 +946,25 @@
     }
 
     uint64_t last_progress = globaltimer_ns();
-    const bool prof = (cx->flags & APUS_FLAG_STATS) != 0 && tid == 0 && wid == 0;
-    uint64_t ph[8], tn[8], tprev = globaltimer_ns();
-    for (int i = 0; i < 8; i++) { ph[i] = ctrl->phase_ns[i]; tn[i] = ctrl->turn_ns[i]; }
+    const bool prof = (cx->flags & APUS_FLAG_STATS) != 0 && tid == 0;
+    uint64_t *wrow = (prof && wid < APUS_WSTAT_ROWS)
+                         ? reinterpret_cast<uint64_t *>(cx->region + APUS_WSTAT_OFF) + (size_t)wid * APUS_WSTAT_WORDS : nullptr;
+    uint64_t *ph = S->prof_ph, *tn = S->prof_tn, tprev = globaltimer_ns();
+    if (prof) for (int i = 0; i < 8; i++) { ph[i] = 0; tn[i] = 0; }
+    if (prof && wid == 0) {
+        for (int i = 0; i < 8; i++) { ph[i] = ctrl->phase_ns[i]; tn[i] = ctrl->turn_ns[i]; }
+    } else if (wrow) {
+        ph[7] = wrow[WS_TILES]; tn[0] = wrow[WS_CLAIM]; tn[1] = wrow[WS_PLACE]; tn[2] = wrow[WS_PUBLISH]; tn[5] = wrow[WS_EXPRESS];
+        for (int q = 0; q < 6; q++) ph[1 + q] = wrow[WS_PHASE + q];
+    }
 #define PHASE(i) do { if (prof) { const uint64_t _t = globaltimer_ns(); ph[i] += _t - tprev; tprev = _t; } } while (0)
+#define PROF_FLUSH() do { if (prof) {                                                                                   \
+        if (wid == 0) for (int _i = 0; _i < 8; _i++) { ctrl->phase_ns[_i] = ph[_i]; ctrl->turn_ns[_i] = tn[_i]; }       \
+        if (wrow) {                                                                                                     \
+            wrow[WS_TILES] = ph[7]; wrow[WS_CLAIM] = tn[0]; wrow[WS_PLACE] = tn[1]; wrow[WS_PUBLISH] = tn[2];           \
+            wrow[WS_EXPRESS] = tn[5];                                                                                   \
+            for (int _q = 0; _q < 6; _q++) wrow[WS_PHASE + _q] = ph[1 + _q];                                            \
+        } } } while (0)
     Express X;
     X.next_seq = 0; X.placed = 0; X.end = 0; X.tf = 0; X.head = 0; X.pub_h = 0; X.have_place = 0; X.hold = 0; X.pub_tail_seen = 0;
     for (int q = 0; q < 5; q++) X.dt[q] = 0;
@@ -1007,7 +1056,7 @@
                             st_relaxed_sys(&hw->error, APUS_KERR_WATCHDOG_LEADER);
                             st_relaxed_sys(&seq->abort_flag, 1); stopf = 1;
                         }
-                        if (prof) for (int i = 0; i < 8; i++) { ctrl->phase_ns[i] = ph[i]; ctrl->turn_ns[i] = tn[i]; }
+                        PROF_FLUSH();
                     }
                     stopf = __shfl_sync(0xffffffffu, stopf, 0);
                     if (stopf) { fin = 1; break; }
@@ -1045,7 +1094,7 @@
             if (lane == 0) { st_relaxed_sys(&seq->avg_es, (se + nf - 1) / nf); st_relaxed_sys(&seq->avg_xb, (sx + nf - 1) / nf); }
         }
         const apus_cslot_t *sl = reinterpret_cast<const apus_cslot_t *>(slots);
-        bool have_pub_turn = false, have_place_turn = false, aborted = false;
+        bool have_place_turn = false, aborted = false;
         uint64_t gap_bytes = 0;
 
         while (S->kbase < nf) {
@@ -1067,16 +1116,18 @@
                     if (lane == 0) {
                         uint32_t spins = 0;
                         const uint64_t tw0 = prof ? globaltimer_ns() : 0;
-                        uint64_t s0, s1, s2, s3, placed, end, tf, headv;
+                        uint64_t s0, s1, s2, s3, s4, placed, end, tf, headv, pubh;
                         for (;;) {
                             ld_relaxed_sys_2x64(seq->rec_placed, s0, placed);
                             ld_relaxed_sys_2x64(seq->rec_end, s1, end);
                             ld_relaxed_sys_2x64(seq->rec_tail, s2, tf);
                             ld_relaxed_sys_2x64(seq->rec_head, s3, headv);
-                            if (s0 == S->my_seq && s1 == S->my_seq && s2 == S->my_seq && s3 == S->my_seq) break;
+                            ld_relaxed_sys_2x64(seq->rec_pubh, s4, pubh);
+                            if (s0 == S->my_seq && s1 == S->my_seq && s2 == S->my_seq && s3 == S->my_seq && s4 == S->my_seq) break;
                             if ((++spins & 0x3ffu) == 0 && ld_relaxed_sys(&seq->abort_flag)) { S->abort = 1; break; }
                         }
                         if (prof) { tn[1] += globaltimer_ns() - tw0; S->t_place_acq = globaltimer_ns(); }
+                        S->pub_h = pubh;
                         if (S->abort) { S->fast = 1; S->blocked = 0; goto place_done; }
                         {
                         const uint64_t L = cx->log_len;
@@ -1118,6 +1169,7 @@
                             st_relaxed_sys_2x64(seq->rec_end, S->my_seq + S->n_fetch, ne);
                             st_relaxed_sys_2x64(seq->rec_tail, S->my_seq + S->n_fetch, nt | (nw ? APUS_REC_WRAPPED : 0ull));
                             st_relaxed_sys_2x64(seq->rec_head, S->my_seq + S->n_fetch, headv);
+                            st_relaxed_sys_2x64(seq->rec_pubh, S->my_seq + S->n_fetch, pubh + 1);
                             if (prof) { tn[7] += globaltimer_ns() - S->t_place_acq; tn[3]++; }
                             const uint64_t hwm = wrapped ? L : pos0;
                             S->gap = 0; S->ghost = 0; S->blocked = 0; S->last = 1;
@@ -1159,6 +1211,7 @@
                         st_relaxed_sys_2x64(seq->rec_tail, S->my_seq + S->n_fetch, S->st_tail | (S->st_hwm == cx->log_len ? APUS_REC_WRAPPED : 0ull) |
                                                                               (S->st_prev_head ? APUS_REC_PREV_HEAD : 0ull));
                         st_relaxed_sys_2x64(seq->rec_head, S->my_seq + S->n_fetch, S->st_head);
+                        st_relaxed_sys_2x64(seq->rec_pubh, S->my_seq + S->n_fetch, S->pub_h + 1);
                         if (prof) tn[7] += globaltimer_ns() - S->t_place_acq;
                     }
                 }
@@ -1326,61 +1379,45 @@
                 continue;
             }
             if (warp == 0) {
-                const bool pubs = lane < N && lane != me && cx->peer[lane];
-                if (pubs) __threadfence_system();
                 if (lane == 0) {
-                    if (!have_pub_turn) {
-                        uint32_t spins = 0;
-                        const uint64_t tw0 = prof ? globaltimer_ns() : 0;
-                        uint64_t sq, h;
-                        for (;;) {
-                            ld_acquire_gpu_2x64(seq->pub_turn, sq, h);
-                            if (sq == S->my_seq) break;
-                            if ((++spins & 0x3ffu) == 0 && ld_relaxed_sys(&seq->abort_flag)) { S->abort = 1; break; }
-                        }
-                        if (prof) tn[2] += globaltimer_ns() - tw0;
-                        S->pub_h = h;
-                    }
                     uint32_t spins = 0;
-                    while (!S->abort && S->pub_h - S->pub_tail_seen >= APUS_PUBRING_RECORDS - 2) {
+                    const uint64_t tw0 = prof ? globaltimer_ns() : 0;
+                    while (S->pub_h - S->pub_tail_seen >= APUS_PUBRING_RECORDS - 2) {
                         S->pub_tail_seen = ld_relaxed_sys(&seq->pub_tail);
                         if ((++spins & 0x3ffu) == 0 && ld_relaxed_sys(&seq->abort_flag)) { S->abort = 1; break; }
                     }
+                    if (prof) tn[2] += globaltimer_ns() - tw0;
                 }
                 __syncwarp();
-                const bool pub_ok = S->abort == 0;
-                if (pubs && pub_ok) {
-                    apus_ctrl_t *pc = reinterpret_cast<apus_ctrl_t *>(cx->peer[lane]);
-                    st_relaxed_sys_2x64(&pc->pub_end, S->new_end, S->cum_after | ((cx->term & 0xffffull) << APUS_PUB_TERM_SHIFT));
-                }
-                if (pub_ok && lane >= 16 && lane < 24) {
+                if (S->abort == 0 && lane >= 16 && lane < 24) {
                     const int q = lane - 16;
                     const uint64_t h = S->pub_h;
                     const uint64_t val = q == PR_CUM ? S->cum_after : q == PR_END ? S->new_end : q == PR_TICKETS ? S->slot0 + kbase + m
                                        : q == PR_T0 ? S->t_dequeue : q == PR_TAIL ? S->tail_after : q == PR_HWM ? S->hwm_after
                                        : q == PR_NEXTIDX ? S->idx0 + m + autoh : (b - a + gap_bytes) * (uint64_t)(N - 1);
+                    fence_acq_rel_gpu();
                     st_relaxed_sys_2x64(&pubring[h & PUBMASK].w[2 * q], h + 1, val);
                 }
                 __syncwarp();
-                if (lane == 0 && pub_ok) {
+                if (lane == 0 && S->abort == 0) {
                     S->pub_h += 1;
-                    if (S->last) st_relaxed_sys_2x64(seq->pub_turn, S->my_seq + S->n_fetch, S->pub_h);
                     S->kbase = kbase + m;
                 }
             }
-            have_pub_turn = true;
             gap_bytes = 0;
             last_progress = globaltimer_ns();
             bar_sync(1, NT);
             if (S->abort) { aborted = true; break; }
             if (prof) {
                 PHASE(6); ph[7]++;
-                for (int i = 0; i < 8; i++) { ctrl->phase_ns[i] = ph[i]; ctrl->turn_ns[i] = tn[i]; }
+                PROF_FLUSH();
             }
         }
         if (aborted) break;
     }
-    if (prof) for (int i = 0; i < 8; i++) { ctrl->phase_ns[i] = ph[i]; ctrl->turn_ns[i] = tn[i]; }
+    PROF_FLUSH();
+#undef PROF_FLUSH
+#undef PHASE
     if (tid == 0) { __threadfence(); atomicAdd(reinterpret_cast<unsigned long long *>(&seq->workers_done), 1ull); }
 }
 
diff --git a/apus_b200/csrc/apus_layout.h b/apus_b200/csrc/apus_layout.h
--- a/apus_b200/csrc/apus_layout.h
+++ b/apus_b200/csrc/apus_layout.h
@@ -68,6 +68,21 @@
     uint64_t turn_ns[8];
 } apus_ctrl_t;
 
+#define APUS_WSTAT_OFF   2048u
+#define APUS_WSTAT_ROWS  16u
+#define APUS_WSTAT_WORDS 12u
+#define WS_TILES    0
+#define WS_CLAIM    1
+#define WS_PLACE    2
+#define WS_PUBLISH  3
+#define WS_PHASE    4
+#define WS_EXPRESS 10
+#define CS_LOOPS    0
+#define CS_BATCHES  1
+#define CS_RECORDS  2
+#define CS_PUB_NS   3
+#define CS_LOOP_NS  4
+
 #define APUS_CTL_OFF 1024u
 typedef struct apus_vote_req {
     uint64_t sid, index, term;
@@ -88,7 +103,7 @@
     uint64_t claimed_slots;
     uint64_t pad_c[15];
     uint64_t place_seq;      uint64_t pad_d[15];
-    uint64_t pub_turn[2];    uint64_t pad_e[14];
+    uint64_t pub_fenced;     uint64_t pad_e[15];
     uint64_t pub_head;       uint64_t pad_f[15];
     uint64_t pub_tail;       uint64_t pad_g[15];
     uint64_t workers_done;
@@ -99,10 +114,11 @@
     uint64_t rec_end[2];
     uint64_t rec_tail[2];
     uint64_t rec_head[2];
+    uint64_t rec_pubh[2];
     uint64_t avg_es, avg_xb;
     uint64_t doorbell;
     uint64_t w0_idle;
-    uint64_t pad_i[4];
+    uint64_t pad_i[2];
 } apus_seq_t;
 #define APUS_REC_PREV_HEAD (1ull << 62)
 #define APUS_REC_WRAPPED   (1ull << 63)
@@ -115,6 +131,7 @@
 #define PR_HWM     5
 #define PR_NEXTIDX 6
 #define PR_BYTES   7
+#define PR_SELF    (1ull << 63)
 typedef struct apus_pubrec {
     uint64_t w[16];
 } apus_pubrec_t;
diff --git a/apus_b200/engine.py b/apus_b200/engine.py
--- a/apus_b200/engine.py
+++ b/apus_b200/engine.py
@@ -44,6 +44,7 @@
 
 
 _lib = None
+WSTAT_ROWS, WSTAT_WORDS = 16, 12
 
 EXPORTS = [
     "apus_abi_version", "apus_last_error", "apus_device_count", "apus_replica_create",
@@ -57,6 +58,7 @@
     "apus_ctl_read", "apus_ctl_set_sid", "apus_ctl_reset_votes", "apus_ctl_clear_vote_request", "apus_ctl_send_vote_request",
     "apus_ctl_send_vote_ack", "apus_ctl_last_entry", "apus_ctl_adjust_follower", "apus_replica_set_role",
     "apus_replica_disconnect", "apus_follower_beats", "apus_device_numa_node", "apus_group_multicast", "apus_ctl_heartbeat",
+    "apus_worker_stats",
 ]
 
 
@@ -108,6 +110,8 @@
         L.apus_leader_suspect.restype = u64
         L.apus_last_commit_ns.argtypes = [vp]
         L.apus_last_commit_ns.restype = u64
+    if hasattr(L, "apus_worker_stats"):
+        L.apus_worker_stats.argtypes = [vp, C.POINTER(u64), u32]
     _lib = L
     return L
 
@@ -265,6 +269,14 @@
         d = {k: int(getattr(s, k)) for k, _ in Stats._fields_ if k not in ("phase_ns", "turn_ns")}
         d["phase_ns"] = [int(x) for x in s.phase_ns]
         d["turn_ns"] = [int(x) for x in s.turn_ns]
+        if hasattr(lib(), "apus_worker_stats"):
+            rows = (u64 * (WSTAT_WORDS * (WSTAT_ROWS + 1)))()
+            _ck(lib().apus_worker_stats(self.h, rows, WSTAT_ROWS + 1), "apus_worker_stats")
+            r = [[int(x) for x in rows[i * WSTAT_WORDS:(i + 1) * WSTAT_WORDS]] for i in range(WSTAT_ROWS + 1)]
+            d["workers"] = [{"tiles": w[0], "claim_wait_ns": w[1], "place_wait_ns": w[2], "publish_wait_ns": w[3],
+                             "phase_ns": w[4:10], "express": w[10]} for w in r[:WSTAT_ROWS]]
+            c = r[WSTAT_ROWS]
+            d["commit_warp"] = {"loops": c[0], "tail_publishes": c[1], "records": c[2], "publish_ns": c[3], "loop_ns": c[4]}
         return d
 
     def latency_ns(self, max_samples=65536):
diff --git a/include/apus_gpu.h b/include/apus_gpu.h
--- a/include/apus_gpu.h
+++ b/include/apus_gpu.h
@@ -127,6 +127,7 @@
 int  apus_log_offsets(apus_replica_t *r, apus_log_offsets_t *out);
 int  apus_log_read(apus_replica_t *r, uint64_t off, uint64_t len, void *dst);
 int  apus_get_stats(apus_replica_t *r, apus_stats_t *out);
+int  apus_worker_stats(apus_replica_t *r, uint64_t *dst, uint32_t rows);
 int  apus_latency_samples(apus_replica_t *r, uint32_t *dst_ns, uint32_t max, uint32_t *n);
 
 int  apus_set_applied(apus_replica_t *r, uint64_t offset);
```

After: 136.5 million (median of 6 runs). 1.03x the previous value.
